# DeepakSridhar/fgdm

Hardware: AMD Instinct MI355X
Metric: 512x512 images/sec @ 50 DDIM steps, seg-ControlNet+CFG (higher is better)
Workload: dtype f16

## Files before the change

### fgdm_amd/_lib.py

```python
import ctypes as C
import os

HERE = os.path.dirname(os.path.abspath(__file__))
LIB_PATH = os.path.join(HERE, 'libfgdm_hip.so')

MAX_LEVELS = 8
MAX_CONTROLNETS = 4

FLAG_USE_ORIGINAL = 1
FLAG_ONLY_MID_CONTROL = 2
FLAG_NO_CONTROL = 4
FLAG_CFG_PAIRS = 8

ACT_NONE, ACT_SILU, ACT_RELU, ACT_GEGLU, ACT_QGELU = 0, 1, 2, 3, 4
OUT_F16, OUT_F32, OUT_F32_NCHW, OUT_F16_T = 0, 1, 2, 3
STRIDE2_PAD_BR = -2


class FgdmConfig(C.Structure):
    _fields_ = [
        ('in_channels', C.c_int32), ('out_channels', C.c_int32), ('model_channels', C.c_int32),
        ('num_res_blocks', C.c_int32), ('n_levels', C.c_int32), ('channel_mult', C.c_int32 * MAX_LEVELS),
        ('n_attention_resolutions', C.c_int32), ('attention_resolutions', C.c_int32 * MAX_LEVELS),
        ('num_heads', C.c_int32), ('context_dim', C.c_int32), ('use_adapter', C.c_int32),
# ... 38 lines not shown

_p = C.c_void_p
_f = C.c_float
_i = C.c_int
_i64 = C.c_int64

SIGNATURES = {
    'fgdm_create': (_i, [C.POINTER(FgdmConfig), _i, C.POINTER(_p)]),
    'fgdm_destroy': (None, [_p]),
    'fgdm_last_error': (C.c_char_p, [_p]),
    'fgdm_param_count': (_i, [C.POINTER(FgdmConfig)]),
    'fgdm_param_info': (_i, [C.POINTER(FgdmConfig), _i, C.c_char_p, _i, C.POINTER(_i64), C.POINTER(_i)]),
    'fgdm_load_tensor': (_i, [_p, C.c_char_p, _p, _i, C.POINTER(_i64), _i]),
    'fgdm_finalize_weights': (_i, [_p]),
    'fgdm_set_hint': (_i, [_p, _i, _p, _i, _i, _i, _p]),
    'fgdm_set_concat': (_i, [_p, _p, _i, _i, _i, _i, _p]),
    'fgdm_set_adapter_conds': (_i, [_p, _p, _i, _i, _i, _i, _p]),
    'fgdm_set_context': (_i, [_p, _p, _i, _p]),
    'fgdm_apply_model': (_i, [_p, _p, _p, _p, _p, _p, _p, _i, _i, _i, _i, _p, _p]),
    'fgdm_clip_encode': (_i, [_p, _p, _i, _i, _p, _p]),
    'fgdm_clip_encode_skip': (_i, [_p, _p, _i, _i, _i, _p, _p]),
    'fgdm_set_context_tokens': (_i, [_p, _i]),
    'fgdm_get_context_tokens': (_i, [_p]),
    'fgdm_run_block': (_i, [_p, C.c_char_p, _p, _i, _p, _i, _p, _p, _i, _i, _i, _p, _i64, C.POINTER(_i64), _p]),
    'fgdm_vae_decode': (_i, [_p, _p, _i, _i, _i, _f, _p, _p]),
    'fgdm_vae_encode': (_i, [_p, _p, _i, _i, _i, _p, _p]),
    'fgdm_unfold': (_i, [_p] + [_i] * 10 + [_p, _p]),
    'fgdm_fold_weighted': (_i, [_p, _p, _p] + [_i] * 9 + [_p, _p]),
    'fgdm_vae_decode_patches': (_i, [_p, _p, _i, _i, _i, _f] + [_i] * 5 + [_p, _p, _i, _p, _p]),
    'fgdm_apply_model_patches': (_i, [_p, _p, _p, _p, _p] + [_i] * 7 + [_p, _p, _i, _i, _p, _p]),
    'fgdm_posterior_sample': (_i, [_p, _p, _f, _p, _i, _i, _i, _p]),
    'fgdm_image_to_uint8': (_i, [_p, _i, _i, _i, _i, _i, _p, _p]),
    'fgdm_resize_linear_uint8': (_i, [_p, _i, _i, _i, _i, _i, _i, _p, _p]),
    'fgdm_uint8_to_hint': (_i, [_p, _i, _i, _i, _i, _p, _p]),
    'fgdm_controlnet': (_i, [_p, _i, _p, _p, _p, _i, _i, _i, _p, _i64, _p]),
    'fgdm_ddim_step': (_i, [_p, _p, _p, _f, _f, _f, _f, _f, _p, _p, _p, _p, _i64, _p]),
    'fgdm_plms_combine': (_i, [_p, _p, _p, _p, _i, _p, _i64, _p]),
    'fgdm_axpby': (_i, [_p, _f, _p, _f, _p, _i64, _p]),
    'fgdm_mask_blend': (_i, [_p, _p, _p, _p, _i64, _p]),
    'fgdm_ancestral_step': (_i, [_p, _p, _f, _f, _f, _f, _f, _p, _p, _i64, _p]),
    'fgdm_sample_ddim': (_i, [_p, _p, _p, _p, _f, _i, C.POINTER(_i64), C.POINTER(_f), C.POINTER(_f), C.POINTER(_f),
                              _p, _i, _i, _i, _i, _p]),
    'fgdm_sample_ddim_ex': (_i, [_p, C.POINTER(FgdmDdimParams), _p]),
    'fgdm_op_ddim_loop_step': (_i, [_p, _p, _p, _f, _f, _f, _f, _f, _p, _p, _p, _p, _f, _f, _p, _p, _p, _p, _p, _i64, _p]),
    'fgdm_sample_plms': (_i, [_p, C.POINTER(FgdmPlmsParams), _p]),
    'fgdm_sample_dpmpp': (_i, [_p, C.POINTER(FgdmDpmppParams), _p]),
    'fgdm_op_plms_loop_step': (_i, [_p, _p, _p, _f, _i, _i, _p, _p, _p, _p, _f, _f, _f, _p, _p, _p, _f, _f, _p, _p, _p, _p, _p,
                                    _i64, _p]),
    'fgdm_op_dpmpp_loop_step': (_i, [_p, _p, _p, _f, _f, _f, _p, _i, _f, _f, _f, _p, _p, _p, _p, _i64, _p]),
    'fgdm_profile_begin': (_i, [_p, _i]),
    'fgdm_profile_end': (_i, [_p, C.POINTER(C.c_double)]),
    'fgdm_workspace_stats': (_i, [_p, C.POINTER(_i64), C.POINTER(_i64)]),
    'fgdm_launch_stats': (_i, [_p, C.POINTER(_i64), C.POINTER(_i64), C.POINTER(_i64)]),
    'fgdm_replay_plan': (_i, [_i, _p, _p, _p, _p, _i, _i, _p, _i, _p]),
    'fgdm_op_conv2d': (_i, [_p, _i, _p, _i, _p, _p, _p, _p, _i, _i, _i, _i, _i, _i, _i, _i, _f, _p, _p]),
    'fgdm_op_linear': (_i, [_p, _p, _p, _p, _i, _i, _i, _i, _i, _i, _i, _p, _p]),
    'fgdm_debug_force_igemm_cfg': (_i, [_i]),
    'fgdm_bench_igemm': (_i, [_i] * 13 + [C.POINTER(_f)]),
    'fgdm_op_linear_ln_linear': (_i, [_p] * 8 + [_i] * 5 + [_p, _p, C.POINTER(_i), _p]),
    'fgdm_bench_norm': (_i, [_i] * 7 + [C.POINTER(_f)]),
    'fgdm_bench_attention': (_i, [_i] * 6 + [C.POINTER(_f)]),
    'fgdm_bench_ff': (_i, [_i] * 4 + [C.POINTER(_f)]),
    'fgdm_op_groupnorm': (_i, [_p, _i, _p, _i, _i, _i, _p, _p, _f, _i, _p, _p]),
    'fgdm_op_layernorm': (_i, [_p, _i, _i, _p, _p, _f, _p, _p]),
    'fgdm_op_attention': (_i, [_p, _i, _p, _i, _p, _i, _p, _i, _i, _i, _i, _i, _i, _p]),
    'fgdm_op_attention_ex': (_i, [_p, _i, _p, _i, _p, _i, _p, _i, _i, _i, _i, _i, _i, _i, _p]),
    'fgdm_debug_last_attention_kernel': (_i, []),
    'fgdm_op_small_attention': (_i, [_p, _i, _i, _i, _p, _i, _i, _i, _i, _i, _i, _p]),
    'fgdm_op_vae_attention': (_i, [_p, _p, _p, _p, _i, _i, _i, _p]),
    'fgdm_op_softmax_rows': (_i, [_p, _p, _i, _i, _p]),
    'fgdm_op_nchw_to_nhwc': (_i, [_p, _p, _i, _i, _i, _i, _p]),
    'fgdm_op_nhwc_to_nchw': (_i, [_p, _p, _i, _i, _i, _p]),
    'fgdm_op_pack_xcat': (_i, [_p, _p, _i, _i, _i, _i, _i, _i, _p, _p]),
    'fgdm_op_avgpool2': (_i, [_p, _p, _i, _i, _i, _i, _p]),
    'fgdm_op_transpose_pad': (_i, [_p, _p, _i, _i, _i, _i, _p]),
    'fgdm_op_timestep_embed': (_i, [_p, _p, _p, _i, _i, _i, _p]),
    'fgdm_op_add_f16': (_i, [_p, _p, _p, _i64, _p]),
    'fgdm_op_ln_qkv': (_i, [_p] * 6 + [_i] * 5 + [_p, _p, _p]),
}

_lib = None


def load():
    global _lib
    if _lib is not None:
        return _lib
    try:
        import torch
    except ImportError:
        pass
    path = os.environ.get('FGDM_LIB') or LIB_PATH
    if not os.path.exists(path):
        raise RuntimeError(f'{path} not found: build it with `python -m fgdm_amd.build` '
                           '(the HIP engine is mandatory, there is no CPU fallback)')
    lib = C.CDLL(os.path.abspath(path))
    for name, (res, args) in SIGNATURES.items():
        fn = getattr(lib, name)
        fn.restype = res
        fn.argtypes = args
    _lib = lib
    return lib
```

### fgdm_amd/csrc/common.h

```cpp
#pragma once
#include <hip/hip_runtime.h>
#include <stdint.h>

typedef _Float16 half_t;
typedef _Float16 h8 __attribute__((ext_vector_type(8)));
typedef _Float16 h4 __attribute__((ext_vector_type(4)));
typedef _Float16 h2 __attribute__((ext_vector_type(2)));
typedef float f32x16 __attribute__((ext_vector_type(16)));
typedef float f32x4 __attribute__((ext_vector_type(4)));

__device__ __forceinline__ float gelu_f(float x) {
    const float z = fminf(fabsf(x), 6.0f);
    float p = -4.7132482596e-04f;
    p = __builtin_fmaf(p, z, 7.0652551839e-03f);
    p = __builtin_fmaf(p, z, -5.1762067461e-02f);
    p = __builtin_fmaf(p, z, -4.6008771426e-01f);
    p = __builtin_fmaf(p, z, -1.1507295505e+00f);
    p = __builtin_fmaf(p, z, -4.8959157159e-05f - 1.0f);
    const float t = __builtin_amdgcn_exp2f(p);
    return __builtin_fmaf(fabsf(x), 0.5f - t, 0.5f * x);
}

typedef float f32x2 __attribute__((ext_vector_type(2)));
__device__ __forceinline__ f32x2 gelu2_f(f32x2 x) {
    const f32x2 ax = {fabsf(x[0]), fabsf(x[1])};
    const f32x2 z = {fminf(ax[0], 6.0f), fminf(ax[1], 6.0f)};
    auto c = [](float k) { return f32x2{k, k}; };
    f32x2 p = c(-4.7132482596e-04f);
    p = __builtin_elementwise_fma(p, z, c(7.0652551839e-03f));
    p = __builtin_elementwise_fma(p, z, c(-5.1762067461e-02f));
    p = __builtin_elementwise_fma(p, z, c(-4.6008771426e-01f));
    p = __builtin_elementwise_fma(p, z, c(-1.1507295505e+00f));
    p = __builtin_elementwise_fma(p, z, c(-4.8959157159e-05f - 1.0f));
    const f32x2 t = {__builtin_amdgcn_exp2f(p[0]), __builtin_amdgcn_exp2f(p[1])};
    return __builtin_elementwise_fma(ax, c(0.5f) - t, c(0.5f) * x);
}

__device__ __forceinline__ float silu_f(float x, float k = 1.0f) {
    return x * __builtin_amdgcn_rcpf(1.0f + __builtin_amdgcn_exp2f(-1.4426950408889634f * k * x));
}

__device__ __forceinline__ float ln_scale(float acc, float mean, float rstd, float u) {
    float t, w;
    asm("v_fma_f32 %0, %1, %2, %3" : "=v"(t) : "v"(-mean), "v"(u), "v"(acc));
    asm("v_mul_f32 %0, %1, %2" : "=v"(w) : "v"(rstd), "v"(t));
    return w;
}

#define FGDM_OK 0
#define FGDM_ERR_ARG -1
#define FGDM_ERR_HIP -2
#define FGDM_ERR_STATE -3
#define FGDM_ERR_NOMEM -4

enum IgemmMode { IG_LINEAR = 0, IG_CONV3 = 1, IG_CONV3_S2 = 2, IG_CONV3_UP2 = 3, IG_CONV3_S2_BR = 4, IG_CONV2_PHASE = 5 };
enum IgemmAct { ACT_NONE = 0, ACT_SILU = 1, ACT_RELU = 2, ACT_GEGLU = 3, ACT_QGELU = 4  };
enum IgemmOut { OUT_F16 = 0, OUT_F32 = 1, OUT_F32_NCHW = 2, OUT_F16_T = 3 };

struct IgemmArgs {
    const half_t* A0;
    const half_t* A1;
    const half_t* Wt;
    const float* bias;
    const float* rowvec;
    const half_t* resid;
    void* out;
    const half_t* zero;
    int C0, C1;
    int B, H, W;
    int Ho, Wo;
    int M, N;
    int K;
    int mode, act, out_kind;
    int ld_out, ld_res;
    int rv_stride;
    int rows_per_sample;
    float scale;
    int force_cfg;
    int splitk;
    float* ws;
    int debug;
    const float* ln_stats;
    const float* ln_u;
    int ln_slots;
    float ln_eps;
    float* stats_out;
    void* out2;
    int split_n, out_kind2, ld_out2;
};

int igemm_launch(const IgemmArgs& a, hipStream_t s);
bool igemm_up_phase(const IgemmArgs& a);
IgemmArgs igemm_phase_args(const IgemmArgs& a, const half_t* wt_phase);
void igemm_set_force_cfg(int cfg);
void igemm_set_twin_layers(bool on);
void igemm_set_pair_hint(int mult);
int igemm2_launch(const IgemmArgs& a, int cfg, hipStream_t s);
int igemm_stats_slots(const IgemmArgs& a);
int row_stats_slots(int C);
int row_stats_launch(const half_t* x, int rows, int C, float* stats , hipStream_t s);
int igemm_splitk_factor(const IgemmArgs& a);
int igemm_splitk_reduce(const IgemmArgs& a, hipStream_t s);
size_t igemm_npad(int n);

#define GN_PIX_PER_CHUNK 256
void groupnorm_set_group(bool on);
int groupnorm_launch(const half_t* x0, int C0, const half_t* x1, int C1, int B, int HW,
                     const float* gamma, const float* beta, float eps, int silu,
                     half_t* out, float* ws , hipStream_t s);
size_t groupnorm_ws_floats(int B, int HW);
int layernorm_launch(const half_t* x, int rows, int C, const float* gamma, const float* beta, float eps,
                     half_t* out, hipStream_t s);

int attention_launch(const half_t* Q, int ldq, const half_t* K, int ldk, const half_t* Vt, int ldvt,
                     half_t* O, int ldo, int B, int H, int T, int Tk, int d, int q_prescaled, hipStream_t s);
int attention_last_kernel();

int nchw_f32_to_nhwc_f16(const float* x, half_t* y, int B, int C, int HW, int Cpad, hipStream_t s);
int pack_xcat(const float* x, const half_t* cc, half_t* y, int B, int Bc, int Cc, int HW, int Cpad, hipStream_t s);
int f32_to_f16(const float* x, half_t* y, size_t n, hipStream_t s);
int silu_f32_to_f16(const float* x, half_t* y, size_t n, hipStream_t s);
int nhwc_f16_to_nchw_f32(const half_t* x, float* y, int B, int C, int HW, hipStream_t s);
int im2col3x3(const half_t* x, half_t* A, int B, int H, int W, int C, int stride, int Kpad, hipStream_t s);
int avgpool2(const half_t* x, half_t* y, int B, int H, int W, int C, hipStream_t s);
int add_f16(const half_t* a, const half_t* b, half_t* y, size_t n, hipStream_t s);
int add_f16_to_f32(const float* a, const half_t* b, float* y, size_t n, hipStream_t s);
int timestep_embed(const int64_t* t, const float* t_float, half_t* y, int B, int dim, int rows_pad, hipStream_t s);
int vae_prequant(const float* z, const float* wb, float scale, half_t* y, int B, int HW, hipStream_t s);
int vae_moments(const float* h, const float* wb, float* moments, int B, int HW, hipStream_t s);
int posterior_sample(const float* moments, const float* noise, float scale, float* z, int B, int zc, int HW, hipStream_t s);
int softmax_rows(const float* S, half_t* P, int rows, int cols, hipStream_t s);
int image_to_u8(const float* x, uint8_t* y, int B, int C, int HW, int mode, hipStream_t s);
int resize_linear_u8(const uint8_t* src, uint8_t* dst, int B, int H, int W, int C, int Ho, int Wo, hipStream_t s);
int u8_to_hint(const uint8_t* src, float* dst, int B, int HW, int C, hipStream_t s);
int embed_tokens(const int64_t* ids, const float* tok, const float* pos, float* out, int rows, int T, int W, int vocab,
                 hipStream_t s);
int layernorm32_launch(const float* x, int rows, int C, const float* gamma, const float* beta, float eps, half_t* out16,
                       float* out32, hipStream_t s);
int f16_to_f32(const half_t* x, float* y, size_t n, hipStream_t s);
int small_attention_launch(const half_t* qkv, int ld, int koff, int voff, half_t* out, int ldo, int B, int heads, int T,
                           int d, int causal, hipStream_t s);
int transpose_pad_keys(const half_t* v, half_t* vt, int B, int Tk, int C, int Tkpad, hipStream_t s);
int ddim_step(const float* x, const float* e_cond, const float* e_uncond, float cfg_scale,
              float a_t, float a_prev, float sigma_t, float sqrt_one_minus_at, const float* noise,
              float* x_prev, float* pred_x0, float* e_out, size_t n, hipStream_t s);
struct DdimLoopStep {
    const float *x, *ec, *eu, *noise, *mask, *x0, *qnoise;
    float *x_out, *xin_a, *xin_b, *log_x, *log_p0;
    float cfg, a_t, a_prev, sigma, s1m, sa_next, s1m_next;
    size_t n;
};
int ddim_loop_step(const DdimLoopStep& a, hipStream_t s);
enum { PLMS_PROBE = 0, PLMS_FINISH_FIRST = 1, PLMS_MULTISTEP = 2 };
struct PlmsLoopStep {
    const float *x, *ec, *eu, *e1, *e2, *e3, *mask, *x0, *qnoise;
    float *e_out, *x_out, *xin_a, *xin_b, *log_x, *log_p0;
    float cfg, a_t, a_prev, s1m, sa_next, s1m_next;
    int mode, order;
    size_t n;
};
int plms_loop_step(const PlmsLoopStep& a, hipStream_t s);
enum { DPMPP_FIRST = 1, DPMPP_SECOND = 2 };
// ... 58 lines not shown
```

### fgdm_amd/csrc/engine.hip

```cpp
#include "model.h"
#include "knobs.h"
#include "replay.h"

#include <algorithm>
#include <array>
#include <cmath>
#include <cstdlib>
#include <cstdio>
#include <cstring>
#include <map>
#include <memory>
#include <string>
#include <unordered_map>
#include <vector>

namespace {

struct Arena {
    struct Blk { char* p; size_t sz; bool free; };
    std::vector<std::vector<Blk>> slabs;
    std::vector<char*> bases;
    size_t slab_bytes = (size_t)4 << 30;
    size_t in_use = 0, peak = 0;
    bool scoped = false;
// ... 66 lines not shown
            if (on) fgdm_record_bracket_begin(cls, w, nbytes, tag);
            return;
        }
        armed = false;
        if (!on || (counter++ % stride) != 0) return;
        armed = true;
        hipEvent_t e = get();
        if (!e) return;
        (void)hipEventRecord(e, s);
        Rec r{cls, used - 1, 0, w, {0}};
        snprintf(r.tag, sizeof(r.tag), "%s", tag);
        recs.push_back(r);
        work[cls] += w;
        bytes[cls] += nbytes;
    }
    void end(hipStream_t s) override {
        if (fgdm_recording()) {
            if (on) fgdm_record_bracket_end();
            return;
        }
        if (!on || !armed || recs.empty()) return;
        armed = false;
        hipEvent_t e = get();
        if (!e) return;
        (void)hipEventRecord(e, s);
        recs.back().e1 = used - 1;
    }
};

}

struct fgdm_engine : Model {
    int device = -1;
    bool device_ready = false, finalized = false;
    struct CtxKV { Tensor k, vt; };
    std::unordered_map<const Layer*, CtxKV> ctx_cache;
    int ctx_B = 0, ctx_T = 0;
    int ctx_tokens = 77;
    Tensor ccat;
    Arena arena;
    half_t* zero = nullptr;
    int cur_comp = -1;
    bool ln_fold = true;
    hipStream_t s = nullptr;
    std::vector<std::unique_ptr<Arena>> cn_arena;
    Arena* ar = &arena;
    hipStream_t s2 = nullptr;
    hipEvent_t ev_fork = nullptr, ev_join = nullptr;
    bool twin_streams = false;
    bool pair_launch = true;
    int group_max = FGDM_MAX_GROUP;
    bool gn_group = true;
    ReplayStats replay_stats;
    struct Deferred { const GemmW* w; Tensor src; int idx; float scale; Arena* owner; };
    Prof prof;

    const ParamSlot* slot(const std::string& name) {
        auto it = params.find(name);
        if (it == params.end() || !it->second.loaded) { err = "parameter not loaded: " + name; return nullptr; }
        return &it->second;
    }
    template <typename T> T* upload(const std::vector<T>& h) {
        T* d = nullptr;
        if (hipMalloc(&d, std::max<size_t>(h.size() * sizeof(T), 256)) != hipSuccess) return nullptr;
        if (hipMemcpy(d, h.data(), h.size() * sizeof(T), hipMemcpyHostToDevice) != hipSuccess) return nullptr;
        comps[cur_comp].allocs.push_back(d);
        return d;
    }
    int pack_rows(GemmW& g, const std::vector<std::pair<const float*, int>>& srcs, int K_src, int K,
                  const std::vector<int>& kmap, const std::vector<const float*>& biases, bool geglu,
                  const std::vector<float>& src_scale = {}, const float* ln_gamma = nullptr, const float* ln_beta = nullptr) {
        int N = 0;
        for (auto& s : srcs) N += s.second;
        const size_t npad = igemm_npad(N);
        std::vector<half_t> w(npad * (size_t)K, (half_t)0);
        std::vector<float> bias(npad, 0.f), lnu(ln_gamma ? npad : 0, 0.f);
        std::vector<const float*> rowp(N);
        std::vector<float> bflat(N, 0.f), rscale(N, 1.f);
        int r = 0;
        for (size_t si = 0; si < srcs.size(); ++si)
            for (int i = 0; i < srcs[si].second; ++i, ++r) {
                rowp[r] = srcs[si].first + (size_t)i * K_src;
                if (si < biases.size() && biases[si]) bflat[r] = biases[si][i];
                if (si < src_scale.size()) rscale[r] = src_scale[si];
            }
        for (int pr = 0; pr < N; ++pr) {
            int sr = pr;
            if (geglu) {
                const int grp = pr >> 6, within = pr & 63;
                sr = within < 32 ? grp * 32 + within : N / 2 + grp * 32 + (within - 32);
            }
            const float* src = rowp[sr];
            const float rs = rscale[sr];
            half_t* dst = w.data() + (size_t)pr * K;
            if (ln_gamma) {
                double us = 0.0, cs = 0.0;
                for (int k = 0; k < K; ++k) {
                    dst[k] = (half_t)(src[k] * rs * ln_gamma[k]);
                    us += (double)(float)dst[k];
                    cs += (double)ln_beta[k] * (double)(src[k] * rs);
                }
                lnu[pr] = (float)us;
                bias[pr] = (float)((double)(bflat[sr] * rs) + cs);
                continue;
            }
            if (kmap.empty()) for (int k = 0; k < K; ++k) dst[k] = (half_t)(src[k] * rs);
// ... 102 lines not shown
        if (comp.packed && !comp.dirty) return FGDM_OK;
        for (auto& name : order) {
            const ParamSlot& ps = params[name];
            if (ps.comp == c && ps.loaded && ps.host.empty())
                return fail(FGDM_ERR_STATE, "tensor " + name + " was released after packing: reload every tensor of " + comp.prefix +
                                            " before finalizing again");
        }
        for (void* p : comp.allocs) (void)hipFree(p);
        comp.allocs.clear();
        cur_comp = c;
        Packer pk{*this};
        visit_component(c, pk);
        cur_comp = -1;
        if (pk.rc != FGDM_OK) return pk.rc;
        for (auto& name : order) { ParamSlot& ps = params[name]; if (ps.comp == c) std::vector<float>().swap(ps.host); }
        comp.packed = true;
        comp.dirty = false;
        return FGDM_OK;
    }

#define CHK(x) do { int _rc = (x); if (_rc != FGDM_OK) return _rc; } while (0)
    int dcopy(void* dst, const void* src, size_t bytes) {
        auto run = [=](hipStream_t rs) -> int { return hipMemcpyAsync(dst, src, bytes, hipMemcpyDeviceToDevice, rs) == hipSuccess ? FGDM_OK : FGDM_ERR_HIP; };
        if (!fgdm_recording()) return run(s);
        fgdm_record(run);
        return FGDM_OK;
    }
    int dzero(void* dst, size_t bytes) {
        auto run = [=](hipStream_t rs) -> int { return hipMemsetAsync(dst, 0, bytes, rs) == hipSuccess ? FGDM_OK : FGDM_ERR_HIP; };
        if (!fgdm_recording()) return run(s);
        fgdm_record(run);
        return FGDM_OK;
    }
    Tensor talloc(int B, int H, int W, int C) {
        Tensor t; t.B = B; t.H = H; t.W = W; t.C = C;
        t.p = (half_t*)ar->alloc(t.numel() * sizeof(half_t));
        return t;
    }
    void tfree(Tensor& t) { ar->release(t.p); t.p = nullptr; }

    struct LnStats { float* p = nullptr; int slots = 0; };
    struct Epi {
        const LnStats* ln = nullptr;
        LnStats* stats = nullptr;
        int act = ACT_NONE;
        const float* rowvec = nullptr; int rv_stride = 0;
        const half_t* resid = nullptr; int ld_res = 0;
        float scale = 1.f;
        int out_kind = OUT_F16;
        void* out = nullptr;
        int ld_out = 0;
        void* out2 = nullptr; int out_kind2 = OUT_F16, ld_out2 = 0, split_n = 0;
        int rps = 0;
    };
    int gemm(const GemmW& w, int mode, const Tensor& x0, const Tensor* x1, int Ho, int Wo, const Epi& e, Tensor* out) {
        IgemmArgs a{};
        a.A0 = x0.p; a.C0 = x0.C;
        a.A1 = x1 ? x1->p : nullptr; a.C1 = x1 ? x1->C : 0;
        a.Wt = w.w; a.bias = w.bias;
        a.rowvec = e.rowvec; a.rv_stride = e.rv_stride;
        a.resid = e.resid; a.ld_res = e.ld_res;
        a.zero = zero;
        a.B = x0.B; a.H = x0.H; a.W = x0.W; a.Ho = Ho; a.Wo = Wo;
        a.M = x0.B * Ho * Wo;
        a.N = w.N;
        a.K = w.K;
        a.mode = mode; a.act = e.act; a.out_kind = e.out_kind;
        const int nout = e.act == ACT_GEGLU ? w.N / 2 : w.N;
        a.out = e.out ? e.out : (void*)out->p;
        a.ld_out = e.ld_out ? e.ld_out : nout;
        a.rows_per_sample = e.rps ? e.rps : Ho * Wo;
        a.scale = e.scale;
        a.out2 = e.out2; a.out_kind2 = e.out_kind2; a.ld_out2 = e.ld_out2; a.split_n = e.split_n;
        const int taps = mode == IG_LINEAR ? 1 : 9;
        if (taps * (a.C0 + a.C1) != a.K) return fail(FGDM_ERR_ARG, "gemm: K mismatch");
        if (!a.out) return fail(FGDM_ERR_NOMEM, "gemm: null output (workspace exhausted?)");
        if (w.wph && !e.stats && !e.ln && igemm_up_phase(a)) a = igemm_phase_args(a, w.wph);
        char tag[56] = "";
        if (prof.on) snprintf(tag, sizeof(tag), "igemm M%d N%d K%d mode%d act%d out%d l%ds%dr%dv%d", a.M, a.N, a.K, a.mode, a.act, a.out_kind,
                              e.ln ? 1 : 0, e.stats ? 1 : 0, e.resid ? 1 : 0, e.rowvec ? 1 : 0);
        a.splitk = igemm_splitk_factor(a);
        if (a.splitk > 1) {
            a.ws = (float*)ar->alloc((size_t)a.splitk * a.M * a.N * sizeof(float));
            if (!a.ws) return fail(FGDM_ERR_NOMEM, "workspace (split-K partials)");
        }
        if (e.ln) {
            if (!w.ln_u || !e.ln->p || a.splitk > 1) return fail(FGDM_ERR_STATE, "gemm: LayerNorm fold without folded weights / statistics");
            a.ln_stats = e.ln->p; a.ln_slots = e.ln->slots; a.ln_u = w.ln_u; a.ln_eps = w.ln_eps;
        } else if (w.ln_u) {
            return fail(FGDM_ERR_STATE, "gemm: these weights have a LayerNorm folded in; statistics are required");
        }
        if (e.stats) {
            e.stats->slots = igemm_stats_slots(a);
            e.stats->p = (float*)ar->alloc((size_t)a.M * std::max(e.stats->slots, row_stats_slots(nout)) * 2 * sizeof(float));
            if (!e.stats->p) return fail(FGDM_ERR_NOMEM, "workspace (LayerNorm statistics)");
            if (e.stats->slots) a.stats_out = e.stats->p;
        }
        double nbytes = 0.0;
        if (prof.on) {
            const double in_b = 2.0 * ((double)x0.numel() + (x1 ? (double)x1->numel() : 0.0));
            const double out_b = (double)a.M * nout * (e.out_kind == OUT_F16 || e.out_kind == OUT_F16_T ? 2.0 : 4.0);
            nbytes = in_b + 2.0 * (double)w.N * w.K + out_b + (e.resid ? 2.0 * (double)a.M * nout : 0.0);
        }
        prof.begin(PC_IGEMM, s, 2.0 * (double)x0.B * Ho * Wo * (double)w.N * (double)w.k_real, tag, nbytes);
        int rc = igemm_launch(a, s);
        prof.end(s);
        if (a.ws) ar->release(a.ws);
        if (rc == FGDM_OK && e.stats && e.stats->slots == 0) {
            if (a.out_kind != OUT_F16 || a.ld_out != nout) return fail(FGDM_ERR_ARG, "gemm: row statistics need a dense fp16 output");
            e.stats->slots = row_stats_slots(nout);
            prof.begin(PC_NORM, s, 2.0 * (double)a.M * nout, "row_stats");
            rc = row_stats_launch((const half_t*)a.out, a.M, nout, e.stats->p, s);
            prof.end(s);
        }
        return rc == FGDM_OK ? rc : fail(rc, "igemm launch failed");
    }
    int conv3(const GemmW& w, const Tensor& x, const Tensor* x1, int stride, bool up, Epi e, Tensor* out) {
        int Ho = x.H, Wo = x.W, mode = IG_CONV3;
        if (up) { Ho *= 2; Wo *= 2; mode = IG_CONV3_UP2; }
        else if (stride == 2) { Ho = (x.H - 1) / 2 + 1; Wo = (x.W - 1) / 2 + 1; mode = IG_CONV3_S2; }
        else if (stride == FGDM_STRIDE2_PAD_BR) { Ho = (x.H - 2) / 2 + 1; Wo = (x.W - 2) / 2 + 1; mode = IG_CONV3_S2_BR; }
        const bool own_out = (e.out == nullptr);
        if (own_out) { *out = talloc(x.B, Ho, Wo, w.N); if (!out->p) return fail(FGDM_ERR_NOMEM, "workspace"); }
        if (!w.im2col) return gemm(w, mode, x, x1, Ho, Wo, e, out);
        if (up || x1 || x.C != w.cin_pad || stride == FGDM_STRIDE2_PAD_BR) return fail(FGDM_ERR_ARG, "im2col conv path: unsupported combination");
        Tensor A = talloc(1, 1, x.B * Ho * Wo, w.K);
        if (!A.p) return fail(FGDM_ERR_NOMEM, "workspace (im2col)");
        prof.begin(PC_ELEM, s, 2.0 * (double)A.numel() + 2.0 * (double)x.numel());
        bool in_gemm = false;
        const int rc = im2col_conv(x.p, A.p, x.B, x.H, x.W, x.C, stride, w.K, s, [&]() { prof.end(s); },
            [&](half_t* Ap, int Bv, int Hv, int Wv, int Kv, int rps) {
                in_gemm = true;
                Tensor Av; Av.p = Ap; Av.B = Bv; Av.H = Hv; Av.W = Wv; Av.C = Kv;
                if (!e.rps) e.rps = rps;
                return gemm(w, IG_LINEAR, Av, nullptr, Hv, Wv, e, out);
            });
        if (rc != FGDM_OK && !in_gemm) return fail(rc, "im2col failed");
        tfree(A);
        return rc;
    }
    int linear(const GemmW& w, const Tensor& x, Epi e, Tensor* out, const Tensor* x1 = nullptr) {
        if (!e.out) { *out = talloc(x.B, x.H, x.W, e.act == ACT_GEGLU ? w.N / 2 : w.N); if (!out->p) return fail(FGDM_ERR_NOMEM, "workspace"); }
        return gemm(w, IG_LINEAR, x, x1, x.H, x.W, e, out);
    }
    int gnorm(const NormW& n, const Tensor& x, const Tensor* x1, float eps, bool silu, Tensor* out) {
        const int C = x.C + (x1 ? x1->C : 0);
        *out = talloc(x.B, x.H, x.W, C);
        float* ws = (float*)ar->alloc(groupnorm_ws_floats(x.B, x.H * x.W) * sizeof(float));
        if (!out->p || !ws) return fail(FGDM_ERR_NOMEM, "workspace");
        char tag[56] = "";
        if (prof.on) snprintf(tag, sizeof(tag), "groupnorm B%d HW%d C%d", x.B, x.H * x.W, C);
        prof.begin(PC_NORM, s, 4.0 * (double)out->numel(), tag);
        const int rc = groupnorm_launch(x.p, x.C, x1 ? x1->p : nullptr, x1 ? x1->C : 0, x.B, x.H * x.W, n.g, n.b, eps,
                                        silu ? 1 : 0, out->p, ws, s);
        prof.end(s);
        ar->release(ws);
        return rc == FGDM_OK ? rc : fail(rc, "groupnorm launch failed");
    }
    int lnorm(const NormW& n, const Tensor& x, Tensor* out) {
        *out = talloc(x.B, x.H, x.W, x.C);
        if (!out->p) return fail(FGDM_ERR_NOMEM, "workspace");
        char tag[56] = "";
        if (prof.on) snprintf(tag, sizeof(tag), "layernorm rows%d C%d", x.rows(), x.C);
        prof.begin(PC_NORM, s, 4.0 * (double)out->numel(), tag);
        const int rc = layernorm_launch(x.p, x.rows(), x.C, n.g, n.b, 1e-5f, out->p, s);
        prof.end(s);
        return rc == FGDM_OK ? rc : fail(rc, "layernorm launch failed");
    }

    struct EmbCtx { const float* emb_all; int stride; };

    int res_fwd(const Layer& l, const Tensor& x, const Tensor* x1, const EmbCtx& ec, Tensor* out) {
        Tensor g1, h, g2, sk, xp;
        CHK(gnorm(l.gn1, x, x1, l.eps, true, &g1));
        const Tensor* xs = &x;
        if (l.down) {
            if (x1) return fail(FGDM_ERR_ARG, "down ResBlock with a concatenated input");
            Tensor gp = talloc(x.B, x.H / 2, x.W / 2, x.C);
            xp = talloc(x.B, x.H / 2, x.W / 2, x.C);
            if (!gp.p || !xp.p) return fail(FGDM_ERR_NOMEM, "workspace");
            if (avgpool2(g1.p, gp.p, x.B, x.H, x.W, x.C, s) != FGDM_OK || avgpool2(x.p, xp.p, x.B, x.H, x.W, x.C, s) != FGDM_OK)
                return fail(FGDM_ERR_ARG, "avgpool2: latent size must be divisible by 8 for the adapter");
            tfree(g1);
            g1 = gp;
            xs = &xp;
        }
        Epi e1;
        if (l.emb_off >= 0) { e1.rowvec = ec.emb_all + l.emb_off; e1.rv_stride = ec.stride; }
        CHK(conv3(l.c1, g1, nullptr, 1, false, e1, &h));
        tfree(g1);
        CHK(gnorm(l.gn2, h, nullptr, l.eps, true, &g2));
        tfree(h);
        Epi e2;
        if (l.cin != l.cout) {
            CHK(linear(l.skip, *xs, Epi{}, &sk, x1));
            e2.resid = sk.p; e2.ld_res = sk.C;
        } else {
            e2.resid = xs->p; e2.ld_res = xs->C;
        }
        CHK(conv3(l.c2, g2, nullptr, 1, false, e2, out));
        tfree(g2);
        if (sk.p) tfree(sk);
        if (xp.p) tfree(xp);
        return FGDM_OK;
    }

    int cross_kv(const Layer& l, const Tensor& ctx16, bool persistent, Tensor* k2, Tensor* v2t) {
        const int B = ctx16.B, C = l.cin, Tk = ctx16.H * ctx16.W, Tkp = roundup(Tk, 64);
        if (persistent) {
            k2->B = B; k2->H = ctx16.H; k2->W = ctx16.W; k2->C = C;
            v2t->B = B; v2t->H = 1; v2t->W = C; v2t->C = Tkp;
            if (hipMalloc(&k2->p, k2->numel() * sizeof(half_t)) != hipSuccess ||
                hipMalloc(&v2t->p, v2t->numel() * sizeof(half_t)) != hipSuccess) return fail(FGDM_ERR_NOMEM, "hipMalloc (context cache)");
            { Epi e; e.out = k2->p; e.ld_out = C; CHK(linear(l.k2, ctx16, e, nullptr)); }
        } else {
            CHK(linear(l.k2, ctx16, Epi{}, k2));
            *v2t = talloc(B, 1, C, Tkp);
            if (!v2t->p) return fail(FGDM_ERR_NOMEM, "workspace");
        }
        if (Tkp != Tk) CHK(dzero(v2t->p, v2t->numel() * sizeof(half_t)));
        { Epi e; e.out_kind = OUT_F16_T; e.out = v2t->p; e.ld_out = Tkp; e.rps = Tk; CHK(linear(l.v2, ctx16, e, nullptr)); }
        return FGDM_OK;
    }
    void drop_context() {
        for (auto& kv : ctx_cache) { (void)hipFree(kv.second.k.p); (void)hipFree(kv.second.vt.p); }
        ctx_cache.clear();
        ctx_B = 0;
    }
    int set_context(const float* ctx, int B) {
        if (!finalized) return fail(FGDM_ERR_STATE, "weights not finalized");
        if (B <= 0) return fail(FGDM_ERR_ARG, "bad shape");
        drop_context();
        Tensor ctx16 = talloc(B, 1, ctx_tokens, cfg.context_dim);
        if (!ctx16.p) return fail(FGDM_ERR_NOMEM, "workspace");
        if (f32_to_f16(ctx, ctx16.p, ctx16.numel(), s) != FGDM_OK) return fail(FGDM_ERR_HIP, "convert kernel");
        auto walk = [&](const Block& blk) -> int {
            for (const Layer& l : blk)
                if (l.type == L_ATTN) { CtxKV kv; CHK(cross_kv(l, ctx16, true, &kv.k, &kv.vt)); ctx_cache[&l] = kv; }
            return FGDM_OK;
        };
        CHK(for_each_block(unet, false, walk));
        for (auto& n : cns) CHK(for_each_block(n, false, walk));
        tfree(ctx16);
        ctx_B = B; ctx_T = ctx_tokens;
        return FGDM_OK;
    }

    int attn_fwd(const Layer& l, const Tensor& x_in, const Tensor& ctx16, Tensor* out, bool dup = false) {
        Tensor x = x_in, x_full;
        int B = x.B;
        const int T = x.H * x.W, C = x.C, d = C / l.heads;
        Tensor g, h, qk, vt, a, h2, q2, k2, v2t, f;
        LnStats s1, s2, s3;
        CHK(gnorm(l.gn, x, nullptr, 1e-6f, false, &g));
        Tensor nrm;
        { Epi e; if (ln_fold) e.stats = &s1; CHK(linear(l.pin, g, e, &h)); }
        tfree(g);
        if (!ln_fold) CHK(lnorm(l.ln1, h, &nrm));
        const Tensor& a1 = ln_fold ? h : nrm;
        const int Tp = roundup(T, 64);
        qk = talloc(B, x.H, x.W, 2 * C);
        vt = talloc(B, 1, C, Tp);
        if (!qk.p || !vt.p) return fail(FGDM_ERR_NOMEM, "workspace");
        if (Tp != T) CHK(dzero(vt.p, vt.numel() * sizeof(half_t)));
        { Epi e; if (ln_fold) e.ln = &s1; e.out = qk.p; e.ld_out = 2 * C; e.rps = T;
          e.out2 = vt.p; e.out_kind2 = OUT_F16_T; e.ld_out2 = Tp; e.split_n = 2 * C;
          CHK(linear(l.qkv1, a1, e, nullptr)); }
        if (s1.p) ar->release(s1.p);
        if (nrm.p) tfree(nrm);
        a = talloc(B, x.H, x.W, C);
        if (!a.p) return fail(FGDM_ERR_NOMEM, "workspace");
        { char tag[56]; snprintf(tag, sizeof(tag), "attn B%d T%d Tk%d d%d", B, T, T, d);
          prof.begin(PC_ATTN, s, 4.0 * (double)B * T * (double)T * C, tag);
          int rc = attention_launch(qk.p, 2 * C, qk.p + C, 2 * C, vt.p, Tp, a.p, C, B, l.heads, T, T, d, 1, s);
          prof.end(s);
          if (rc != FGDM_OK) return fail(rc, "attention launch failed (unsupported head dim?)"); }
        tfree(qk); tfree(vt);
        { Epi e; e.resid = h.p; e.ld_res = C; if (ln_fold) e.stats = &s2; CHK(linear(l.o1, a, e, &h2)); }
        tfree(a); tfree(h);
        if (dup) {
            Tensor f2;
            CHK(dup_rows(h2, &f2)); tfree(h2); h2 = f2;
            CHK(dup_rows(x, &x_full)); x = x_full;
            B *= 2;
        }
        if (dup && ln_fold) {
            const size_t sb = (size_t)(B / 2) * T * s2.slots * 2 * sizeof(float);
            float* s2f = (float*)ar->alloc(2 * sb);
            if (!s2f) return fail(FGDM_ERR_NOMEM, "workspace");
            CHK(dcopy(s2f, s2.p, sb));
            CHK(dcopy((char*)s2f + sb, s2.p, sb));
            ar->release(s2.p); s2.p = s2f;
        }
        if (!ln_fold) CHK(lnorm(l.ln2, h2, &nrm));
        { Epi e; if (ln_fold) e.ln = &s2; CHK(linear(l.q2, ln_fold ? h2 : nrm, e, &q2)); }
        if (s2.p) ar->release(s2.p);
        if (nrm.p) tfree(nrm);
        int Tk, Tkp;
        const bool cached = (ctx16.p == nullptr);
        if (cached) {
            auto it = ctx_cache.find(&l);
            if (it == ctx_cache.end() || ctx_B != B) return fail(FGDM_ERR_STATE, "no cached context for this batch (fgdm_set_context)");
            k2 = it->second.k; v2t = it->second.vt;
            Tk = ctx_T; Tkp = roundup(Tk, 64);
        } else {
            Tk = ctx16.H * ctx16.W; Tkp = roundup(Tk, 64);
            CHK(cross_kv(l, ctx16, false, &k2, &v2t));
        }
        a = talloc(B, x.H, x.W, C);
        if (!a.p) return fail(FGDM_ERR_NOMEM, "workspace");
        { char tag[56]; snprintf(tag, sizeof(tag), "attn B%d T%d Tk%d d%d", B, T, Tk, d);
          prof.begin(PC_ATTN, s, 4.0 * (double)B * T * (double)Tk * C, tag);
          int rc = attention_launch(q2.p, C, k2.p, C, v2t.p, Tkp, a.p, C, B, l.heads, T, Tk, d, 1, s);
          prof.end(s);
          if (rc != FGDM_OK) return fail(rc, "attention launch failed"); }
        tfree(q2);
        if (!cached) { tfree(k2); tfree(v2t); }
        { Epi e; e.resid = h2.p; e.ld_res = C; if (ln_fold) e.stats = &s3; CHK(linear(l.o2, a, e, &h)); }
        tfree(a); tfree(h2);
        if (!ln_fold) CHK(lnorm(l.ln3, h, &nrm));
        { Epi e; if (ln_fold) e.ln = &s3; e.act = ACT_GEGLU; CHK(linear(l.ffp, ln_fold ? h : nrm, e, &f)); }
        if (s3.p) ar->release(s3.p);
        if (nrm.p) tfree(nrm);
        { Epi e; e.resid = h.p; e.ld_res = C; CHK(linear(l.ffo, f, e, &h2)); }
        tfree(f); tfree(h);
        { Epi e; e.resid = x.p; e.ld_res = C; CHK(linear(l.pout, h2, e, out)); }
        tfree(h2);
        if (x_full.p) tfree(x_full);
        return FGDM_OK;
    }

    int dup_rows(const Tensor& h, Tensor* full) {
        *full = talloc(2 * h.B, h.H, h.W, h.C);
        if (!full->p) return fail(FGDM_ERR_NOMEM, "workspace");
        const size_t bytes = h.numel() * sizeof(half_t);
        CHK(dcopy(full->p, h.p, bytes));
        CHK(dcopy((char*)full->p + bytes, h.p, bytes));
        return FGDM_OK;
    }
    int block_fwd_shared(const Block& blk, Tensor xh, bool own_x, const EmbCtx& ec, const Tensor& ctx16, Tensor* out) {
        Tensor cur = xh;
        bool own = own_x, full = false;
        for (size_t j = 0; j < blk.size(); ++j) {
            const Layer& l = blk[j];
            Tensor nxt;
            switch (l.type) {
                case L_CONV: CHK(conv3(l.conv, cur, nullptr, 1, false, Epi{}, &nxt)); break;
                case L_RES: CHK(res_fwd(l, cur, nullptr, ec, &nxt)); break;
                case L_ATTN: CHK(attn_fwd(l, cur, ctx16, &nxt, !full)); full = true; break;
                case L_DOWN: CHK(conv3(l.conv, cur, nullptr, 2, false, Epi{}, &nxt)); break;
                case L_UP: CHK(conv3(l.conv, cur, nullptr, 1, true, Epi{}, &nxt)); break;
            }
            if (own) tfree(cur);
            cur = nxt;
            own = true;
        }
        if (!full) { Tensor f; CHK(dup_rows(cur, &f)); if (own) tfree(cur); cur = f; }
        *out = cur;
        return FGDM_OK;
    }

    int block_fwd(const Block& blk, Tensor x, bool own_x, const Tensor* x1, const EmbCtx& ec, const Tensor& ctx16,
                  const half_t* conv_resid, Tensor* out) {
        Tensor cur = x;
        bool own = own_x;
        for (size_t j = 0; j < blk.size(); ++j) {
            const Layer& l = blk[j];
            Tensor nxt;
            switch (l.type) {
                case L_CONV: { Epi e; if (conv_resid) { e.resid = conv_resid; e.ld_res = l.cout; }
                               CHK(conv3(l.conv, cur, nullptr, 1, false, e, &nxt)); break; }
                case L_RES: CHK(res_fwd(l, cur, j == 0 ? x1 : nullptr, ec, &nxt)); break;
                case L_ATTN: CHK(attn_fwd(l, cur, ctx16, &nxt)); break;
                case L_DOWN: CHK(conv3(l.conv, cur, nullptr, 2, false, Epi{}, &nxt)); break;
                case L_UP: CHK(conv3(l.conv, cur, nullptr, 1, true, Epi{}, &nxt)); break;
            }
            if (own) tfree(cur);
            cur = nxt;
            own = true;
        }
        *out = cur;
        return FGDM_OK;
    }

    int embed(Net& n, const int64_t* t, const float* tf, int B, float** emb_all) {
        const int mc = cfg.model_channels;
        Tensor te = talloc(1, 1, B, mc), e1, e2;
        if (!te.p) return fail(FGDM_ERR_NOMEM, "workspace");
        if (timestep_embed(t, tf, te.p, B, mc, B, s) != FGDM_OK) return fail(FGDM_ERR_HIP, "timestep_embed");
        { Epi e; e.act = ACT_SILU; e.rps = 1; CHK(linear(n.time0, te, e, &e1)); }
        { Epi e; e.act = ACT_SILU; e.rps = 1; CHK(linear(n.time2, e1, e, &e2)); }
        *emb_all = (float*)ar->alloc((size_t)B * n.emb_total * sizeof(float));
        if (!*emb_all) return fail(FGDM_ERR_NOMEM, "workspace");
        { Epi e; e.out_kind = OUT_F32; e.out = *emb_all; e.ld_out = n.emb_total; e.rps = 1; CHK(linear(n.emb_all, e2, e, nullptr)); }
        tfree(te); tfree(e1); tfree(e2);
        return FGDM_OK;
    }

    int adapter_fwd(Net& n, const Tensor& x4, Tensor feats[4]) { return adapter_run(n.ad_conv_in, n.ad_body, x4, feats); }
    int adapter_run(const GemmW& conv_in, const std::vector<AdapterBlk>& body, const Tensor& x4, Tensor feats[4]) {
        Tensor cur;
        CHK(conv3(conv_in, x4, nullptr, 1, false, Epi{}, &cur));
        auto drop = [&](Tensor& t) {
            for (int f = 0; f < 4; ++f) if (feats[f].p == t.p) return;
            tfree(t);
        };
        for (size_t k = 0; k < body.size(); ++k) {
            const AdapterBlk& b = body[k];
            if (b.down) {
                Tensor p = talloc(cur.B, cur.H / 2, cur.W / 2, cur.C);
                if (!p.p) return fail(FGDM_ERR_NOMEM, "workspace");
                if (avgpool2(cur.p, p.p, cur.B, cur.H, cur.W, cur.C, s) != FGDM_OK)
                    return fail(FGDM_ERR_ARG, "avgpool2: latent size must be divisible by 8 for the adapter");
                drop(cur);
                cur = p;
            }
            if (b.ic != b.oc) { Tensor y; CHK(linear(b.in_conv, cur, Epi{}, &y)); drop(cur); cur = y; }
            Tensor h, y;
            { Epi e; e.act = ACT_RELU; CHK(conv3(b.b1, cur, nullptr, 1, false, e, &h)); }
            { Epi e; e.resid = cur.p; e.ld_res = cur.C; CHK(linear(b.b2, h, e, &y)); }
            tfree(h);
            drop(cur);
            cur = y;
            if (k % 2 == 1) feats[k / 2] = cur;
        }
        return FGDM_OK;
    }

    void drop_adapter_conds() {
        for (Tensor& t : unet.xad_sum) { if (t.p) (void)hipFree(t.p); t = Tensor{}; }
        unet.xad_valid = false;
    }
    int set_adapter_conds(const float* const* conds, int nc, int B, int H, int W) {
// ... 318 lines not shown
                        half_t* dst = nxt.p + (size_t)half * fa[k].numel();
                        if (n.xad_valid) {
                            if (n.xad_sum[k].numel() != nxt.numel()) return fail(FGDM_ERR_ARG, "registered adapter conds do not match this batch / latent size");
                            const half_t* xs = n.xad_sum[k].p + (size_t)half * fa[k].numel();
                            if (add_f16(dst, xs, dst, fa[k].numel(), s) != FGDM_OK) return fail(FGDM_ERR_HIP, "add kernel");
                        }
                        if (add_f16(dst, fa[k].p, dst, fa[k].numel(), s) != FGDM_OK) return fail(FGDM_ERR_HIP, "add kernel");
                    }
                    tfree(fa[k]);
                    ++k;
                }
                h = nxt;
                hs.push_back(h);
            }
            CHK(block_fwd(n.middle, h, false, nullptr, ec, ctx16, nullptr, &hm));
            return FGDM_OK;
        };
        if (paired) {
            std::vector<RecWalk> walks(1 + cns.size());
            {
                const bool fat = knob_once(KNOB_PAIR_FAT_TILES) != 0;
                LayerHints fused(*this, false, fat ? std::min<int>(group_max, 1 + (int)cns.size()) : 0);
                groupnorm_set_group(gn_group);
                CHK(controlnets_fwd(x4, t, tf, ctx16, scales, nullptr, nullptr, false, pairs, &deferred,
                                    [&](size_t c) { return RecordScope(*this, &walks[1 + c], cn_arena[c].get()); }));
                RecordScope rec(*this, &walks[0], &arena);
                CHK(encoder());
            }
            std::vector<RecWalk*> lists;
            for (RecWalk& w : walks) lists.push_back(&w);
            CHK(fgdm_replay(lists, group_max, s, prof, replay_stats));
        } else {
            if (twin) {
                if (hipEventRecord(ev_fork, s) != hipSuccess || hipStreamWaitEvent(s2, ev_fork, 0) != hipSuccess) return fail(FGDM_ERR_HIP, "stream fork");
                hipStream_t main_s = s;
                s = s2;
                const int rc = controlnets_fwd(x4, t, tf, ctx16, scales, nullptr, nullptr, false, pairs, &deferred,
                                               [&](size_t) { return RecordScope(*this, nullptr, cn_arena[0].get()); });
                s = main_s;
                if (rc != FGDM_OK) return rc;
                if (hipEventRecord(ev_join, s2) != hipSuccess) return fail(FGDM_ERR_HIP, "stream join");
            }
            CHK(encoder());
        }
        if (twin || paired) {
            if (twin && hipStreamWaitEvent(s, ev_join, 0) != hipSuccess) return fail(FGDM_ERR_HIP, "stream join");
            for (const Deferred& d : deferred) CHK(zero_conv_into(*d.w, d.src, d.idx < 0 ? hm : hs[d.idx], d.scale));
            for (Deferred& d : deferred) { d.owner->release(d.src.p); d.src.p = nullptr; }
        } else if (with_cn) {
            CHK(controlnets_fwd(x4, t, tf, ctx16, scales, &hs, &hm, (flags & FGDM_FLAG_ONLY_MID_CONTROL) != 0, pairs, nullptr,
                                [&](size_t) { return RecordScope(*this, nullptr, &arena); }));
        }
        h = hm;
        for (size_t i = 0; i < n.output.size(); ++i) {
            Tensor skip = hs.back();
            hs.pop_back();
            Tensor nxt;
            CHK(block_fwd(n.output[i], h, true, &skip, ec, ctx16, nullptr, &nxt));
            tfree(skip);
            h = nxt;
        }
        Tensor g;
        CHK(gnorm(n.out_gn, h, nullptr, 1e-5f, true, &g));
        tfree(h);
        { Epi e; e.out_kind = OUT_F32_NCHW; e.out = eps_out; e.ld_out = HW; CHK(conv3(n.out_conv, g, nullptr, 1, false, e, nullptr)); }
        tfree(g);
        tfree(x4);
        if (ctx16.p) tfree(ctx16);
        ar->release(emb);
        return FGDM_OK;
    }

    int clip_encode(const int64_t* ids, int B, int T, float* out, int clip_skip = 0) {
        if (!clip.on) return fail(FGDM_ERR_STATE, "engine was created without a text encoder (clip_layers = 0)");
        if (!comps[clip_comp].packed) return fail(FGDM_ERR_STATE, "weights not finalized");
        if (B <= 0 || T <= 0 || T > cfg.clip_max_len) return fail(FGDM_ERR_ARG, "bad shape (T must be <= clip_max_len)");
        if (clip_skip > cfg.clip_layers + 1) return fail(FGDM_ERR_ARG, "clip_skip exceeds the number of hidden states");
        const int n_run = cfg.clip_layers - (clip_skip > 1 ? clip_skip - 1 : 0);
        int li = 0;
        const int W = cfg.clip_width, rows = B * T;
        Tensor n, qkv, a, f;
        float* h = (float*)ar->alloc((size_t)rows * W * sizeof(float));
        float* h2 = (float*)ar->alloc((size_t)rows * W * sizeof(float));
        if (!h || !h2) return fail(FGDM_ERR_NOMEM, "workspace");
        if (embed_tokens(ids, clip.tok, clip.pos, h, rows, T, W, cfg.clip_vocab, s) != FGDM_OK) return fail(FGDM_ERR_HIP, "embedding kernel");
        auto ln32 = [&](const NormW& nw, const float* src, Tensor* dst) -> int {
            *dst = talloc(1, 1, rows, W);
            if (!dst->p) return fail(FGDM_ERR_NOMEM, "workspace");
            return layernorm32_launch(src, rows, W, nw.g, nw.b, 1e-5f, dst->p, nullptr, s) == FGDM_OK ? FGDM_OK : fail(FGDM_ERR_HIP, "layernorm");
        };
        for (const ClipLayer& l : clip.layers) {
            if (li++ >= n_run) break;
            CHK(ln32(l.ln1, h, &n));
            CHK(linear(l.qkv, n, Epi{}, &qkv));
            tfree(n);
            a = talloc(1, 1, rows, W);
            if (!a.p) return fail(FGDM_ERR_NOMEM, "workspace");
            if (small_attention_launch(qkv.p, 3 * W, W, 2 * W, a.p, W, B, cfg.clip_heads, T, W / cfg.clip_heads, 1, s) != FGDM_OK)
                return fail(FGDM_ERR_HIP, "text attention kernel");
            tfree(qkv);
            Tensor br;
            CHK(linear(l.o, a, Epi{}, &br));
            tfree(a);
            if (add_f16_to_f32(h, br.p, h2, br.numel(), s) != FGDM_OK) return fail(FGDM_ERR_HIP, "add kernel");
            tfree(br);
            CHK(ln32(l.ln2, h2, &n));
            { Epi e; e.act = ACT_QGELU; CHK(linear(l.fc1, n, e, &f)); }
            tfree(n);
            CHK(linear(l.fc2, f, Epi{}, &br));
            tfree(f);
            if (add_f16_to_f32(h2, br.p, h, br.numel(), s) != FGDM_OK) return fail(FGDM_ERR_HIP, "add kernel");
            tfree(br);
        }
        if (layernorm32_launch(h, rows, W, clip.final_ln.g, clip.final_ln.b, 1e-5f, nullptr, out, s) != FGDM_OK) return fail(FGDM_ERR_HIP, "layernorm");
        ar->release(h); ar->release(h2);
        return FGDM_OK;
// ... 139 lines not shown
    void drop_concat() { if (ccat.p) (void)hipFree(ccat.p); ccat = Tensor{}; }
    int set_concat(const float* cc, int B, int Cc, int H, int W) {
        if (cfg.in_channels == 4) return fail(FGDM_ERR_ARG, "fgdm_set_concat: this engine's UNet takes x alone (in_channels = 4)");
        if (!cc) { drop_concat(); return FGDM_OK; }
        if (Cc != cfg.in_channels - 4) {
            drop_concat();
            return fail(FGDM_ERR_ARG, "fgdm_set_concat: c_concat must have in_channels - 4 = " + std::to_string(cfg.in_channels - 4) + " channels");
        }
        if (B <= 0 || H <= 0 || W <= 0) { drop_concat(); return fail(FGDM_ERR_ARG, "bad shape"); }
        if (ccat.p && (ccat.B != B || ccat.H != H || ccat.W != W)) drop_concat();
        if (!ccat.p) {
            ccat.B = B; ccat.H = H; ccat.W = W; ccat.C = Cc;
            if (hipMalloc(&ccat.p, ccat.numel() * sizeof(half_t)) != hipSuccess) { ccat = Tensor{}; return fail(FGDM_ERR_NOMEM, "hipMalloc (c_concat cache)"); }
        }
        if (nchw_f32_to_nhwc_f16(cc, ccat.p, B, Cc, H * W, Cc, s) != FGDM_OK) return fail(FGDM_ERR_HIP, "layout kernel");
        return FGDM_OK;
    }
};

static std::string g_create_err;

static int make_desc(const fgdm_config* cfg, fgdm_engine** out) {
    fgdm_engine* e = new fgdm_engine();
    e->cfg = *cfg;
    const int rc = e->build();
    if (rc != FGDM_OK) { g_create_err = "unsupported configuration: " + e->err; delete e; return rc; }
    *out = e;
    return FGDM_OK;
}

template <typename F> static int scoped_call(fgdm_engine* e, void* stream, F f) {
    e->s = as_stream(stream);
    e->ar = &e->arena;
    e->arena.begin_scope();
    for (auto& a : e->cn_arena) a->begin_scope();
    const int rc = f();
    e->s = as_stream(stream);
    e->ar = &e->arena;
    if (rc != FGDM_OK && e->s2) (void)hipStreamSynchronize(e->s2);
    e->arena.end_scope(rc != FGDM_OK);
    for (auto& a : e->cn_arena) a->end_scope(rc != FGDM_OK);
    return rc;
}

extern "C" {

int fgdm_create(const fgdm_config* cfg, int device, fgdm_engine** out) {
    if (!cfg || !out) return FGDM_ERR_ARG;
    fgdm_engine* e = nullptr;
    int rc = make_desc(cfg, &e);
    if (rc != FGDM_OK) return rc;
    e->device = device;
    e->ln_fold = knob_on(KNOB_LN_FOLD);
    rc = e->ensure_device();
    if (rc != FGDM_OK) {
        g_create_err = e->err + " [" + hipGetErrorString(hipGetLastError()) + "]";
        delete e;
        return rc;
    }
    e->twin_streams = knob_on(KNOB_TWIN_STREAMS);
    e->pair_launch = knob_on(KNOB_PAIR_LAUNCH);
    e->group_max = std::max(2, std::min(FGDM_MAX_GROUP, knob_int(KNOB_GROUP_MAX)));
    e->gn_group = knob_on(KNOB_GN_GROUP);
    if (e->twin_streams && !e->cns.empty()) {
        if (hipStreamCreateWithFlags(&e->s2, hipStreamNonBlocking) != hipSuccess ||
            hipEventCreateWithFlags(&e->ev_fork, hipEventDisableTiming) != hipSuccess ||
            hipEventCreateWithFlags(&e->ev_join, hipEventDisableTiming) != hipSuccess) {
            g_create_err = "second stream could not be created";
            delete e;
            return FGDM_ERR_HIP;
        }
    }
    for (size_t c = 0; c < e->cns.size(); ++c) {
        e->cn_arena.emplace_back(new Arena());
        if (e->cfg.workspace_bytes > 0) e->cn_arena.back()->slab_bytes = (size_t)e->cfg.workspace_bytes;
    }
    *out = e;
    return FGDM_OK;
}

void fgdm_destroy(fgdm_engine* e) {
    if (!e) return;
    for (hipEvent_t ev : e->prof.pool) (void)hipEventDestroy(ev);
    for (auto& c : e->comps) for (void* p : c.allocs) (void)hipFree(p);
    if (e->zero) (void)hipFree(e->zero);
    for (auto& n : e->cns) if (n.guided.p) (void)hipFree(n.guided.p);
    e->drop_concat();
    e->drop_context();
    e->drop_adapter_conds();
    if (knob_text(KNOB_PAIR_DEBUG) && e->replay_stats.replayed)
        fprintf(stderr, "[fgdm] grouped twin launches: %ld of %ld replayed launches were fused (%ld problems)\n", e->replay_stats.fused, e->replay_stats.replayed, e->replay_stats.problems);
    if (e->s2) { (void)hipStreamSynchronize(e->s2); (void)hipStreamDestroy(e->s2); }
    if (e->ev_fork) (void)hipEventDestroy(e->ev_fork);
    if (e->ev_join) (void)hipEventDestroy(e->ev_join);
    delete e;
}

const char* fgdm_last_error(const fgdm_engine* e) { return e ? e->err.c_str() : g_create_err.c_str(); }

static fgdm_engine* g_desc = nullptr;
static fgdm_config g_desc_cfg;
static fgdm_engine* desc_for(const fgdm_config* cfg) {
    if (g_desc && memcmp(&g_desc_cfg, cfg, sizeof(*cfg)) == 0) return g_desc;
    if (g_desc) { delete g_desc; g_desc = nullptr; }
    if (make_desc(cfg, &g_desc) != FGDM_OK) return nullptr;
    g_desc_cfg = *cfg;
// ... 61 lines not shown
    e->prof.counter = 0;
    e->prof.used = 0;
    e->prof.recs.clear();
    for (int c = 0; c < PC_COUNT; ++c) { e->prof.work[c] = 0; e->prof.bytes[c] = 0; }
    return FGDM_OK;
}
int fgdm_profile_end(fgdm_engine* e, double* out) {
    if (!e || !out) return FGDM_ERR_ARG;
    e->prof.on = false;
    if (hipDeviceSynchronize() != hipSuccess) return e->fail(FGDM_ERR_HIP, "hipDeviceSynchronize failed");
    for (int c = 0; c < PC_COUNT * 4; ++c) out[c] = 0;
    for (auto& r : e->prof.recs) {
        if (!r.e1) continue;
        float ms = 0.f;
        if (hipEventElapsedTime(&ms, e->prof.pool[r.e0], e->prof.pool[r.e1]) != hipSuccess) continue;
        out[r.cls * 4 + 0] += ms;
        out[r.cls * 4 + 1] += 1;
    }
    for (int c = 0; c < PC_COUNT; ++c) { out[c * 4 + 2] = e->prof.work[c]; out[c * 4 + 3] = e->prof.bytes[c]; }
    if (const char* path = knob_text(KNOB_PROF_DUMP)) {
        std::map<std::string, std::array<double, 3>> agg;
        for (auto& r : e->prof.recs) {
            if (!r.e1) continue;
            float ms = 0.f;
            if (hipEventElapsedTime(&ms, e->prof.pool[r.e0], e->prof.pool[r.e1]) != hipSuccess) continue;
            auto& a = agg[r.tag];
            a[0] += 1; a[1] += ms; a[2] += r.w;
        }
        if (FILE* f = fopen(path, "w")) {
            for (auto& kv : agg) fprintf(f, "%s\t%.0f\t%.4f\t%.6g\n", kv.first.c_str(), kv.second[0], kv.second[1], kv.second[2]);
            fclose(f);
        }
    }
    return FGDM_OK;
}
int fgdm_workspace_stats(fgdm_engine* e, int64_t* peak_bytes, int64_t* reserved_bytes) {
    if (!e || !peak_bytes || !reserved_bytes) return FGDM_ERR_ARG;
    size_t pk = e->arena.peak, r = 0;
    for (auto& sl : e->arena.slabs) for (auto& b : sl) r += b.sz;
    for (auto& a : e->cn_arena) {
        pk += a->peak;
        for (auto& sl : a->slabs) for (auto& b : sl) r += b.sz;
    }
    *peak_bytes = (int64_t)pk;
    *reserved_bytes = (int64_t)r;
    return FGDM_OK;
}

int fgdm_launch_stats(fgdm_engine* e, int64_t* replayed_launches, int64_t* fused_launches, int64_t* fused_problems) {
    if (!e || !replayed_launches || !fused_launches || !fused_problems) return FGDM_ERR_ARG;
    *replayed_launches = (int64_t)e->replay_stats.replayed;
    *fused_launches = (int64_t)e->replay_stats.fused;
    *fused_problems = (int64_t)e->replay_stats.problems;
    return FGDM_OK;
}

int fgdm_set_hint(fgdm_engine* e, int cn, const float* hint, int B, int Hh, int Wh, void* stream) {
    if (!e || !hint) return FGDM_ERR_ARG;
    return scoped_call(e, stream, [&] { return e->set_hint(cn, hint, B, Hh, Wh); });
}

int fgdm_set_concat(fgdm_engine* e, const float* c_concat, int B, int Cc, int H, int W, void* stream) {
    if (!e) return FGDM_ERR_ARG;
    return scoped_call(e, stream, [&] { return e->set_concat(c_concat, B, Cc, H, W); });
}

int fgdm_apply_model(fgdm_engine* e, const float* x, const int64_t* t, const float* t_float, const float* ctx,
                     const float* pcond, const float* control_scales, int B, int H, int W, int flags, float* eps_out,
                     void* stream) {
    if (!e || !x || (!t && !t_float) || !eps_out) return FGDM_ERR_ARG;
    return scoped_call(e, stream, [&] { return e->apply_model(x, t, t_float, ctx, pcond, control_scales, B, H, W, flags, eps_out); });
}

int fgdm_set_adapter_conds(fgdm_engine* e, const float* const* conds, int n_conds, int B, int H, int W, void* stream) {
    if (!e) return FGDM_ERR_ARG;
    return scoped_call(e, stream, [&] { return e->set_adapter_conds(conds, n_conds, B, H, W); });
}

int fgdm_set_context(fgdm_engine* e, const float* ctx, int B, void* stream) {
    if (!e || !ctx) return FGDM_ERR_ARG;
    return scoped_call(e, stream, [&] { return e->set_context(ctx, B); });
}

int fgdm_clip_encode(fgdm_engine* e, const int64_t* ids, int B, int T, float* out, void* stream) {
    if (!e || !ids || !out) return FGDM_ERR_ARG;
    return scoped_call(e, stream, [&] { return e->clip_encode(ids, B, T, out); });
}

int fgdm_clip_encode_skip(fgdm_engine* e, const int64_t* ids, int B, int T, int clip_skip, float* out, void* stream) {
    if (!e || !ids || !out) return FGDM_ERR_ARG;
    return scoped_call(e, stream, [&] { return e->clip_encode(ids, B, T, out, clip_skip); });
}

int fgdm_set_context_tokens(fgdm_engine* e, int tokens) {
    if (!e) return FGDM_ERR_ARG;
    if (tokens < 1) return e->fail(FGDM_ERR_ARG, "context token count must be >= 1");
    if (tokens != e->ctx_tokens) { e->drop_context(); e->ctx_tokens = tokens; }
    return FGDM_OK;
}

int fgdm_get_context_tokens(const fgdm_engine* e) { return e ? e->ctx_tokens : FGDM_ERR_ARG; }

int fgdm_vae_decode(fgdm_engine* e, const float* z, int B, int H, int W, float scale, float* image, void* stream) {
    if (!e || !z || !image) return FGDM_ERR_ARG;
    return scoped_call(e, stream, [&] { return e->vae_decode(z, B, H, W, scale, image); });
}
// ... 438 lines not shown
```

### fgdm_amd/csrc/igemm.hip

```cpp
#include "common.h"
#include "knobs.h"
#include <algorithm>

#define LDS_AS __attribute__((address_space(3)))
#define GLB_AS __attribute__((address_space(1)))

__device__ __forceinline__ void glds16(const void* g, void* lds_wave_base) {
    __builtin_amdgcn_global_load_lds((const GLB_AS void*)g, (LDS_AS void*)lds_wave_base, 16, 0, 0);
}

template <int BM, int BN, int WM, int WN>
__global__ __launch_bounds__(WM * WN * 64) void igemm_kernel(const IgemmArgs a) {
    constexpr int T = WM * WN * 64;
    constexpr int TM = BM / WM, TN = BN / WN;
    constexpr int MI = TM / 32, NI = TN / 32;
    constexpr int A_IT = BM * 8 / T, B_IT = BN * 8 / T;
    constexpr int A_BYTES = BM * 128, STAGE = (BM + BN) * 128;
    static_assert(A_IT >= 1 && B_IT >= 1, "tile too small for the thread count");
    extern __shared__ __attribute__((aligned(16))) char smem[];

    const int tid = threadIdx.x, lane = tid & 63;
    const int wave = __builtin_amdgcn_readfirstlane(tid >> 6);
    const int wm = wave / WN, wn = wave % WN;

// ... 249 lines not shown
}

static int g_force_cfg = 0;
void igemm_set_force_cfg(int cfg) { g_force_cfg = cfg; }
static thread_local int g_pair_mult = 1;
void igemm_set_pair_hint(int mult) { g_pair_mult = mult > 1 ? mult : 1; }

static int pick_force(const IgemmArgs& a) {
    int force = a.force_cfg ? a.force_cfg : g_force_cfg;
    if (a.act == ACT_QGELU) {
        if (force >= 4) force = 0;
        if (force == 0) return 0;
    }
    const bool small_tiles = knob_once(KNOB_IGEMM_SMALL_TILES) != 0;
    const bool other_widths = knob_once(KNOB_IGEMM_OTHER_WIDTHS) != 0;
    if (a.mode == IG_CONV2_PHASE) {
        if (force >= 4) return force;
        return (long)((a.M + 255) / 256) * (a.N / 320) * 4 * g_pair_mult >= 192 ? 4 : 6;
    }
    if (force == 0) {
        const bool geglu = a.act == ACT_GEGLU;
        if (!geglu && a.N % 320 == 0) {
            const long b256 = (long)((a.M + 255) / 256) * (a.N / 320);
            const long b128 = (long)((a.M + 127) / 128) * (a.N / 320);
            const bool small_m = knob_once(KNOB_IGEMM_SMALL_M) != 0;
            const bool lin64 = a.mode == IG_LINEAR && !(a.K & 31) && !(a.C0 & 31) && !(a.C1 & 31) && small_tiles;
            const long b64 = (long)((a.M + 63) / 64) * (a.N / 160);
            const long b256n = (long)((a.M + 255) / 256) * (a.N / 128);
            if (b256 * g_pair_mult >= 192) force = 4;
            else if (small_m && lin64 && a.K >= 2560 && !(a.N % 128) && !a.ln_stats && !a.stats_out && !a.out2 && b128 >= 96 && b128 * g_pair_mult < 192 &&
                     b64 >= 512 && b256n >= 144 && b256n <= 256) force = 10;
            else if (b128 >= 96 && !(small_m && lin64 && b128 * g_pair_mult < 192 && b64 >= 512)) force = 6;
            else if (lin64 && b64 >= 128) force = 11;
        } else if (geglu && a.N % 256 == 0 && (long)((a.M + 255) / 256) * (a.N / 256) >= 128) {
            force = 5;
        } else if (!geglu && !a.ln_stats && !(a.K & 31) && !(a.C0 & 31) && !(a.C1 & 31) && other_widths) {
            const long rows = (a.M + 255) / 256;
            if (a.N % 256 == 0 && rows * (a.N / 256) >= 192) force = 5;
            else if (a.N == 128 && rows >= 192) force = 10;
        }
    }
    return force;
}

int igemm_stats_slots(const IgemmArgs& a) {
    if (a.out_kind != OUT_F16 || a.act == ACT_GEGLU || a.splitk > 1 || (a.N % 320) || (a.K & 31) || (a.C0 & 31) || (a.C1 & 31)) return 0;
    const int f = pick_force(a);
    if (f < 4) return 0;
    const int tile = (f - 4) & 15;
    const bool stats64 = knob_once(KNOB_IGEMM_STATS64) != 0;
    return (tile == 0 || tile == 2 || tile == 3 || tile == 5 || (tile == 7 && stats64)) ? a.N / 160 : 0;
}

bool igemm_up_phase(const IgemmArgs& a) {
    if (!knob_once(KNOB_IGEMM_UP_PHASE)) return false;
    const int force = a.force_cfg ? a.force_cfg : g_force_cfg;
    if (force >= 1 && force <= 3) return false;
    if (a.H * a.W < 64) return false;
    return a.mode == IG_CONV3_UP2 && !a.C1 && a.C0 > 0 && !(a.C0 & 63) && a.K == 9 * a.C0 && a.N % 320 == 0 && a.out_kind == OUT_F16 &&
           a.act != ACT_GEGLU && a.act != ACT_QGELU && !a.rowvec && !a.stats_out && !a.out2 && !a.ln_stats;
}
IgemmArgs igemm_phase_args(const IgemmArgs& a, const half_t* wt_phase) {
    IgemmArgs p = a;
    p.mode = IG_CONV2_PHASE;
    p.Wt = wt_phase;
    p.K = 4 * a.C0;
    p.M = a.B * a.H * a.W;
    p.rows_per_sample = a.H * a.W;
    p.splitk = 1; p.ws = nullptr;
    return p;
}

int igemm_launch(const IgemmArgs& a, hipStream_t s) {
    if (a.M <= 0 || a.N <= 0 || a.K <= 0 || (a.K & 63) || (a.C0 & 63) || (a.C1 & 63)) return FGDM_ERR_ARG;
    if (a.act == ACT_GEGLU && (a.N & 63)) return FGDM_ERR_ARG;
    if (a.ln_stats && (a.mode != IG_LINEAR || a.C1 || a.ln_slots <= 0 || !a.ln_u)) return FGDM_ERR_ARG;
    if (a.stats_out && igemm_stats_slots(a) == 0) return FGDM_ERR_ARG;
    if (a.out2 && (a.act == ACT_GEGLU || a.splitk > 1 || a.stats_out || a.split_n <= 0 || a.split_n >= a.N || (a.split_n % 640))) return FGDM_ERR_ARG;
    if (a.mode == IG_CONV2_PHASE && (a.splitk > 1 || a.N % 320)) return FGDM_ERR_ARG;
    if (a.splitk > 1) {
        if (!a.ws || a.ln_stats) return FGDM_ERR_ARG;
        const bool fat = (long)((a.M + 255) / 256) * (a.N / 320) * a.splitk >= 192 && !(a.K & 31) && !(a.C0 & 31) && !(a.C1 & 31);
        const int rc = igemm2_launch(a, fat ? 0 : 2, s);
        return rc == FGDM_OK ? igemm_splitk_reduce(a, s) : rc;
    }
    int force = pick_force(a);
    const bool mfma32 = knob_once(KNOB_IGEMM_MFMA32) != 0;
    if (mfma32 && force >= 4 && force <= 6 && !a.force_cfg && !g_force_cfg) force += 3;
    if (force >= 4) return igemm2_launch(a, force - 4, s);
    struct Cfg { int bm, bn; float eff; int per_cu; };
    static const Cfg cfgs[] = {{128, 128, 1.00f, 2}, {128, 64, 0.80f, 3}, {64, 64, 0.62f, 4}};
    int best = 0;
    float best_cost = 1e30f;
    for (int i = 0; i < 3; ++i) {
        const Cfg& c = cfgs[i];
        const long nblk = (long)((a.M + c.bm - 1) / c.bm) * ((a.N + c.bn - 1) / c.bn);
        const long slots = 256L * c.per_cu;
        const float rounds = (float)((nblk + slots - 1) / slots);
        const long conc = std::min<long>(c.per_cu, (nblk + 255) / 256);
        const float cost = rounds * (float)conc * (float)(c.bm * c.bn) / c.eff;
        if (cost < best_cost) { best_cost = cost; best = i; }
    }
    if ((long)((a.M + 127) / 128) * ((a.N + 127) / 128) < 256) best = 2;
    if (a.act == ACT_GEGLU) best = 0;
    if (force >= 1 && force <= 3) best = force - 1;
    switch (best) {
        case 0: return launch_cfg<128, 128, 2, 2>(a, s);
        case 1: return launch_cfg<128, 64, 2, 2>(a, s);
        default: return launch_cfg<64, 64, 2, 2>(a, s);
    }
}
```

### fgdm_amd/csrc/igemm2.hip

```cpp
#include "common.h"
#include "knobs.h"
#include <algorithm>
#include <type_traits>

#pragma clang diagnostic ignored "-Winline-asm"
#define LDS_AS __attribute__((address_space(3)))
#define GLB_AS __attribute__((address_space(1)))

namespace {

__device__ __forceinline__ void glds16(const void* g, unsigned lds_wave_addr) {
    unsigned keep;
    asm volatile("s_mov_b32 %0, m0\n\ts_mov_b32 m0, %2\n\ts_nop 0\n\tglobal_load_lds_dwordx4 %1, off\n\ts_mov_b32 m0, %0"
                 : "=&s"(keep)
                 : "v"(g), "s"(lds_wave_addr)
                 : "memory", "m0");
}
__device__ __forceinline__ void glds16_m0(const void* g, unsigned lds_wave_addr) {
    asm volatile("s_mov_b32 m0, %1\n\ts_nop 0\n\tglobal_load_lds_dwordx4 %0, off" ::"v"(g), "s"(lds_wave_addr) : "memory", "m0");
}
__device__ __forceinline__ void glds16_sv(unsigned voff, const void* sbase, unsigned lds_wave_addr) {
    asm volatile("s_mov_b32 m0, %2\n\ts_nop 0\n\tglobal_load_lds_dwordx4 %0, %1" ::"v"(voff), "s"(sbase), "s"(lds_wave_addr) : "memory", "m0");
}
__device__ __forceinline__ unsigned lds_addr(const void* p) { return (unsigned)(size_t)(LDS_AS const void*)p; }
template <int N> __device__ __forceinline__ void wait_vmcnt() {
    asm volatile("s_waitcnt vmcnt(%0)" ::"n"(N) : "memory");
}

constexpr int BK = 32;
constexpr int ROWB = BK * 2;

constexpr int RV_MAX = 6;

template <int BM> constexpr int halo_px() { return BM == 256 ? 400 : 272; }
template <int BM, int BN, int STAGES, int PIPE> constexpr int ring_bytes() {
    return PIPE == 2 ? 2 * halo_px<BM>() * ROWB + STAGES * BN * ROWB : STAGES * (BM + BN) * ROWB;
}

template <int BM, int BN, int WM, int WN, int STAGES, int CONV, bool GEGLU, bool SPLIT, int MS, bool LN, int PATH, int PIPE, bool ABL>
__device__ __forceinline__ void igemm2_body(const IgemmArgs& a, const int yb) {
    constexpr int NW = WM * WN, T = NW * 64;
    constexpr int TM = BM / WM, TN = BN / WN;
    constexpr int MI = TM / MS, NI = TN / MS;
    constexpr int KS = MS == 32 ? 2 : 1;
    constexpr int AR = MS == 32 ? 16 : 4;
    typedef float acc_t __attribute__((ext_vector_type(AR)));
    auto swz_of = [](int r) { return MS == 32 ? ((r >> 2) & 3) : (((r >> 3) & 1) << 1); };
    constexpr int A_INSTR = BM * 4 / 64, B_INSTR = BN * 4 / 64;
    static_assert(A_INSTR % NW == 0, "A tile must split evenly over the waves");
    constexpr int LA = A_INSTR / NW, LB = (B_INSTR + NW - 1) / NW;
    constexpr int LPS = LA + LB;
    constexpr int STAGE_BYTES = (BM + BN) * ROWB;
    constexpr int A_BYTES = BM * ROWB;
    constexpr int RING_BYTES = ring_bytes<BM, BN, STAGES, PIPE>();
    static_assert(TM % 32 == 0 && TN % MS == 0, "wave tile: 32-pixel epilogue passes, MFMA-sized channel tiles");
    static_assert(!GEGLU || TN % 64 == 0, "GEGLU: whole 64-row [32 value | 32 gate] groups per wave");
    extern __shared__ __attribute__((aligned(16))) char smem[];

    const int tid = threadIdx.x, lane = tid & 63;
    const int wave = __builtin_amdgcn_readfirstlane(tid >> 6);
    const int wm = wave / WN, wn = wave % WN;

    const int ntn = (a.N + BN - 1) / BN;
    const int nb = gridDim.x;
    int logical;
    {
        const int bid = blockIdx.x, xcd = bid & 7, q = nb >> 3, r = nb & 7;
        logical = (xcd < r ? xcd * (q + 1) : r * (q + 1) + (xcd - r) * q) + (bid >> 3);
    }
    const int nsplit = SPLIT ? a.splitk : 1;
    int split = 0, m0, n0;
    if (SPLIT) {
        const int ntm = (a.M + BM - 1) / BM;
        const int row = logical % ntm, pair = logical / ntm;
        split = pair % nsplit; n0 = (pair / nsplit) * BN; m0 = row * BM;
    } else {
        m0 = (logical / ntn) * BM; n0 = (logical % ntn) * BN;
    }

    const int nk_all = a.K >> 5;
    const int per = (nk_all + nsplit - 1) / nsplit;
    const int k_begin = split * per;
    const int nk = max(0, min(per, nk_all - k_begin));

    int a_pix[LA], a_yx[LA], a_off[LA];
    int b_off[LB], b_lds[LB];
    const int br = (CONV && a.mode == IG_CONV3_S2_BR) ? 1 : 0;
    const int sy = (CONV && (a.mode == IG_CONV3_S2 || a.mode == IG_CONV3_S2_BR)) ? 2 : 1;
    const int up = (CONV && a.mode == IG_CONV3_UP2) ? 1 : 0;
    constexpr bool ph = CONV == 2;
    const int pa = ph ? (yb >> 1) : 0, pb = ph ? (yb & 1) : 0;
    const int NT = ph ? 4 : 9;
    const int Wq = ph ? a.W : a.Wo, hwq = ph ? a.H * a.W : a.Ho * a.Wo;
// ... 430 lines not shown
                    const int col = n0 + wn * TN + j * MS + (MS == 32 ? 8 * g : 0) + lq;
                    f32x4 pk = {acc[j][i][g * 4], acc[j][i][g * 4 + 1], acc[j][i][g * 4 + 2], acc[j][i][g * 4 + 3]};
                    *(f32x4*)(wsp + (size_t)row * a.N + col) = pk;
                }
        }
        return;
    } else {
    if (ABL && (a.debug & 4)) {
        float sink = 0.f;
#pragma unroll
        for (int j = 0; j < NI; ++j)
#pragma unroll
            for (int i = 0; i < MI; ++i) sink += acc[j][i][0] + acc[j][i][AR - 1];
        if (sink == 12345.678f) ((float*)a.out)[0] = sink;
        return;
    }
    asm volatile("s_waitcnt lgkmcnt(0)" ::: "memory");
    __builtin_amdgcn_s_barrier();
    if constexpr (LN) {
        const float* uw = u_l + wn * TN;
#pragma unroll
        for (int j = 0; j < NI; ++j)
#pragma unroll
            for (int g = 0; g < AR / 4; ++g) {
                const f32x4 uq = *(const f32x4*)(uw + j * MS + (MS == 32 ? 8 * g : 0) + lq);
#pragma unroll
                for (int i = 0; i < MI; ++i) {
                    const int trow = wm * TM + i * MS + lrow;
                    const float mean = mr_l[2 * trow], rstd = mr_l[2 * trow + 1];
#pragma unroll
                    for (int e = 0; e < 4; ++e) acc[j][i][g * 4 + e] = ln_scale(acc[j][i][g * 4 + e], mean, rstd, uq[e]);
                }
            }
    }
    constexpr int OUT_TN = GEGLU ? TN / 2 : TN;
    constexpr int PITCH = OUT_TN * 2 + 8;
    constexpr int CPR = OUT_TN / 8;
    constexpr int WB_IT = (32 * CPR + 63) / 64;
    static_assert(!GEGLU || NI % 2 == 0, "GEGLU needs value/gate tile pairs");
    constexpr bool TR = PATH == 1 && LN && !GEGLU;
    constexpr int TPITCH = 32 * 2 + 16;
    constexpr int CST_BYTES = TR && OUT_TN * TPITCH > 32 * PITCH ? OUT_TN * TPITCH : 32 * PITCH;
    static_assert(NW * CST_BYTES <= RING_BYTES, "epilogue staging must fit in the ring");
    char* cst = smem + wave * CST_BYTES;
    const bool second = a.out2 && n0 >= a.split_n;
    void* const outp = second ? a.out2 : a.out;
    const int okind = second ? a.out_kind2 : a.out_kind, ldo = second ? a.ld_out2 : a.ld_out;
    const int ncol0 = second ? a.split_n : 0, nend = a.out2 ? (second ? a.N : a.split_n) : a.N;
    const bool tr = TR && okind == OUT_F16_T;
    const int ocol0 = GEGLU ? ((n0 + wn * TN) >> 1) : (n0 + wn * TN - ncol0);
    const int nvalid = GEGLU ? a.N / 2 : nend - ncol0;
    const float* bw = bias_l + wn * TN;

    constexpr int PT = 32 / MS;
    constexpr int NG = AR / 4;
#pragma unroll
    for (int ip = 0; ip < TM / 32; ++ip) {
#pragma unroll
      for (int hf = 0; hf < PT; ++hf) {
        const int i = ip * PT + hf;
        const int prow = hf * MS + lrow;
        const int row = m0 + wm * TM + ip * 32 + prow;
        const int bsmp = (a.rowvec && row < a.M) ? row / rps : smp0;
        const float* rw = rv_l + (bsmp - smp0) * BN + wn * TN;
#pragma unroll
        for (int j = 0; j < NI; ++j) {
            if (GEGLU && (MS == 32 ? (j & 1) : (j & 2))) continue;
#pragma unroll
            for (int g = 0; g < NG; ++g) {
                const int wc = j * MS + (MS == 32 ? 8 * g : 0) + lq;
                const f32x4 bq = *(const f32x4*)(bw + wc);
                float v[4];
#pragma unroll
                for (int e = 0; e < 4; ++e) v[e] = acc[j][i][g * 4 + e] + bq[e];
                if (PATH == 2 || (PATH == 0 && a.rowvec)) {
                    if (PATH == 2 || rv_in_lds) {
                        const f32x4 rq = *(const f32x4*)(rw + wc);
#pragma unroll
                        for (int e = 0; e < 4; ++e) v[e] += rq[e];
                    } else if (row < a.M) {
#pragma unroll
                        for (int e = 0; e < 4; ++e) v[e] += a.rowvec[(size_t)bsmp * a.rv_stride + n0 + wn * TN + wc + e];
                    }
                }
                if (PATH == 0 && a.act == ACT_SILU) {
#pragma unroll
                    for (int e = 0; e < 4; ++e) v[e] = silu_f(v[e]);
                } else if (PATH == 0 && a.act == ACT_RELU) {
#pragma unroll
                    for (int e = 0; e < 4; ++e) v[e] = fmaxf(v[e], 0.f);
                }
                if constexpr (GEGLU) {
                    constexpr int GJ = MS == 32 ? 1 : 2;
                    const f32x4 gq = *(const f32x4*)(bw + wc + 32);
                    const f32x2 g01 = gelu2_f(f32x2{acc[j + GJ][i][g * 4] + gq[0], acc[j + GJ][i][g * 4 + 1] + gq[1]});
                    const f32x2 g23 = gelu2_f(f32x2{acc[j + GJ][i][g * 4 + 2] + gq[2], acc[j + GJ][i][g * 4 + 3] + gq[3]});
                    v[0] *= g01[0]; v[1] *= g01[1]; v[2] *= g23[0]; v[3] *= g23[1];
                }
#pragma unroll
                for (int e = 0; e < 4; ++e) v[e] *= a.scale;
                const int oc = !GEGLU ? wc : (MS == 32 ? (j >> 1) * 32 + 8 * g + lq : (j >> 2) * 32 + (j & 1) * 16 + lq);
                if (TR && tr) {
#pragma unroll
                    for (int e = 0; e < 4; ++e) *(half_t*)(cst + (oc + e) * TPITCH + prow * 2) = (half_t)v[e];
                } else if (PATH != 0 || okind == OUT_F16) {
                    h4 pk = {(half_t)v[0], (half_t)v[1], (half_t)v[2], (half_t)v[3]};
// ... 17 lines not shown
        }
      }
        if (TR && tr) {
            asm volatile("s_waitcnt lgkmcnt(0)" ::: "memory");
            const int row0 = m0 + wm * TM + ip * 32;
            const int b = row0 / rps, t0 = row0 - b * rps;
            constexpr int TT = OUT_TN * 4;
            if (row0 < a.M) {
#pragma unroll
                for (int it = 0; it < (TT + 63) / 64; ++it) {
                    const int task = lane + it * 64, c = task >> 2, q = task & 3;
                    if (task < TT && ocol0 + c < nvalid) {
                        const h8 val = *(const h8*)(cst + c * TPITCH + q * 16);
                        *(h8*)((half_t*)outp + ((size_t)b * nvalid + ocol0 + c) * ldo + t0 + q * 8) = val;
                    }
                }
            }
            asm volatile("s_waitcnt lgkmcnt(0)" ::: "memory");
        } else if (PATH != 0 || okind == OUT_F16) {
            asm volatile("s_waitcnt lgkmcnt(0)" ::: "memory");
            h8 v[WB_IT], rr[WB_IT];
            size_t goff[WB_IT];
            bool ok[WB_IT];
#pragma unroll
            for (int it = 0; it < WB_IT; ++it) {
                const int c = lane + it * 64;
                const int pr = c / CPR, ck = c - pr * CPR;
                const int grow = m0 + wm * TM + ip * 32 + pr;
                const int gcol = ocol0 + ck * 8;
                ok[it] = c < 32 * CPR && grow < a.M && gcol < nvalid;
                size_t orow = (size_t)grow;
                if (ph) {
                    const int img = grow / hwq, rem = grow - img * hwq, si = rem / a.W, sj = rem - si * a.W;
                    orow = ((size_t)img * a.Ho + (size_t)(2 * si + pa)) * a.Wo + (size_t)(2 * sj + pb);
                }
                goff[it] = orow * ldo + gcol;
                if (ok[it]) {
                    const char* sp = cst + pr * PITCH + ck * 16;
                    const h4 lo = *(const h4*)sp, hi = *(const h4*)(sp + 8);
                    v[it] = h8{lo[0], lo[1], lo[2], lo[3], hi[0], hi[1], hi[2], hi[3]};
                    if (a.resid) rr[it] = *(const h8*)(a.resid + orow * a.ld_res + gcol);
                }
            }
            bool want_stats = false;
            constexpr bool HALF = OUT_TN == 80 && WN == 2 && TM == 32 && !GEGLU;
            if constexpr (OUT_TN == 160 || HALF) want_stats = a.stats_out != nullptr;
            float* tab = (float*)cst;
            if (want_stats) asm volatile("s_waitcnt lgkmcnt(0)" ::: "memory");
#pragma unroll
            for (int it = 0; it < WB_IT; ++it) {
                if (ok[it]) {
                    if (a.resid) v[it] = v[it] + rr[it];
                    *(h8*)((half_t*)outp + goff[it]) = v[it];
                }
                if (want_stats) {
                    const int c = lane + it * 64;
                    if (c < 32 * CPR) {
                        float sm = 0.f, sq = 0.f;
                        if (ok[it]) {
#pragma unroll
                            for (int e = 0; e < 8; ++e) { const float f = (float)v[it][e]; sm += f; sq += f * f; }
                        }
                        tab[2 * c] = sm; tab[2 * c + 1] = sq;
                    }
                }
            }
            asm volatile("s_waitcnt lgkmcnt(0)" ::: "memory");
            if constexpr (HALF) {
                if (want_stats) {
                    __builtin_amdgcn_s_barrier();
                    if (wn == 0 && lane < 32) {
                        const float* tab1 = (const float*)(smem + (wave + 1) * CST_BYTES);
                        const int grow = m0 + wm * TM + ip * 32 + lane;
                        float sm = 0.f, sq = 0.f;
#pragma unroll
                        for (int k = 0; k < CPR; ++k) { sm += tab[2 * (lane * CPR + k)]; sq += tab[2 * (lane * CPR + k) + 1]; }
#pragma unroll
                        for (int k = 0; k < CPR; ++k) { sm += tab1[2 * (lane * CPR + k)]; sq += tab1[2 * (lane * CPR + k) + 1]; }
                        if (grow < a.M) {
                            float* dst = a.stats_out + ((size_t)grow * (a.N / 160) + n0 / 160) * 2;
                            dst[0] = sm; dst[1] = sq;
                        }
                    }
                    asm volatile("s_waitcnt lgkmcnt(0)" ::: "memory");
                }
            } else
            if (want_stats) {
                if (lane < 32) {
                    const int grow = m0 + wm * TM + ip * 32 + lane;
                    float sm = 0.f, sq = 0.f;
#pragma unroll
                    for (int k = 0; k < CPR; ++k) { sm += tab[2 * (lane * CPR + k)]; sq += tab[2 * (lane * CPR + k) + 1]; }
                    if (grow < a.M) {
                        float* dst = a.stats_out + ((size_t)grow * (a.N / 160) + (n0 + wn * TN) / 160) * 2;
                        dst[0] = sm; dst[1] = sq;
                    }
                }
                asm volatile("s_waitcnt lgkmcnt(0)" ::: "memory");
            }
        }
    }
    }
}

template <int BM, int BN, int WM, int WN, int STAGES, int CONV, bool GEGLU, bool SPLIT, int MS, bool LN, int PATH, int PIPE, bool ABL>
__global__ __launch_bounds__(WM * WN * 64) void igemm2_kernel(const IgemmArgs a) {
    igemm2_body<BM, BN, WM, WN, STAGES, CONV, GEGLU, SPLIT, MS, LN, PATH, PIPE, ABL>(a, (int)blockIdx.y);
}
struct IgemmArgsG { IgemmArgs g[FGDM_MAX_GROUP]; };
template <int BM, int BN, int WM, int WN, int STAGES, int CONV, bool GEGLU, bool SPLIT, int MS, bool LN, int PATH, int PIPE, bool ABL>
__global__ __launch_bounds__(WM * WN * 64) void igemm2_pair_kernel(const IgemmArgsG p) {
    igemm2_body<BM, BN, WM, WN, STAGES, CONV, GEGLU, SPLIT, MS, LN, PATH, PIPE, ABL>(p.g[blockIdx.y], 0);
}

template <bool LN>
__global__ __launch_bounds__(512) void igemm2_geglu_persist_kernel(const IgemmArgs a, int ntiles, int contiguous) {
    constexpr int BM = 256, BN = 256, WM = 4, WN = 2, NW = 8, T = 512, STAGES = 4, MS = 16;
    constexpr int TM = BM / WM, TN = BN / WN, MI = TM / MS, NI = TN / MS, AR = 4;
    typedef float acc_t __attribute__((ext_vector_type(AR)));
    constexpr int LA = BM * 4 / 64 / NW, LB = BN * 4 / 64 / NW, LPS = LA + LB;
    constexpr int STAGE_BYTES = (BM + BN) * ROWB, A_BYTES = BM * ROWB, RING_BYTES = STAGES * STAGE_BYTES;
    constexpr int OPS_FLOATS = BN + 2 * BM + BN;
    extern __shared__ __attribute__((aligned(16))) char smem[];
    auto swz_of = [](int r) { return ((r >> 3) & 1) << 1; };

    const int tid = threadIdx.x, lane = tid & 63;
    const int wave = __builtin_amdgcn_readfirstlane(tid >> 6);
    const int wm = wave / WN, wn = wave % WN;
    const int ntn = a.N / BN;
    const int nk = a.K >> 5;
    const int xcd = blockIdx.x & 7, G8 = gridDim.x >> 3, tq = ntiles >> 3, tr = ntiles & 7;
    const int x_first = xcd < tr ? xcd * (tq + 1) : tr * (tq + 1) + (xcd - tr) * tq, x_count = tq + (xcd < tr ? 1 : 0);
    const int per = (x_count + G8 - 1) / G8, jw = blockIdx.x >> 3;
    const int t_first = contiguous ? x_first + jw * per : x_first + jw;
    const int t_count = contiguous ? min(per, x_count - jw * per) : (x_count - jw + G8 - 1) / G8;
    const int t_step = contiguous ? 1 : G8;
    int local = 0;
    if (t_count <= 0) return;

    const int lrow = lane & (MS - 1), lh = lane / MS, lq = 4 * lh;
    const int koff = lrow * ROWB + ((lh ^ swz_of(lrow)) << 4);
    unsigned a_b0[LA], a_ok[LA], b_b[LB];
    int b_lds[LB];
    auto setup = [&](int m0x, int n0x) {
#pragma unroll
        for (int i = 0; i < LA; ++i) {
            const int q = (wave + i * NW) * 64 + lane, r = q >> 2, sp = q & 3, m = m0x + r;
            a_ok[i] = m < a.M ? 1u : 0u;
            a_b0[i] = a_ok[i] ? ((unsigned)m * (unsigned)a.C0 + (unsigned)((sp ^ swz_of(r)) << 3)) * 2u : 0u;
        }
#pragma unroll
// ... 221 lines not shown
    if (fgdm_dyn_lds<k>(smem) != FGDM_OK) return FGDM_ERR_HIP;
    const int ntm = (a.M + BM - 1) / BM, ntn = (a.N + BN - 1) / BN;
    const unsigned gx = (unsigned)(ntm * ntn * (SPLIT ? a.splitk : 1));
    constexpr bool phases = CONV == 2;
    const unsigned gy = phases ? 4u : 1u;
    if (fgdm_recording()) {
        auto single = [=](hipStream_t rs) -> int {
            hipLaunchKernelGGL(k, dim3(gx, gy), dim3(WM * WN * 64), smem, rs, a);
            return hipGetLastError() == hipSuccess ? FGDM_OK : FGDM_ERR_HIP;
        };
        if (phases) { fgdm_record(single); return FGDM_OK; }
        if constexpr (PIPE != 0 && PATH != 0 && !SPLIT && !ABL && MS == 16) {
            constexpr auto kp = igemm2_pair_kernel<BM, BN, WM, WN, STAGES, CONV, GEGLU, SPLIT, MS, LN, PATH, PIPE, ABL>;
            if (fgdm_dyn_lds<kp>(smem) != FGDM_OK) return FGDM_ERR_HIP;
            static_assert(sizeof(IgemmArgs) <= FGDM_GROUP_BLOB, "the recorded blob holds an IgemmArgs");
            FgdmGroupFn pf = [](const void* const* av, int n, unsigned grid_x, hipStream_t rs) -> int {
                if (n < 2 || n > FGDM_MAX_GROUP) return FGDM_ERR_ARG;
                IgemmArgsG pg;
                for (int i = 0; i < FGDM_MAX_GROUP; ++i) pg.g[i] = *(const IgemmArgs*)av[i < n ? i : 0];
                hipLaunchKernelGGL((igemm2_pair_kernel<BM, BN, WM, WN, STAGES, CONV, GEGLU, SPLIT, MS, LN, PATH, PIPE, ABL>), dim3(grid_x, n),
                                   dim3(WM * WN * 64), smem, rs, pg);
                return hipGetLastError() == hipSuccess ? FGDM_OK : FGDM_ERR_HIP;
            };
            fgdm_record(single, (const void*)kp, pf, &a, sizeof(a), gx, 0);
        } else {
            fgdm_record(single);
        }
        return FGDM_OK;
    }
    hipLaunchKernelGGL(k, dim3(gx, gy), dim3(WM * WN * 64), smem, s, a);
    return hipGetLastError() == hipSuccess ? FGDM_OK : FGDM_ERR_HIP;
}
template <int BM, bool GEGLU, bool LN>
int epilogue_path(const IgemmArgs& a) {
    if (a.out_kind != OUT_F16 || !(a.act == ACT_NONE || GEGLU)) return 0;
    if (a.out2 && a.out_kind2 != OUT_F16) {
        const bool staged = LN && a.out_kind2 == OUT_F16_T && a.rows_per_sample % 32 == 0 && a.M % 32 == 0 && a.ld_out2 % 8 == 0 &&
                            ((size_t)a.out2 & 15) == 0;
        if (!staged || a.rowvec) return 0;
    }
    if (!a.rowvec) return 1;
    return (BM - 1) / a.rows_per_sample + 2 <= RV_MAX ? 2 : 0;
}
template <int BM, int BN, int WM, int WN, int STAGES, int CONV, bool GEGLU, bool SPLIT, int MS, bool LN, bool FAST, int PIPE>
int launch2(const IgemmArgs& a, hipStream_t s) {
    const bool fast_on = knob_once(KNOB_IGEMM_EPI_PATHS) != 0;
    if constexpr (FAST && !SPLIT && !LN) {
        if (a.debug)
            return epilogue_path<BM, GEGLU, LN>(a) == 1 ? launch2p<BM, BN, WM, WN, STAGES, CONV, GEGLU, SPLIT, MS, LN, 1, (PIPE == 2 ? 1 : PIPE), true>(a, s)
                                                        : FGDM_ERR_ARG;
    }
    if (a.debug) return FGDM_ERR_ARG;
    if constexpr (SPLIT) return launch2p<BM, BN, WM, WN, STAGES, CONV, GEGLU, SPLIT, MS, LN, 0, PIPE, false>(a, s);
    if constexpr (FAST && !SPLIT) {
        switch (fast_on ? epilogue_path<BM, GEGLU, LN>(a) : 0) {
            case 1: return launch2p<BM, BN, WM, WN, STAGES, CONV, GEGLU, SPLIT, MS, LN, 1, PIPE, false>(a, s);
            case 2: if constexpr (!GEGLU && !LN && CONV != 2) return launch2p<BM, BN, WM, WN, STAGES, CONV, GEGLU, SPLIT, MS, LN, 2, PIPE, false>(a, s);
            default: break;
        }
    }
    if constexpr (CONV == 2 && BM == 256 && BN == 320 && MS == 16) return launch2p<128, BN, WM, WN, STAGES, CONV, GEGLU, SPLIT, MS, LN, 0, 0, false>(a, s);
    else return launch2p<BM, BN, WM, WN, STAGES, CONV, GEGLU, SPLIT, MS, LN, 0, 0, false>(a, s);
}
template <int BM, int BN, bool GEGLU, int MS, int PIPE, int WM, int WN>
int launch2m(const IgemmArgs& a, hipStream_t s) {
    constexpr int PL = PIPE == 2 ? 1 : PIPE;
    if (a.mode == IG_CONV2_PHASE) {
        if constexpr (!GEGLU) return launch2<BM, BN, WM, WN, 4, 2, false, false, MS, false, MS == 16, PL>(a, s);
        else return FGDM_ERR_ARG;
    }
    return a.mode == IG_LINEAR ? launch2<BM, BN, WM, WN, 4, 0, GEGLU, false, MS, false, MS == 16, PL>(a, s)
                               : launch2<BM, BN, WM, WN, 4, 1, GEGLU, false, MS, false, MS == 16, (GEGLU ? PL : PIPE)>(a, s);
}
template <int BM, int BN, bool GEGLU, int MS, int PIPE, int WM, int WN>
int launch2ln(const IgemmArgs& a, hipStream_t s) {
    return launch2<BM, BN, WM, WN, 4, false, GEGLU, false, MS, true, MS == 16, (PIPE == 2 ? 1 : PIPE)>(a, s);
}
template <int BM, int BN, int MS, int PIPE, int WM = 4, int WN = 2>
int launch_tile(const IgemmArgs& a, hipStream_t s) {
    const bool g = a.act == ACT_GEGLU;
    if (a.ln_stats) {
        if constexpr (BN == 256) { if (g) return launch2ln<BM, BN, true, MS, PIPE, WM, WN>(a, s); }
        if constexpr (BN == 128) return FGDM_ERR_ARG;
        else return launch2ln<BM, BN, false, MS, PIPE, WM, WN>(a, s);
    }
    if constexpr (BN == 256) { if (g) return launch2m<BM, BN, true, MS, PIPE, WM, WN>(a, s); }
    return launch2m<BM, BN, false, MS, PIPE, WM, WN>(a, s);
}

__global__ __launch_bounds__(256) void splitk_reduce_kernel(const IgemmArgs a) {
    const size_t total4 = (size_t)a.M * a.N / 4, plane = (size_t)a.M * a.N;
    for (size_t i = (size_t)blockIdx.x * 256 + threadIdx.x; i < total4; i += (size_t)gridDim.x * 256) {
        const size_t e0 = i * 4;
        const int row = (int)(e0 / a.N), col = (int)(e0 - (size_t)row * a.N);
        f32x4 v = *(const f32x4*)(a.ws + e0);
        for (int s = 1; s < a.splitk; ++s) {
            const f32x4 u = *(const f32x4*)(a.ws + (size_t)s * plane + e0);
            v[0] += u[0]; v[1] += u[1]; v[2] += u[2]; v[3] += u[3];
        }
        h4 r = {(half_t)0, (half_t)0, (half_t)0, (half_t)0};
        if (a.resid) r = *(const h4*)(a.resid + (size_t)row * a.ld_res + col);
        h4 o;
#pragma unroll
        for (int e = 0; e < 4; ++e) {
            float x = v[e] + (a.bias ? a.bias[col + e] : 0.f);
            if (a.rowvec) x += a.rowvec[(size_t)(row / a.rows_per_sample) * a.rv_stride + col + e];
            if (a.act == ACT_SILU) x = silu_f(x);
            else if (a.act == ACT_RELU) x = fmaxf(x, 0.f);
            else if (a.act == ACT_QGELU) x = silu_f(x, 1.702f);
            const half_t y = (half_t)(x * a.scale);
            o[e] = a.resid ? (half_t)((float)y + (float)r[e]) : y;
        }
        *(h4*)((half_t*)a.out + (size_t)row * a.ld_out + col) = o;
    }
}

}

static thread_local bool g_twin_layers = false;
void igemm_set_twin_layers(bool on) { g_twin_layers = on; }

int igemm_splitk_factor(const IgemmArgs& a) {
    if (a.force_cfg || a.act == ACT_GEGLU || a.out_kind != OUT_F16 || a.N % 320 || (a.K & 31)) return 1;
    if (a.mode == IG_CONV2_PHASE) return 1;
    const int nk = a.K >> 5;
    const bool fat = knob_once(KNOB_SPLITK_FAT) != 0;
    if (fat && a.rows_per_sample > 64 && a.rows_per_sample <= 256 && (nk >= 540 || (nk >= 360 && !g_twin_layers))) return 2;
    if (a.rows_per_sample > 64 || nk < 96) return 1;
    return (fat && nk >= 360) ? 8 : 4;
}
int igemm_splitk_reduce(const IgemmArgs& a, hipStream_t s) {
    const size_t total4 = (size_t)a.M * a.N / 4;
    const int grid = (int)std::min<size_t>(2048, (total4 + 255) / 256);
    FGDM_LAUNCH(splitk_reduce_kernel, dim3(grid), dim3(256), 0, s, a);
    return hipGetLastError() == hipSuccess ? FGDM_OK : FGDM_ERR_HIP;
}

static bool halo_geometry(const IgemmArgs& a) {
    if (a.mode != IG_CONV3 || a.Ho != a.H || a.Wo != a.W || (a.C0 & 63) || (a.C1 & 63) || (a.K % 288) || a.debug) return false;
    if ((a.W == 16 || a.W == 32 || a.W == 64) && (a.H * a.W) % 256 == 0) return true;
    return a.W == 8 && a.H == 8;
}

int igemm2_launch(const IgemmArgs& a, int cfg, hipStream_t s) {
    if ((a.K & 31) || (a.C0 & 31) || (a.C1 & 31)) return FGDM_ERR_ARG;
    const int pipe_default = knob_once(KNOB_IGEMM_PIPE);
    const int tile = cfg & 15, psel = cfg >> 4;
    const size_t px = a.mode == IG_LINEAR ? (size_t)a.M : (size_t)a.B * a.H * a.W;
    const bool small = px * (size_t)std::max(a.C0, a.C1) * 2 < (1ull << 32) && (size_t)(a.N + 320) * a.K * 2 < (1ull << 32);
    const bool pipe = (psel == 0 ? pipe_default != 0 : psel == 2) && small;
    if (a.mode == IG_CONV2_PHASE && (a.splitk > 1 || a.C1 || a.out_kind != OUT_F16 || a.stats_out || a.out2 || a.ln_stats || a.act == ACT_GEGLU ||
                                     a.Ho != 2 * a.H || a.Wo != 2 * a.W || a.K != 4 * a.C0 || a.M != a.B * a.H * a.W || !small))
        return FGDM_ERR_ARG;
    const bool halo = knob_once(KNOB_IGEMM_HALO) != 0 && pipe && halo_geometry(a);
    const int bn = (tile == 1 || tile == 4) ? 256 : tile == 6 ? 128 : tile == 7 ? 160 : 320;
    if (a.N % bn) return FGDM_ERR_ARG;
    if (a.act == ACT_GEGLU && bn != 256) return FGDM_ERR_ARG;
    if (a.splitk > 1) {
        if ((tile != 2 && tile != 0) || a.ln_stats) return FGDM_ERR_ARG;
        const int nk_all = a.K >> 5;
        if (halo && nk_all % a.splitk == 0 && (nk_all / a.splitk) % 9 == 0)
            return tile == 0 ? launch2<256, 320, 4, 2, 4, true, false, true, 16, false, false, 2>(a, s)
                             : launch2<128, 320, 4, 2, 4, true, false, true, 16, false, false, 2>(a, s);
        if (tile == 0 && pipe)
            return a.mode == IG_LINEAR ? launch2<256, 320, 4, 2, 4, false, false, true, 16, false, false, 1>(a, s)
                                       : launch2<256, 320, 4, 2, 4, true, false, true, 16, false, false, 1>(a, s);
        if (pipe)
            return a.mode == IG_LINEAR ? launch2<128, 320, 4, 2, 4, false, false, true, 16, false, false, 1>(a, s)
                                       : launch2<128, 320, 4, 2, 4, true, false, true, 16, false, false, 1>(a, s);
        return a.mode == IG_LINEAR ? launch2<128, 320, 4, 2, 4, false, false, true, 16, false, false, 0>(a, s)
                                   : launch2<128, 320, 4, 2, 4, true, false, true, 16, false, false, 0>(a, s);
    }
    if (a.ln_stats && a.mode != IG_LINEAR) return FGDM_ERR_ARG;
    const int persist_mode = knob_once(KNOB_IGEMM_PERSIST);
    const bool persist_on = persist_mode != 0;
    if (persist_on && tile == 1 && pipe && a.act == ACT_GEGLU && a.mode == IG_LINEAR && !a.C1 && a.out_kind == OUT_F16 && !a.rowvec &&
        !a.resid && !a.out2 && !a.stats_out && !a.debug && a.N % 256 == 0) {
        const int ntiles = ((a.M + 255) / 256) * (a.N / 256);
        if (ntiles > 256) return a.ln_stats ? launch_geglu_persist<true>(a, ntiles, persist_mode == 2, s) : launch_geglu_persist<false>(a, ntiles, persist_mode == 2, s);
    }
    switch (tile) {
        case 0: return halo ? launch_tile<256, 320, 16, 2>(a, s) : pipe ? launch_tile<256, 320, 16, 1>(a, s) : launch_tile<256, 320, 16, 0>(a, s);
        case 1: return pipe ? launch_tile<256, 256, 16, 1>(a, s) : launch_tile<256, 256, 16, 0>(a, s);
        case 2: return halo ? launch_tile<128, 320, 16, 2>(a, s) : pipe ? launch_tile<128, 320, 16, 1>(a, s) : launch_tile<128, 320, 16, 0>(a, s);
        case 3: return launch_tile<256, 320, 32, 0>(a, s);
        case 4: return launch_tile<256, 256, 32, 0>(a, s);
        case 5: return launch_tile<128, 320, 32, 0>(a, s);
        case 6: return pipe ? launch_tile<256, 128, 16, 1>(a, s) : launch_tile<256, 128, 16, 0>(a, s);
        case 7: return a.mode != IG_LINEAR ? FGDM_ERR_ARG : pipe ? launch_tile<64, 160, 16, 1, 2, 2>(a, s) : launch_tile<64, 160, 16, 0, 2, 2>(a, s);
        default: return FGDM_ERR_ARG;
    }
}
```

### fgdm_amd/csrc/knobs.h

```cpp
#pragma once
#include "common.h"
#include <array>
#include <cstdlib>

#define FGDM_STR_(x) #x
#define FGDM_STR(x) FGDM_STR_(x)

#define FGDM_KNOBS(X)                                                                                                          \
    X(ATTN_PP, "FGDM_ATTN_PP", "1", "0: the four-wave attention kernel where the eight-wave ping-pong one would run")           \
    X(ATTN_DQ, "FGDM_ATTN_DQ", "3", "long self-attention, d = 40: 3 = two-strand kernel, 32-wide V^T P^T; 1 = 16-wide; 0 = off") \
    X(ATTN_DQ80, "FGDM_ATTN_DQ80", "1", "0: the ping-pong kernel instead of the two-strand one at d = 64 / 80")                 \
    X(ATTN_ABL, "FGDM_ATTN_ABL", "0", "ablation instantiations of the two-strand kernel (tools/bench_attention.py only)")       \
    X(ATTN_CROSS, "FGDM_ATTN_CROSS", "4", "query chunks per wave of the text-token kernel (65 - 96 keys); 0 = off")             \
    X(ATTN_CROSS_LONG, "FGDM_ATTN_CROSS_LONG", "8", "query chunks per wave of the key-resident kernel (97 - 256 keys); 0 = off") \
    X(IGEMM_EPI_PATHS, "FGDM_IGEMM_EPI_PATHS", "1", "0: the general GEMM epilogue instead of the host-selected straight-line paths") \
    X(IGEMM_HALO, "FGDM_IGEMM_HALO", "1", "0: per-tap K loop instead of the halo-tile loop (stride-1 3x3 convolutions, split K too)") \
    X(IGEMM_MFMA32, "FGDM_IGEMM_MFMA32", "0", "1: automatic tile choices take the 32x32x16 MFMA instantiations")                \
    X(IGEMM_OTHER_WIDTHS, "FGDM_IGEMM_OTHER_WIDTHS", "1", "0: widths 128 / 256 / 512 back on the 2-stage kernel")               \
    X(IGEMM_PERSIST, "FGDM_IGEMM_PERSIST", "1", "GEGLU projections: 1 = persistent, tiles round-robin; 2 = contiguous runs; 0 = off") \
    X(IGEMM_PIPE, "FGDM_IGEMM_PIPE", "1", "0: the phase-locked K loop instead of the software-pipelined one")                   \
    X(IGEMM_UP_PHASE, "FGDM_IGEMM_UP_PHASE", "1", "0: Upsample convs as the 3x3 walk over the virtual upsampled image, not four 2x2 phase GEMMs") \
    X(IGEMM_SMALL_M, "FGDM_IGEMM_SMALL_M", "1", "0: linears with a thin 128-row grid stay on 128 x 320 tiles")                  \
    X(IGEMM_SMALL_TILES, "FGDM_IGEMM_SMALL_TILES", "1", "0: the 8x8 level's linears back on the 2-stage kernel")                \
    X(IGEMM_STATS64, "FGDM_IGEMM_STATS64", "1", "0: the 64 x 160 tile leaves the LayerNorm partial sums to the row-statistics pass") \
    X(SPLITK_FAT, "FGDM_SPLITK_FAT", "1", "0: split K four ways on 128 x 320 tiles at the 8x8 level only")                      \
    X(PAIR_FAT_TILES, "FGDM_PAIR_FAT_TILES", "1", "0: grouped launches keep the tile a single problem would take")              \
    X(GN_REG, "FGDM_GN_REG", "1024", "largest pixel count per sample of the register-resident GroupNorm; 0 = off")              \
    X(GN_REG_NG, "FGDM_GN_REG_NG", "4", "widest slice of the register-resident GroupNorm, in groups")                           \
    X(GN_FUSED_MAXKB, "FGDM_GN_FUSED_MAXKB", "64", "largest LDS slice (KB) of the single-kernel GroupNorm; 0 = always two kernels") \
    X(GN_CHUNK, "FGDM_GN_CHUNK", FGDM_STR(GN_PIX_PER_CHUNK), "pixels per partial-sum chunk of the two-kernel GroupNorm (multiples of 64)") \
    X(LN_FOLD, "FGDM_LN_FOLD", "1", "fgdm_create; 0: the transformer blocks' LayerNorms as kernels of their own")               \
    X(TWIN_STREAMS, "FGDM_TWIN_STREAMS", "0", "fgdm_create; 1: the ControlNets on a second stream next to the UNet encoder")    \
    X(PAIR_LAUNCH, "FGDM_PAIR_LAUNCH", "1", "fgdm_create; 0: no grouped launches of twin layers")                               \
    X(GROUP_MAX, "FGDM_GROUP_MAX", FGDM_STR(FGDM_MAX_GROUP), "fgdm_create; problems per grouped launch, clamped to [2, FGDM_MAX_GROUP]") \
    X(GN_GROUP, "FGDM_GN_GROUP", "1", "fgdm_create; 0: single-pass GroupNorm launches stay out of the grouped launches")        \
    X(PAIR_DEBUG, "FGDM_PAIR_DEBUG", nullptr, "set (to anything): fgdm_destroy prints how many replayed launches were fused")   \
    X(PROF_DUMP, "FGDM_PROF_DUMP", nullptr, "path: fgdm_profile_end writes the per-shape time table there")                     \
    X(BENCH_DATA_SCALE, "FGDM_BENCH_DATA_SCALE", "1", "atof; scale of the random operands of fgdm_bench_igemm / _attention")

enum Knob {
#define X(id, name, dflt, meaning) KNOB_##id,
    FGDM_KNOBS(X)
#undef X
    KNOB_COUNT
};
struct KnobDef { const char* name; const char* dflt; const char* meaning; };
inline constexpr KnobDef KNOB_TABLE[KNOB_COUNT] = {
#define X(id, name, dflt, meaning) {name, dflt, meaning},
    FGDM_KNOBS(X)
#undef X
};

inline const char* knob_text(Knob k) {
    const char* v = getenv(KNOB_TABLE[k].name);
    return v ? v : KNOB_TABLE[k].dflt;
}
inline int knob_int(Knob k) { return atoi(knob_text(k)); }
inline bool knob_on(Knob k) { return knob_int(k) != 0; }
inline int knob_once(Knob k) {
    static const std::array<int, KNOB_COUNT> v = [] {
        std::array<int, KNOB_COUNT> a{};
        for (int i = 0; i < KNOB_COUNT; ++i)
            if (KNOB_TABLE[i].dflt) a[i] = knob_int((Knob)i);
        return a;
    }();
    return v[k];
}
```

### fgdm_amd/csrc/norm.hip

```cpp
#include "common.h"
#include "knobs.h"
#include <algorithm>
#include <cstring>

__device__ __forceinline__ const half_t* src_octet(const half_t* x0, int C0, const half_t* x1, int C1,
                                                   size_t pix, int o) {
    const int c = o << 3;
    return c < C0 ? x0 + pix * C0 + c : x1 + pix * C1 + (c - C0);
}

__global__ __launch_bounds__(256) void gn_stats_kernel(const half_t* __restrict__ x0, int C0,
                                                        const half_t* __restrict__ x1, int C1, int HW,
                                                        float* __restrict__ partial, int pix_per_chunk) {
    extern __shared__ float red[];
    const int C = C0 + C1, P = C >> 3, cpg = C >> 5;
    const int b = blockIdx.y, chunk = blockIdx.x, nchunk = gridDim.x;
    const int tid = threadIdx.x;
    const int p_begin = chunk * pix_per_chunk;
    const int p_end = min(HW, p_begin + pix_per_chunk);
    const int PI = P <= 256 ? 256 / P : 1;
    const int nslot = P <= 256 ? 1 : 2;
    for (int slot = 0; slot < nslot; ++slot) {
        int o, pi;
        bool active;
        if (P <= 256) { o = tid % P; pi = tid / P; active = pi < PI; }
        else { o = tid + slot * 256; pi = 0; active = o < P; }
        if (active) {
            float s[8], q[8];
#pragma unroll
            for (int e = 0; e < 8; ++e) { s[e] = 0.f; q[e] = 0.f; }
            int p = p_begin + pi;
            for (; p + 3 * PI < p_end; p += 4 * PI) {
                h8 v[4];
#pragma unroll
                for (int u = 0; u < 4; ++u) v[u] = *(const h8*)src_octet(x0, C0, x1, C1, (size_t)b * HW + p + u * PI, o);
#pragma unroll
                for (int u = 0; u < 4; ++u)
#pragma unroll
                    for (int e = 0; e < 8; ++e) { const float f = (float)v[u][e]; s[e] += f; q[e] += f * f; }
            }
            for (; p < p_end; p += PI) {
                const h8 v = *(const h8*)src_octet(x0, C0, x1, C1, (size_t)b * HW + p, o);
#pragma unroll
                for (int e = 0; e < 8; ++e) { const float f = (float)v[e]; s[e] += f; q[e] += f * f; }
            }
#pragma unroll
            for (int e = 0; e < 8; ++e) {
                red[((size_t)pi * C + (o << 3) + e) * 2] = s[e];
                red[((size_t)pi * C + (o << 3) + e) * 2 + 1] = q[e];
            }
        }
    }
    __syncthreads();
    if (tid < 64) {
        const int g = tid >> 1, which = tid & 1;
        float acc = 0.f;
        for (int pi = 0; pi < PI; ++pi)
            for (int c = g * cpg; c < (g + 1) * cpg; ++c) acc += red[((size_t)pi * C + c) * 2 + which];
        partial[((size_t)b * nchunk + chunk) * 64 + tid] = acc;
    }
}

__global__ __launch_bounds__(256) void gn_apply_kernel(const half_t* __restrict__ x0, int C0,
                                                        const half_t* __restrict__ x1, int C1, int HW,
                                                        const float* __restrict__ partial, int nchunk,
                                                        float inv_count, float eps,
                                                        const float* __restrict__ gamma,
                                                        const float* __restrict__ beta, int silu,
                                                        half_t* __restrict__ out) {
    extern __shared__ __attribute__((aligned(16))) float sc[];
    const int C = C0 + C1, P = C >> 3, cpg = C >> 5;
    const int b = blockIdx.y;
    float* scale = sc;
    float* shift = sc + C;
    float* stats = sc + 2 * C;
    {
        const int g = threadIdx.x >> 3, part = threadIdx.x & 7;
        double s = 0.0, q = 0.0;
        for (int c = part; c < nchunk; c += 8) {
            s += (double)partial[((size_t)b * nchunk + c) * 64 + g * 2];
            q += (double)partial[((size_t)b * nchunk + c) * 64 + g * 2 + 1];
        }
#pragma unroll
        for (int off = 4; off > 0; off >>= 1) { s += __shfl_xor(s, off); q += __shfl_xor(q, off); }
        if (part == 0) {
            const double mean = s * inv_count;
            double var = q * inv_count - mean * mean;
            if (var < 0.0) var = 0.0;
            stats[g * 2] = (float)mean;
            stats[g * 2 + 1] = (float)(1.0 / sqrt(var + (double)eps));
        }
    }
    __syncthreads();
    for (int c = threadIdx.x; c < C; c += 256) {
        const int g = c / cpg;
        const float mean = stats[g * 2], rstd = stats[g * 2 + 1];
        const float w = gamma[c] * rstd;
        scale[c] = w;
        shift[c] = beta[c] - mean * w;
    }
    __syncthreads();
    const unsigned total = (unsigned)HW * (unsigned)P;
    for (unsigned i0 = blockIdx.x * 1024u + threadIdx.x; i0 < total; i0 += gridDim.x * 1024u) {
        h8 v[4];
        unsigned pix[4];
        int oct[4];
#pragma unroll
        for (int u = 0; u < 4; ++u) {
            const unsigned i = i0 + (unsigned)u * 256u;
            pix[u] = i / (unsigned)P;
            oct[u] = (int)(i - pix[u] * (unsigned)P);
            if (i < total) v[u] = *(const h8*)src_octet(x0, C0, x1, C1, (size_t)b * HW + pix[u], oct[u]);
        }
// ... 243 lines not shown
    bool same = n <= FGDM_MAX_GROUP;
    for (int k = 1; k < n && same; ++k) same = gn_same_shape(r0, *(const GnRec*)args[k]);
    if (!same) {
        for (int k = 0; k < n; ++k) { const int rc = single(*(const GnRec*)args[k], grid_x, s); if (rc != FGDM_OK) return rc; }
        return FGDM_OK;
    }
    GnArgsG g{};
    for (int k = 0; k < n; ++k) g.p[k] = ((const GnRec*)args[k])->p;
    g.C0 = r0.C0; g.C1 = r0.C1; g.B = r0.B; g.HW = r0.HW; g.NG = r0.NG; g.silu = r0.silu; g.eps = r0.eps;
    return group(g, r0, grid_x, (unsigned)n, s);
}
#define GN_SINGLE(KERNEL) [](const GnRec& r, unsigned gx, hipStream_t st) -> int {                                                       \
        hipLaunchKernelGGL(KERNEL, dim3(gx), dim3(GN_BLOCK), r.smem, st, r.p.x0, r.C0, r.p.x1, r.C1, r.B, r.HW, r.NG, r.eps, r.p.gamma,   \
                           r.p.beta, r.silu, r.p.out);                                                                                 \
        return hipGetLastError() == hipSuccess ? FGDM_OK : FGDM_ERR_HIP; }
#define GN_GROUP(KERNEL) [](const GnArgsG& g, const GnRec& r, unsigned gx, unsigned n, hipStream_t st) -> int {                            \
        hipLaunchKernelGGL(KERNEL, dim3(gx, n), dim3(GN_BLOCK), r.smem, st, g);                                                       \
        return hipGetLastError() == hipSuccess ? FGDM_OK : FGDM_ERR_HIP; }
static int gn_group_fn(const void* const* args, int n, unsigned grid_x, hipStream_t s) {
    const int sel = ((const GnRec*)args[0])->np_sel;
    switch (sel) {
#define GN_BLOCK 1024
        case 6: return gn_group_dispatch(args, n, grid_x, s, 1024, GN_SINGLE(gn_reg_kernel<6>), GN_GROUP(gn_reg_group_kernel<6>));
        case 11: return gn_group_dispatch(args, n, grid_x, s, 1024, GN_SINGLE(gn_reg_kernel<11>), GN_GROUP(gn_reg_group_kernel<11>));
        case 16: return gn_group_dispatch(args, n, grid_x, s, 1024, GN_SINGLE(gn_reg_kernel<16>), GN_GROUP(gn_reg_group_kernel<16>));
        case 21: return gn_group_dispatch(args, n, grid_x, s, 1024, GN_SINGLE(gn_reg_kernel<21>), GN_GROUP(gn_reg_group_kernel<21>));
#undef GN_BLOCK
#define GN_BLOCK 256
        case 256: return gn_group_dispatch(args, n, grid_x, s, 256, GN_SINGLE(gn_fused_kernel<256>), GN_GROUP(gn_fused_group_kernel<256>));
#undef GN_BLOCK
#define GN_BLOCK 512
        case 512: return gn_group_dispatch(args, n, grid_x, s, 512, GN_SINGLE(gn_fused_kernel<512>), GN_GROUP(gn_fused_group_kernel<512>));
#undef GN_BLOCK
        default: return FGDM_ERR_ARG;
    }
}
static thread_local bool g_gn_group = true;
void groupnorm_set_group(bool on) { g_gn_group = on; }
static int gn_single_pass_launch(const GnRec& r, unsigned grid_x, hipStream_t s) {
    const void* args[1] = {&r};
    if (!fgdm_recording()) return gn_group_fn(args, 1, grid_x, s);
    const GnRec rc = r;
    static_assert(sizeof(GnRec) <= FGDM_GROUP_BLOB, "the recorded blob holds a GnRec");
    fgdm_record([rc, grid_x](hipStream_t rs) -> int { const void* a1[1] = {&rc}; return gn_group_fn(a1, 1, grid_x, rs); },
                (const void*)&gn_group_fn, g_gn_group ? gn_group_fn : nullptr, &r, sizeof(r), grid_x, gn_shape_hash(r, r.np_sel));
    return FGDM_OK;
}

size_t groupnorm_ws_floats(int B, int HW) {
    const int nchunk = (HW + 63) / 64;
    return (size_t)B * nchunk * 64 + (size_t)B * 64;
}

int groupnorm_launch(const half_t* x0, int C0, const half_t* x1, int C1, int B, int HW, const float* gamma,
                     const float* beta, float eps, int silu, half_t* out, float* ws, hipStream_t s) {
    const int C = C0 + C1;
    if ((C & 31) || (C0 & 7) || (C1 & 7) || C > 4096 || B <= 0 || HW <= 0 || (size_t)HW * (C >> 3) >= (1u << 31)) return FGDM_ERR_ARG;
    auto try_reg = [&]() -> int {
        const int reg_hw = knob_once(KNOB_GN_REG);
        const bool reg_on = HW <= reg_hw;
        const int cpg = C >> 5;
        const int ng_max = knob_once(KNOB_GN_REG_NG);
        for (int NG = ng_max; reg_on && NG >= 1; NG >>= 1) {
            const int CW = NG * cpg;
            if (CW & 7) continue;
            const int OW = CW >> 3;
            if (OW < 5 || OW > 64) continue;
            const int PI = 1024 / OW, np = (HW + PI - 1) / PI;
            if (np > 21) continue;
            const size_t smem = ((size_t)PI * CW * 2 + 8 + 2 * (size_t)CW + 2 * (size_t)CW) * sizeof(float);
            if (smem > 150 * 1024) continue;
            constexpr int lds = 150 * 1024;
            if (fgdm_dyn_lds<gn_reg_kernel<6>>(lds) || fgdm_dyn_lds<gn_reg_kernel<11>>(lds) || fgdm_dyn_lds<gn_reg_kernel<16>>(lds) ||
                fgdm_dyn_lds<gn_reg_kernel<21>>(lds) || fgdm_dyn_lds<gn_reg_group_kernel<6>>(lds) || fgdm_dyn_lds<gn_reg_group_kernel<11>>(lds) ||
                fgdm_dyn_lds<gn_reg_group_kernel<16>>(lds) || fgdm_dyn_lds<gn_reg_group_kernel<21>>(lds))
                return FGDM_ERR_HIP;
            GnRec r{{x0, x1, gamma, beta, out}, C0, C1, B, HW, NG, silu, eps, np <= 6 ? 6 : np <= 11 ? 11 : np <= 16 ? 16 : 21, (unsigned)smem};
            return gn_single_pass_launch(r, (unsigned)((32 / NG) * 8 * ((B + 7) / 8)), s);
        }
        return 1;
    };
    if ((size_t)HW * C >= 64 * 2560) { const int rc = try_reg(); if (rc != 1) return rc; }
    {
        const int cpg = C >> 5;
        const int max_kb = knob_once(KNOB_GN_FUSED_MAXKB);
        for (int pass = 0; pass < 2; ++pass)
        for (int NG = 4; NG >= 1; NG >>= 1) {
            const int CW = NG * cpg;
            const size_t slice = (size_t)HW * CW * 2;
            if ((CW & 7) || CW > 320 || slice > (size_t)std::min(pass == 0 ? 40 : 64, max_kb) * 1024) continue;
            const int NT = slice > 40 * 1024 ? 512 : 256;
            const int OW = CW >> 3, PI = NT / OW;
            const size_t smem = slice + ((size_t)PI * CW * 2 + 8 + 2 * (size_t)CW) * sizeof(float);
            if (smem > 150 * 1024) continue;
            constexpr int lds = 150 * 1024;
            if (fgdm_dyn_lds<gn_fused_kernel<256>>(lds) || fgdm_dyn_lds<gn_fused_kernel<512>>(lds) ||
                fgdm_dyn_lds<gn_fused_group_kernel<256>>(lds) || fgdm_dyn_lds<gn_fused_group_kernel<512>>(lds))
                return FGDM_ERR_HIP;
            GnRec r{{x0, x1, gamma, beta, out}, C0, C1, B, HW, NG, silu, eps, NT, (unsigned)smem};
            return gn_single_pass_launch(r, (unsigned)((32 / NG) * 8 * ((B + 7) / 8)), s);
        }
    }
    { const int rc = try_reg(); if (rc != 1) return rc; }
    const int ppc_env = knob_once(KNOB_GN_CHUNK);
    const int ppc = (ppc_env >= 64 && ppc_env % 64 == 0) ? ppc_env : GN_PIX_PER_CHUNK;
    const int nchunk = (HW + ppc - 1) / ppc;
    float* partial = ws;
    const int P = C >> 3, PI = P <= 256 ? 256 / P : 1;
    FGDM_LAUNCH(gn_stats_kernel, dim3(nchunk, B), dim3(256), (size_t)PI * C * 2 * sizeof(float), s, x0, C0, x1,
                       C1, HW, partial, ppc);
    const float inv_count = 1.0f / ((float)HW * (float)(C / 32));
    const size_t total = (size_t)HW * (C >> 3);
    int gx = (int)((total + 1023) / 1024);
    const int cap = 256 / (B < 8 ? B : 8);
    if (gx > cap) gx = cap;
    if (gx < 1) gx = 1;
    FGDM_LAUNCH(gn_apply_kernel, dim3(gx, B), dim3(256), (2 * C + 64) * sizeof(float), s, x0, C0, x1, C1, HW,
                       partial, nchunk, inv_count, eps, gamma, beta, silu, out);
    return hipGetLastError() == hipSuccess ? FGDM_OK : FGDM_ERR_HIP;
}

template <int NO>
__global__ __launch_bounds__(256) void ln_kernel(const half_t* __restrict__ x, int rows, int C,
                                                 const float* __restrict__ gamma, const float* __restrict__ beta,
                                                 float eps, half_t* __restrict__ out) {
    const int lane = threadIdx.x & 63;
    const int row = blockIdx.x * 4 + (threadIdx.x >> 6);
    if (row >= rows) return;
    const int P = C >> 3;
    h8 v[NO];
    float sum = 0.f;
#pragma unroll
    for (int k = 0; k < NO; ++k) {
        const int o = lane + k * 64;
        if (o < P) {
            v[k] = *(const h8*)(x + (size_t)row * C + (o << 3));
#pragma unroll
            for (int e = 0; e < 8; ++e) sum += (float)v[k][e];
        }
    }
#pragma unroll
    for (int off = 32; off > 0; off >>= 1) sum += __shfl_xor(sum, off);
    const float mean = sum / (float)C;
    float sq = 0.f;
#pragma unroll
    for (int k = 0; k < NO; ++k) {
        const int o = lane + k * 64;
        if (o < P) {
#pragma unroll
            for (int e = 0; e < 8; ++e) { const float d = (float)v[k][e] - mean; sq += d * d; }
        }
    }
#pragma unroll
    for (int off = 32; off > 0; off >>= 1) sq += __shfl_xor(sq, off);
    const float rstd = rsqrtf(sq / (float)C + eps);
#pragma unroll
    for (int k = 0; k < NO; ++k) {
        const int o = lane + k * 64;
        if (o < P) {
            h8 r;
#pragma unroll
            for (int e = 0; e < 8; ++e) {
                const int c = (o << 3) + e;
// ... 79 lines not shown
```

### fgdm_amd/csrc/ops_abi.hip

```cpp
#include "engine_shared.h"
#include "replay_plan.h"

static int op_pack(IgemmArgs& a, TmpDev& tmp, const float* w, const float* bias, int N, int K, int Ks, bool geglu,
                   const int* kmap = nullptr, const float* gamma = nullptr, const float* beta = nullptr) {
    auto host = [](const float* d, size_t n, std::vector<float>& v) { v.resize(n); return hipMemcpy(v.data(), d, n * sizeof(float), hipMemcpyDefault) == hipSuccess; };
    std::vector<float> wh, bh(N, 0.f), g, bt;
    if (!host(w, (size_t)N * Ks, wh) || (bias && !host(bias, N, bh))) return FGDM_ERR_HIP;
    if (gamma && (!host(gamma, K, g) || !host(beta, K, bt))) return FGDM_ERR_HIP;
    const size_t npad = igemm_npad(N);
    std::vector<half_t> pk(npad * (size_t)K, (half_t)0);
    std::vector<float> bp(npad, 0.f), u(gamma ? npad : 0, 0.f);
    for (int pr = 0; pr < N; ++pr) {
        int sr = pr;
        if (geglu) { const int grp = pr >> 6, within = pr & 63; sr = within < 32 ? grp * 32 + within : N / 2 + grp * 32 + (within - 32); }
        const float* row = &wh[(size_t)sr * Ks];
        double us = 0.0, cs = 0.0;
        for (int k = 0; k < K; ++k) {
            const int ks = kmap ? kmap[k] : k;
            if (ks < 0) continue;
            const half_t wq = (half_t)(gamma ? row[ks] * g[k] : row[ks]);
            pk[(size_t)pr * K + k] = wq;
            if (gamma) { us += (double)(float)wq; cs += (double)bt[k] * (double)row[ks]; }
        }
        bp[pr] = gamma ? (float)((double)bh[sr] + cs) : bh[sr];
        if (gamma) u[pr] = (float)us;
    }
    a.Wt = tmp.up(pk); a.bias = tmp.up(bp);
    if (gamma) a.ln_u = tmp.up(u);
    return a.Wt && a.bias && (!gamma || a.ln_u) ? FGDM_OK : FGDM_ERR_NOMEM;
}

static int op_gemm_rows(IgemmArgs& a, const half_t* A, int B, int Ho, int Wo, int K, int rps, TmpDev& tmp, hipStream_t s) {
    a.A0 = A; a.C0 = K; a.A1 = nullptr; a.C1 = 0;
    a.zero = g_zero_page();
    if (!a.zero) return FGDM_ERR_NOMEM;
    a.B = B; a.H = Ho; a.W = Wo; a.Ho = Ho; a.Wo = Wo;
    a.M = B * Ho * Wo; a.K = K; a.mode = IG_LINEAR; a.rows_per_sample = rps;
    if (plan_splitk(a, tmp) != FGDM_OK) return FGDM_ERR_NOMEM;
    return igemm_launch(a, s);
}

static int op_conv3_im2col(const half_t* x, int Cin, const float* w, const float* bias, const float* rowvec, const half_t* resid,
                           int B, int H, int W, int Cout, int stride, int act, float scale, void* out, hipStream_t s) {
    int cp = 0;
    const std::vector<int> kmap = conv3_kmap(Cin, &cp);
    const int K = (int)kmap.size(), Ho = (H - 1) / stride + 1, Wo = (W - 1) / stride + 1;
    TmpDev tmp;
    IgemmArgs a{};
    const int prc = op_pack(a, tmp, w, bias, Cout, K, Cin * 9, false, kmap.data());
    if (prc != FGDM_OK) return prc;
    half_t* A = tmp.alloc<half_t>((size_t)B * Ho * Wo * K);
    if (!A) return FGDM_ERR_NOMEM;
    a.rowvec = rowvec; a.rv_stride = Cout;
    a.resid = resid; a.ld_res = Cout;
// ... 97 lines not shown
    int slots = igemm_stats_slots(a);
    float* stats = tmp.alloc<float>((size_t)M * std::max(slots, row_stats_slots(C)) * 2);
    if (!stats) return FGDM_ERR_NOMEM;
    if (slots) a.stats_out = stats;
    rc = igemm_launch(a, s);
    if (rc == FGDM_OK && !slots) { slots = row_stats_slots(C); rc = row_stats_launch((const half_t*)h_out, M, C, stats, s); }
    if (slots_used) *slots_used = a.stats_out ? slots : -slots;
    if (rc != FGDM_OK) { (void)hipStreamSynchronize(s); return rc; }
    b.A0 = (const half_t*)h_out; b.C0 = C; b.zero = a.zero;
    b.ln_stats = stats; b.ln_slots = slots; b.ln_eps = 1e-5f;
    const int nout = act2 == ACT_GEGLU ? N2 / 2 : N2;
    b.B = 1; b.H = 1; b.W = M; b.Ho = 1; b.Wo = M; b.M = M; b.N = N2; b.K = C; b.mode = IG_LINEAR; b.act = act2;
    b.out_kind = OUT_F16; b.out = y_out; b.ld_out = nout; b.rows_per_sample = M; b.scale = 1.f;
    rc = igemm_launch(b, s);
    (void)hipStreamSynchronize(s);
    return rc;
}

int fgdm_op_ln_qkv(const void* h, const float* gamma, const float* beta, const float* wq, const float* wk, const float* wv,
                   int B, int T, int C, int Tp, int fold, void* qk, void* vt, void* stream) {
    if (!h || !wq || !wk || !wv || !qk || !vt) return FGDM_ERR_ARG;
    if (B <= 0 || T <= 0 || C <= 0 || (C % 320) || Tp < T || (Tp & 7)) return FGDM_ERR_ARG;
    if (fold ? (!gamma || !beta) : (gamma || beta)) return FGDM_ERR_ARG;
    if ((long long)B * T > 0x7fffffffLL / (3 * C)) return FGDM_ERR_ARG;
    hipStream_t s = as_stream(stream);
    const int M = B * T, N = 3 * C;
    const size_t cc = (size_t)C * C;
    std::vector<float> w(3 * cc);
    const float* src[3] = {wq, wk, wv};
    for (int i = 0; i < 3; ++i)
        if (hipMemcpy(&w[i * cc], src[i], cc * sizeof(float), hipMemcpyDefault) != hipSuccess) return FGDM_ERR_HIP;
    TmpDev tmp;
    IgemmArgs a{};
    int rc = op_pack(a, tmp, w.data(), nullptr, N, C, C, false, nullptr, fold ? gamma : nullptr, fold ? beta : nullptr);
    if (rc != FGDM_OK) return rc;
    a.A0 = (const half_t*)h; a.C0 = C; a.zero = g_zero_page();
    if (!a.zero) return FGDM_ERR_NOMEM;
    a.B = B; a.H = 1; a.W = T; a.Ho = 1; a.Wo = T; a.M = M; a.N = N; a.K = C; a.mode = IG_LINEAR; a.act = ACT_NONE;
    a.out_kind = OUT_F16; a.out = qk; a.ld_out = 2 * C; a.rows_per_sample = T; a.scale = 1.f;
    a.out2 = vt; a.out_kind2 = OUT_F16_T; a.ld_out2 = Tp; a.split_n = 2 * C;
    if (fold) {
        const int slots = row_stats_slots(C);
        float* stats = tmp.alloc<float>((size_t)M * slots * 2);
        if (!stats) return FGDM_ERR_NOMEM;
        rc = row_stats_launch((const half_t*)h, M, C, stats, s);
        if (rc != FGDM_OK) { (void)hipStreamSynchronize(s); return rc; }
        a.ln_stats = stats; a.ln_slots = slots; a.ln_eps = 1e-5f;
    }
    rc = igemm_launch(a, s);
    (void)hipStreamSynchronize(s);
    return rc;
}

int fgdm_debug_force_igemm_cfg(int cfg) { igemm_set_force_cfg(cfg); return FGDM_OK; }

int fgdm_op_groupnorm(const void* x0, int C0, const void* x1, int C1, int B, int HW, const float* gamma, const float* beta,
                      float eps, int silu, void* out, void* stream) {
    if (!x0 || !gamma || !beta || !out) return FGDM_ERR_ARG;
    hipStream_t s = as_stream(stream);
    float* ws = nullptr;
    if (hipMalloc(&ws, groupnorm_ws_floats(B, HW) * sizeof(float)) != hipSuccess) return FGDM_ERR_NOMEM;
    const int rc = groupnorm_launch((const half_t*)x0, C0, (const half_t*)x1, C1, B, HW, gamma, beta, eps, silu, (half_t*)out, ws, s);
    (void)hipStreamSynchronize(s);
    (void)hipFree(ws);
    return rc;
}
int fgdm_op_layernorm(const void* x, int rows, int C, const float* gamma, const float* beta, float eps, void* out, void* stream) {
    if (!x || !gamma || !beta || !out) return FGDM_ERR_ARG;
    return layernorm_launch((const half_t*)x, rows, C, gamma, beta, eps, (half_t*)out, as_stream(stream));
}
int fgdm_op_attention(const void* q, int ldq, const void* k, int ldk, const void* vt, int ldvt, void* o, int ldo, int B,
                      int heads, int T, int Tk, int d, void* stream) {
    if (!q || !k || !vt || !o) return FGDM_ERR_ARG;
    return attention_launch((const half_t*)q, ldq, (const half_t*)k, ldk, (const half_t*)vt, ldvt, (half_t*)o, ldo, B, heads, T, Tk, d, 0, as_stream(stream));
}
int fgdm_op_attention_ex(const void* q, int ldq, const void* k, int ldk, const void* vt, int ldvt, void* o, int ldo, int B,
                         int heads, int T, int Tk, int d, int q_prescaled, void* stream) {
    if (!q || !k || !vt || !o) return FGDM_ERR_ARG;
    return attention_launch((const half_t*)q, ldq, (const half_t*)k, ldk, (const half_t*)vt, ldvt, (half_t*)o, ldo, B, heads, T, Tk, d,
                            q_prescaled ? 1 : 0, as_stream(stream));
}
int fgdm_debug_last_attention_kernel(void) { return attention_last_kernel(); }
int fgdm_op_small_attention(const void* qkv, int ld, int koff, int voff, void* out, int ldo, int B, int heads, int T, int d,
                            int causal, void* stream) {
    if (!qkv || !out) return FGDM_ERR_ARG;
    return small_attention_launch((const half_t*)qkv, ld, koff, voff, (half_t*)out, ldo, B, heads, T, d, causal, as_stream(stream));
}

int fgdm_op_vae_attention(const void* q, const void* k, const void* vt, void* out, int B, int T, int C, void* stream) {
    if (!q || !k || !vt || !out || B <= 0 || T <= 0 || C <= 0 || (T & 63) || (C & 63)) return FGDM_ERR_ARG;
    hipStream_t s = as_stream(stream);
    TmpDev tmp;
    float* S = tmp.alloc<float>((size_t)T * T);
    half_t* P = tmp.alloc<half_t>((size_t)T * T);
    if (!S || !P) return FGDM_ERR_NOMEM;
    bool softmax_failed = false;
    const int rc = vattn_core((const half_t*)q, (const half_t*)k, (const half_t*)vt, (half_t*)out, S, P, B, T, C, s, &softmax_failed,
        [&](const half_t* Wt, int N, int K, const half_t* A, int M, int out_kind, void* o, int ld_out, float scale) {
            IgemmArgs a{};
            a.Wt = Wt; a.N = N; a.act = ACT_NONE; a.out_kind = out_kind; a.out = o; a.ld_out = ld_out; a.scale = scale;
            return op_gemm_rows(a, A, 1, 1, M, K, M, tmp, s);
        });
    (void)hipStreamSynchronize(s);
    return rc;
}
int fgdm_op_softmax_rows(const float* S, void* P, int rows, int cols, void* stream) {
// ... 88 lines not shown
```

### fgdm_amd/engine.py

```python
import ctypes as C
import os
from collections import OrderedDict

import numpy as np
import torch

from . import _lib

SD_V1 = dict(in_channels=4, out_channels=4, model_channels=320, attention_resolutions=(4, 2, 1),
             num_res_blocks=2, channel_mult=(1, 2, 4, 4), num_heads=8, context_dim=768)


SD_VAE = dict(ch=128, out_ch=3, ch_mult=(1, 2, 4, 4), num_res_blocks=2, attn_resolutions=(), z_channels=4)


SD_CLIP = dict(vocab_size=49408, hidden_size=768, intermediate_size=3072, num_hidden_layers=12,
               num_attention_heads=12, max_position_embeddings=77)


def make_config(cfg=None, use_adapter=False, n_controlnets=0, hint_channels=3, workspace_bytes=0, vae=None, clip=None,
                num_prompts=1, vae_encoder=False):
    if vae_encoder and not vae:
        raise ValueError('vae_encoder needs the first-stage config: pass vae=True or a ddconfig dict')
    if cfg is not None and ('target' in cfg or any(k not in SD_V1 for k in cfg)):
# ... 341 lines not shown
    def run_block(self, prefix, x, emb=None, ctx=None, x_skip=None):
        f32 = lambda v: None if v is None else v.to(self.device, torch.float32).contiguous()
        x, emb, ctx, x_skip = f32(x), f32(emb), f32(ctx), f32(x_skip)
        if ctx is not None:
            self.set_context_tokens(ctx.shape[1])
        B, Cc, H, W = x.shape
        cap = 4 * B * 1280 * 4 * H * W
        out = torch.empty(cap, device=self.device, dtype=torch.float32)
        n = C.c_int64(0)
        rc = self.lib.fgdm_run_block(self.h, prefix.encode(), _ptr(x), Cc, _ptr(x_skip), 0 if x_skip is None else x_skip.shape[1],
                                     _ptr(emb), _ptr(ctx), B, H, W, _ptr(out), cap, C.byref(n), _stream())
        self._check(rc, f'fgdm_run_block({prefix})')
        return out[:n.value]

    def controlnet(self, cn, x, t, ctx):
        x = x.to(self.device, torch.float32).contiguous()
        t = t.to(self.device, torch.int64).contiguous()
        ctx = ctx.to(self.device, torch.float32).contiguous()
        self.set_context_tokens(ctx.shape[1])
        B, _, H, W = x.shape
        shapes = self.control_shapes(B, H, W)
        total = sum(int(np.prod(s)) for s in shapes)
        buf = torch.empty(total, device=self.device, dtype=torch.float32)
        rc = self.lib.fgdm_controlnet(self.h, cn, _ptr(x), _ptr(t), _ptr(ctx), B, H, W, _ptr(buf), total, _stream())
        self._check(rc, 'fgdm_controlnet')
        outs, off = [], 0
        for s in shapes:
            n = int(np.prod(s))
            outs.append(buf[off:off + n].view(*s))
            off += n
        return outs

    PROFILE_CLASSES = ('igemm', 'attention', 'norm', 'im2col')

    def profile_begin(self, stride=1):
        self._check(self.lib.fgdm_profile_begin(self.h, int(stride)), 'fgdm_profile_begin')

    def profile_end(self):
        buf = (C.c_double * 16)()
        self._check(self.lib.fgdm_profile_end(self.h, buf), 'fgdm_profile_end')
        return {n: dict(ms=buf[4 * i], launches=int(buf[4 * i + 1]), work=buf[4 * i + 2], bytes=buf[4 * i + 3])
                for i, n in enumerate(self.PROFILE_CLASSES)}

    def workspace_stats(self):
        a, b = C.c_int64(), C.c_int64()
        self._check(self.lib.fgdm_workspace_stats(self.h, C.byref(a), C.byref(b)), 'fgdm_workspace_stats')
        return dict(peak_bytes=a.value, reserved_bytes=b.value)

    def launch_stats(self):
        a, b, c = C.c_int64(), C.c_int64(), C.c_int64()
        self._check(self.lib.fgdm_launch_stats(self.h, C.byref(a), C.byref(b), C.byref(c)), 'fgdm_launch_stats')
        return dict(replayed_launches=a.value, fused_launches=b.value, fused_problems=c.value)

    def control_shapes(self, B, H, W):
        c = self.config
        mc = c.model_channels
        shapes = [(B, mc, H, W)]
        ch, h, w = mc, H, W
        for level in range(c.n_levels):
            for _ in range(c.num_res_blocks):
                ch = mc * c.channel_mult[level]
                shapes.append((B, ch, h, w))
            if level != c.n_levels - 1:
                h, w = (h - 1) // 2 + 1, (w - 1) // 2 + 1
                shapes.append((B, ch, h, w))
        shapes.append((B, ch, h, w))
        return shapes

    def sample_ddim(self, x_T, cond, uncond, cfg_scale, timesteps, alphas, alphas_prev, sqrt_one_minus_alphas,
                    control_scales=None, flags=0):
        x = x_T.to(self.device, torch.float32).clone().contiguous()
        cond = cond.to(self.device, torch.float32).contiguous()
        if uncond is not None:
            uncond = uncond.to(self.device, torch.float32).contiguous()
            if tuple(uncond.shape) != tuple(cond.shape):
                raise ValueError(f'sample_ddim: cond {tuple(cond.shape)} and uncond {tuple(uncond.shape)} must agree')
        self.set_context_tokens(cond.shape[1])
        B, _, H, W = x.shape
        S = len(timesteps)
        ts = (C.c_int64 * S)(*[int(v) for v in timesteps])
        fa = lambda a: (C.c_float * S)(*[float(v) for v in a])
        if control_scales is not None:
            sc_host = np.asarray(control_scales, dtype=np.float32).ravel().copy()
            sc_ptr = sc_host.ctypes.data_as(C.c_void_p)
        else:
            sc_ptr = C.c_void_p(0)
        rc = self.lib.fgdm_sample_ddim(self.h, _ptr(x), _ptr(cond), _ptr(uncond), float(cfg_scale), S, ts, fa(alphas),
                                       fa(alphas_prev), fa(sqrt_one_minus_alphas), sc_ptr, B, H, W, flags, _stream())
        self._ctx_policy = ContextCachePolicy()
        self._check(rc, 'fgdm_sample_ddim')
        return x

    def sample_ddim_ex(self, x_T, cond, uncond, cfg_scale, timesteps, alphas, alphas_prev, sqrt_one_minus_alphas, sigmas=None,
                       cfg_scales=None, step_noise=None, mask=None, x0=None, q_noise=None, sqrt_alphas_cumprod_t=None,
                       sqrt_one_minus_alphas_cumprod_t=None, log_steps=(), control_scales=None, flags=0, out=None,
                       x_inter_out=None, pred_x0_out=None):
        dev = lambda v: None if v is None else v.to(self.device, torch.float32).contiguous()
        x = x_T.to(self.device, torch.float32).clone().contiguous() if out is None else out.copy_(x_T)
        cond, uncond = dev(cond), dev(uncond)
        if uncond is not None and tuple(uncond.shape) != tuple(cond.shape):
            raise ValueError(f'sample_ddim_ex: cond {tuple(cond.shape)} and uncond {tuple(uncond.shape)} must agree')
        self.set_context_tokens(cond.shape[1])
        B, _, H, W = x.shape
        S, n_log = len(timesteps), len(log_steps)
        step_noise, q_noise, mask, x0 = dev(step_noise), dev(q_noise), dev(mask), dev(x0)
        for name, v, shape in (('step_noise', step_noise, (S, *x.shape)), ('q_noise', q_noise, (S, *x.shape)),
# ... 237 lines not shown
```

### include/fgdm.h

```cpp
#ifndef FGDM_H
#define FGDM_H
#include <stdint.h>
#ifdef __cplusplus
extern "C" {
#endif

#define FGDM_MAX_LEVELS 8
#define FGDM_MAX_CONTROLNETS 4

typedef struct fgdm_engine fgdm_engine;

typedef struct fgdm_config {
    int32_t in_channels, out_channels, model_channels, num_res_blocks;
    int32_t n_levels;
    int32_t channel_mult[FGDM_MAX_LEVELS];
    int32_t n_attention_resolutions;
    int32_t attention_resolutions[FGDM_MAX_LEVELS];
    int32_t num_heads, context_dim;
    int32_t use_adapter;
    int32_t n_controlnets;
    int32_t hint_channels;
    int64_t workspace_bytes;
    int32_t vae_ch, vae_n_levels;
    int32_t vae_ch_mult[FGDM_MAX_LEVELS];
// ... 124 lines not shown
    const float* alphas_prev;
    const float* sqrt_one_minus_alphas;
    const float* control_scales;
    const float* mask;
    const float* x0;
    const float* q_noise;
    const float* sqrt_alphas_cumprod_t;
    const float* sqrt_one_minus_alphas_cumprod_t;
    const int32_t* log_steps;
    float* x_inter_out;
    float* pred_x0_out;
    float cfg_scale;
    int32_t S;
    int32_t B;
    int32_t H;
    int32_t W;
    int32_t flags;
    int32_t n_log;
    int32_t reserved0;
} fgdm_plms_params;
int fgdm_sample_plms(fgdm_engine* e, const fgdm_plms_params* p, void* stream);

#define FGDM_DPMPP_FIRST 1
#define FGDM_DPMPP_SECOND 2
#define FGDM_DPMPP_PARAMS_SIZE_V1 128
typedef struct fgdm_dpmpp_params {
    int64_t struct_size;
    float* x;
    const float* cond;
    const float* uncond;
    const float* control_scales;
    const float* t_float;
    const float* inv_alpha;
    const float* neg_sigma_over_alpha;
    const int32_t* update_kind;
    const float* c1;
    const float* cm0;
    const float* cm1;
    float cfg_scale;
    int32_t n_eval;
    int32_t B;
    int32_t H;
    int32_t W;
    int32_t flags;
    int32_t reserved0;
    int32_t reserved1;
} fgdm_dpmpp_params;
int fgdm_sample_dpmpp(fgdm_engine* e, const fgdm_dpmpp_params* p, void* stream);

int fgdm_profile_begin(fgdm_engine* e, int stride );
int fgdm_profile_end(fgdm_engine* e, double* out);
int fgdm_workspace_stats(fgdm_engine* e, int64_t* peak_bytes, int64_t* reserved_bytes);
int fgdm_launch_stats(fgdm_engine* e, int64_t* replayed_launches, int64_t* fused_launches, int64_t* fused_problems);
int fgdm_replay_plan(int n_walks, const int32_t* lens, const uint64_t* key, const uint32_t* grid_x, const uint64_t* shape,
                     int group_max, int chunk, int32_t* out, int out_cap, int* limits);

#define FGDM_STRIDE2_PAD_BR (-2)
int fgdm_op_conv2d(const void* x0, int C0, const void* x1, int C1, const float* w, const float* bias,
                   const float* rowvec, const void* resid, int B, int H, int W, int Cout, int ksize, int stride,
                   int upsample, int act, float scale, void* out, void* stream);
int fgdm_op_linear(const void* x, const float* w, const float* bias, const void* resid, int M, int K, int N,
                   int act, int out_kind, int rows_per_sample, int ld_out, void* out, void* stream);
int fgdm_op_linear_ln_linear(const void* x, const float* w1, const float* b1, const void* resid, const float* gamma,
                             const float* beta, const float* w2, const float* b2, int M, int K1, int C, int N2, int act2,
                             void* h_out, void* y_out, int* slots_used, void* stream);
int fgdm_debug_force_igemm_cfg(int cfg);
int fgdm_bench_igemm(int B, int H, int W, int C0, int C1, int Cout, int ksize, int stride, int upsample, int act,
                     int use_resid, int cfg, int iters, float* avg_ms);
int fgdm_bench_ff(int M, int C, int chunk_rows, int iters, float* avg_ms);
int fgdm_bench_attention(int B, int heads, int T, int Tk, int d, int iters, float* avg_ms);
int fgdm_bench_norm(int kind, int B, int HW, int C0, int C1, int silu, int iters, float* avg_ms);
int fgdm_op_groupnorm(const void* x0, int C0, const void* x1, int C1, int B, int HW, const float* gamma,
                      const float* beta, float eps, int silu, void* out, void* stream);
int fgdm_op_layernorm(const void* x, int rows, int C, const float* gamma, const float* beta, float eps,
                      void* out, void* stream);
int fgdm_op_attention(const void* q, int ldq, const void* k, int ldk, const void* vt, int ldvt, void* o, int ldo,
                      int B, int heads, int T, int Tk, int d, void* stream);
int fgdm_op_attention_ex(const void* q, int ldq, const void* k, int ldk, const void* vt, int ldvt, void* o, int ldo,
                         int B, int heads, int T, int Tk, int d, int q_prescaled, void* stream);
int fgdm_debug_last_attention_kernel(void);
int fgdm_op_small_attention(const void* qkv, int ld, int koff, int voff, void* out, int ldo, int B, int heads, int T, int d,
                            int causal, void* stream);

int fgdm_op_vae_attention(const void* q, const void* k, const void* vt, void* out, int B, int T, int C, void* stream);
int fgdm_op_softmax_rows(const float* S, void* P, int rows, int cols, void* stream);
int fgdm_op_nchw_to_nhwc(const float* x, void* y, int B, int C, int HW, int Cpad, void* stream);
int fgdm_op_nhwc_to_nchw(const void* x, float* y, int B, int C, int HW, void* stream);
int fgdm_op_pack_xcat(const float* x, const void* cc16, int B, int Bc, int Cc, int H, int W, int cin_pad, void* out, void* stream);
int fgdm_op_avgpool2(const void* x, void* y, int B, int H, int W, int C, void* stream);
int fgdm_op_transpose_pad(const void* v, void* vt, int B, int Tk, int C, int Tkpad, void* stream);
int fgdm_op_timestep_embed(const int64_t* t, const float* t_float, void* y, int B, int dim, int rows_pad, void* stream);
int fgdm_op_add_f16(const void* a, const void* b, void* y, int64_t n, void* stream);

int fgdm_op_ddim_loop_step(const float* x, const float* e_cond, const float* e_uncond, float cfg_scale, float a_t, float a_prev,
                           float sigma_t, float sqrt_one_minus_at, const float* noise, const float* mask, const float* x0,
                           const float* q_noise, float sqrt_ac_next, float sqrt_one_minus_ac_next, float* x_out, float* xin_a,
                           float* xin_b, float* log_x, float* log_pred_x0, int64_t n, void* stream);

int fgdm_op_plms_loop_step(const float* x, const float* e_cond, const float* e_uncond, float cfg_scale, int mode, int order,
                           const float* e1, const float* e2, const float* e3, float* e_out, float a_t, float a_prev,
                           float sqrt_one_minus_at, const float* mask, const float* x0, const float* q_noise, float sqrt_ac_next,
                           float sqrt_one_minus_ac_next, float* x_out, float* xin_a, float* xin_b, float* log_x, float* log_pred_x0,
                           int64_t n, void* stream);
int fgdm_op_dpmpp_loop_step(const float* x, const float* e_cond, const float* e_uncond, float cfg_scale, float inv_alpha,
                            float neg_sigma_over_alpha, const float* m1, int update_kind, float c1, float cm0, float cm1,
                            float* m0_out, float* x_out, float* xin_a, float* xin_b, int64_t n, void* stream);
// ... 9 lines not shown
```

Measured before the change: 8.219.

## Emit GroupNorm partial sums from producing GEMM epilogue to skip stats pass

The implicit-GEMM epilogue for the 256x320 tile now accumulates per-group sum and sum-of-squares of its output and writes per-block partials. The engine threads these partials through res, attention and block forward passes so the following GroupNorm can skip its separate statistics kernel. This saves one full read of the activation per GroupNorm, at the cost of extra LDS work, a barrier in the GEMM epilogue, and more template instantiations. A test entry point and a counter are added to check the producer partials against the standalone stats.

```diff
diff --git a/fgdm_amd/_lib.py b/fgdm_amd/_lib.py
--- a/fgdm_amd/_lib.py
+++ b/fgdm_amd/_lib.py
@@ -114,6 +114,8 @@
     'fgdm_profile_end': (_i, [_p, C.POINTER(C.c_double)]),
     'fgdm_workspace_stats': (_i, [_p, C.POINTER(_i64), C.POINTER(_i64)]),
     'fgdm_launch_stats': (_i, [_p, C.POINTER(_i64), C.POINTER(_i64), C.POINTER(_i64)]),
+    'fgdm_gn_producer_stats': (_i, [_p, C.POINTER(_i64)]),
+    'fgdm_op_conv_gn_partials': (_i, [_p, _p, _i, _p, _p, _p, _p, _i, _i, _i, _i, _i, _p, _p, _p, _p, _p, _p, C.POINTER(_i), _p]),
     'fgdm_replay_plan': (_i, [_i, _p, _p, _p, _p, _i, _i, _p, _i, _p]),
     'fgdm_op_conv2d': (_i, [_p, _i, _p, _i, _p, _p, _p, _p, _i, _i, _i, _i, _i, _i, _i, _i, _f, _p, _p]),
     'fgdm_op_linear': (_i, [_p, _p, _p, _p, _i, _i, _i, _i, _i, _i, _i, _p, _p]),
diff --git a/fgdm_amd/csrc/common.h b/fgdm_amd/csrc/common.h
--- a/fgdm_amd/csrc/common.h
+++ b/fgdm_amd/csrc/common.h
@@ -45,6 +45,16 @@
     asm("v_fma_f32 %0, %1, %2, %3" : "=v"(t) : "v"(-mean), "v"(u), "v"(acc));
     asm("v_mul_f32 %0, %1, %2" : "=v"(w) : "v"(rstd), "v"(t));
     return w;
+}
+
+#define GN_BLOCK_PIX 32
+__device__ __forceinline__ void gn_acc(float& s, float& q, float f) {
+    s += f;
+    q = __builtin_fmaf(f, f, q);
+}
+__device__ __forceinline__ void gn_acc2(float& s, float& q, h2 x) {
+    s = __builtin_amdgcn_fdot2(x, h2{(half_t)1, (half_t)1}, s, false);
+    q = __builtin_amdgcn_fdot2(x, x, q, false);
 }
 
 #define FGDM_OK 0
@@ -87,6 +97,7 @@
     float* stats_out;
     void* out2;
     int split_n, out_kind2, ld_out2;
+    float* gn_partial_out;
 };
 
 int igemm_launch(const IgemmArgs& a, hipStream_t s);
@@ -96,6 +107,8 @@
 void igemm_set_twin_layers(bool on);
 void igemm_set_pair_hint(int mult);
 int igemm2_launch(const IgemmArgs& a, int cfg, hipStream_t s);
+bool igemm_gn_partials(const IgemmArgs& a);
+bool igemm2_gn_capable(const IgemmArgs& a, int cfg);
 int igemm_stats_slots(const IgemmArgs& a);
 int row_stats_slots(int C);
 int row_stats_launch(const half_t* x, int rows, int C, float* stats , hipStream_t s);
@@ -107,7 +120,10 @@
 void groupnorm_set_group(bool on);
 int groupnorm_launch(const half_t* x0, int C0, const half_t* x1, int C1, int B, int HW,
                      const float* gamma, const float* beta, float eps, int silu,
-                     half_t* out, float* ws , hipStream_t s);
+                     half_t* out, float* ws , hipStream_t s,
+                     const float* partial_in = nullptr );
+int groupnorm_stats_launch(const half_t* x0, int C0, const half_t* x1, int C1, int B, int HW, float* partial, hipStream_t s);
+bool groupnorm_takes_partials(int C, int HW);
 size_t groupnorm_ws_floats(int B, int HW);
 int layernorm_launch(const half_t* x, int rows, int C, const float* gamma, const float* beta, float eps,
                      half_t* out, hipStream_t s);
diff --git a/fgdm_amd/csrc/engine.hip b/fgdm_amd/csrc/engine.hip
--- a/fgdm_amd/csrc/engine.hip
+++ b/fgdm_amd/csrc/engine.hip
@@ -142,6 +142,8 @@
     int group_max = FGDM_MAX_GROUP;
     bool gn_group = true;
     ReplayStats replay_stats;
+    bool gn_producer_stats = true;
+    int64_t gn_stats_skipped = 0;
     struct Deferred { const GemmW* w; Tensor src; int idx; float scale; Arena* owner; };
     Prof prof;
 
@@ -350,6 +352,7 @@
         int ld_out = 0;
         void* out2 = nullptr; int out_kind2 = OUT_F16, ld_out2 = 0, split_n = 0;
         int rps = 0;
+        float** gn_part = nullptr;
     };
     int gemm(const GemmW& w, int mode, const Tensor& x0, const Tensor* x1, int Ho, int Wo, const Epi& e, Tensor* out) {
         IgemmArgs a{};
@@ -394,6 +397,14 @@
             if (!e.stats->p) return fail(FGDM_ERR_NOMEM, "workspace (LayerNorm statistics)");
             if (e.stats->slots) a.stats_out = e.stats->p;
         }
+        if (e.gn_part) {
+            *e.gn_part = nullptr;
+            if (gn_producer_stats && !e.out && groupnorm_takes_partials(nout, a.rows_per_sample) && igemm_gn_partials(a)) {
+                a.gn_partial_out = (float*)ar->alloc((size_t)(a.M / 256) * 64 * sizeof(float));
+                if (!a.gn_partial_out) return fail(FGDM_ERR_NOMEM, "workspace (GroupNorm statistics)");
+                *e.gn_part = a.gn_partial_out;
+            }
+        }
         double nbytes = 0.0;
         if (prof.on) {
             const double in_b = 2.0 * ((double)x0.numel() + (x1 ? (double)x1->numel() : 0.0));
@@ -441,7 +452,7 @@
         if (!e.out) { *out = talloc(x.B, x.H, x.W, e.act == ACT_GEGLU ? w.N / 2 : w.N); if (!out->p) return fail(FGDM_ERR_NOMEM, "workspace"); }
         return gemm(w, IG_LINEAR, x, x1, x.H, x.W, e, out);
     }
-    int gnorm(const NormW& n, const Tensor& x, const Tensor* x1, float eps, bool silu, Tensor* out) {
+    int gnorm(const NormW& n, const Tensor& x, const Tensor* x1, float eps, bool silu, Tensor* out, const float* part = nullptr) {
         const int C = x.C + (x1 ? x1->C : 0);
         *out = talloc(x.B, x.H, x.W, C);
         float* ws = (float*)ar->alloc(groupnorm_ws_floats(x.B, x.H * x.W) * sizeof(float));
@@ -450,9 +461,10 @@
         if (prof.on) snprintf(tag, sizeof(tag), "groupnorm B%d HW%d C%d", x.B, x.H * x.W, C);
         prof.begin(PC_NORM, s, 4.0 * (double)out->numel(), tag);
         const int rc = groupnorm_launch(x.p, x.C, x1 ? x1->p : nullptr, x1 ? x1->C : 0, x.B, x.H * x.W, n.g, n.b, eps,
-                                        silu ? 1 : 0, out->p, ws, s);
+                                        silu ? 1 : 0, out->p, ws, s, part);
         prof.end(s);
         ar->release(ws);
+        if (part && rc == FGDM_OK) ++gn_stats_skipped;
         return rc == FGDM_OK ? rc : fail(rc, "groupnorm launch failed");
     }
     int lnorm(const NormW& n, const Tensor& x, Tensor* out) {
@@ -468,9 +480,11 @@
 
     struct EmbCtx { const float* emb_all; int stride; };
 
-    int res_fwd(const Layer& l, const Tensor& x, const Tensor* x1, const EmbCtx& ec, Tensor* out) {
+    int res_fwd(const Layer& l, const Tensor& x, const Tensor* x1, const EmbCtx& ec, Tensor* out, const float* x_part = nullptr,
+                float** out_part = nullptr) {
         Tensor g1, h, g2, sk, xp;
-        CHK(gnorm(l.gn1, x, x1, l.eps, true, &g1));
+        float* h_part = nullptr;
+        CHK(gnorm(l.gn1, x, x1, l.eps, true, &g1, x1 ? nullptr : x_part));
         const Tensor* xs = &x;
         if (l.down) {
             if (x1) return fail(FGDM_ERR_ARG, "down ResBlock with a concatenated input");
@@ -485,11 +499,14 @@
         }
         Epi e1;
         if (l.emb_off >= 0) { e1.rowvec = ec.emb_all + l.emb_off; e1.rv_stride = ec.stride; }
+        e1.gn_part = &h_part;
         CHK(conv3(l.c1, g1, nullptr, 1, false, e1, &h));
         tfree(g1);
-        CHK(gnorm(l.gn2, h, nullptr, l.eps, true, &g2));
+        CHK(gnorm(l.gn2, h, nullptr, l.eps, true, &g2, h_part));
+        if (h_part) ar->release(h_part);
         tfree(h);
         Epi e2;
+        e2.gn_part = out_part;
         if (l.cin != l.cout) {
             CHK(linear(l.skip, *xs, Epi{}, &sk, x1));
             e2.resid = sk.p; e2.ld_res = sk.C;
@@ -544,13 +561,14 @@
         return FGDM_OK;
     }
 
-    int attn_fwd(const Layer& l, const Tensor& x_in, const Tensor& ctx16, Tensor* out, bool dup = false) {
+    int attn_fwd(const Layer& l, const Tensor& x_in, const Tensor& ctx16, Tensor* out, bool dup = false, const float* x_part = nullptr,
+                 float** out_part = nullptr) {
         Tensor x = x_in, x_full;
         int B = x.B;
         const int T = x.H * x.W, C = x.C, d = C / l.heads;
         Tensor g, h, qk, vt, a, h2, q2, k2, v2t, f;
         LnStats s1, s2, s3;
-        CHK(gnorm(l.gn, x, nullptr, 1e-6f, false, &g));
+        CHK(gnorm(l.gn, x, nullptr, 1e-6f, false, &g, x_part));
         Tensor nrm;
         { Epi e; if (ln_fold) e.stats = &s1; CHK(linear(l.pin, g, e, &h)); }
         tfree(g);
@@ -622,7 +640,7 @@
         if (nrm.p) tfree(nrm);
         { Epi e; e.resid = h.p; e.ld_res = C; CHK(linear(l.ffo, f, e, &h2)); }
         tfree(f); tfree(h);
-        { Epi e; e.resid = x.p; e.ld_res = C; CHK(linear(l.pout, h2, e, out)); }
+        { Epi e; e.resid = x.p; e.ld_res = C; e.gn_part = out_part; CHK(linear(l.pout, h2, e, out)); }
         tfree(h2);
         if (x_full.p) tfree(x_full);
         return FGDM_OK;
@@ -659,24 +677,35 @@
     }
 
     int block_fwd(const Block& blk, Tensor x, bool own_x, const Tensor* x1, const EmbCtx& ec, const Tensor& ctx16,
-                  const half_t* conv_resid, Tensor* out) {
+                  const half_t* conv_resid, Tensor* out, const float* x_part = nullptr, float** out_part = nullptr) {
         Tensor cur = x;
         bool own = own_x;
+        float* part = nullptr;
+        if (out_part) *out_part = nullptr;
         for (size_t j = 0; j < blk.size(); ++j) {
             const Layer& l = blk[j];
             Tensor nxt;
+            float* nxt_part = nullptr;
+            const bool last = j + 1 == blk.size();
+            const bool gn_next = last ? out_part != nullptr : (blk[j + 1].type == L_RES || blk[j + 1].type == L_ATTN);
+            float** np = gn_next ? &nxt_part : nullptr;
+            const float* cp = j == 0 ? x_part : part;
             switch (l.type) {
                 case L_CONV: { Epi e; if (conv_resid) { e.resid = conv_resid; e.ld_res = l.cout; }
+                               e.gn_part = np;
                                CHK(conv3(l.conv, cur, nullptr, 1, false, e, &nxt)); break; }
-                case L_RES: CHK(res_fwd(l, cur, j == 0 ? x1 : nullptr, ec, &nxt)); break;
-                case L_ATTN: CHK(attn_fwd(l, cur, ctx16, &nxt)); break;
+                case L_RES: CHK(res_fwd(l, cur, j == 0 ? x1 : nullptr, ec, &nxt, cp, np)); break;
+                case L_ATTN: CHK(attn_fwd(l, cur, ctx16, &nxt, false, cp, np)); break;
                 case L_DOWN: CHK(conv3(l.conv, cur, nullptr, 2, false, Epi{}, &nxt)); break;
                 case L_UP: CHK(conv3(l.conv, cur, nullptr, 1, true, Epi{}, &nxt)); break;
             }
+            if (part) ar->release(part);
+            part = nxt_part;
             if (own) tfree(cur);
             cur = nxt;
             own = true;
         }
+        if (out_part) *out_part = part;
         *out = cur;
         return FGDM_OK;
     }
@@ -1101,16 +1130,19 @@
                                 [&](size_t) { return RecordScope(*this, nullptr, &arena); }));
         }
         h = hm;
+        float* out_part = nullptr;
         for (size_t i = 0; i < n.output.size(); ++i) {
             Tensor skip = hs.back();
             hs.pop_back();
             Tensor nxt;
-            CHK(block_fwd(n.output[i], h, true, &skip, ec, ctx16, nullptr, &nxt));
+            const bool last = i + 1 == n.output.size();
+            CHK(block_fwd(n.output[i], h, true, &skip, ec, ctx16, nullptr, &nxt, nullptr, last ? &out_part : nullptr));
             tfree(skip);
             h = nxt;
         }
         Tensor g;
-        CHK(gnorm(n.out_gn, h, nullptr, 1e-5f, true, &g));
+        CHK(gnorm(n.out_gn, h, nullptr, 1e-5f, true, &g, out_part));
+        if (out_part) ar->release(out_part);
         tfree(h);
         { Epi e; e.out_kind = OUT_F32_NCHW; e.out = eps_out; e.ld_out = HW; CHK(conv3(n.out_conv, g, nullptr, 1, false, e, nullptr)); }
         tfree(g);
@@ -1356,6 +1388,7 @@
     if (rc != FGDM_OK) return rc;
     e->device = device;
     e->ln_fold = knob_on(KNOB_LN_FOLD);
+    e->gn_producer_stats = knob_on(KNOB_GN_PRODUCER_STATS);
     rc = e->ensure_device();
     if (rc != FGDM_OK) {
         g_create_err = e->err + " [" + hipGetErrorString(hipGetLastError()) + "]";
@@ -1523,6 +1556,12 @@
     *replayed_launches = (int64_t)e->replay_stats.replayed;
     *fused_launches = (int64_t)e->replay_stats.fused;
     *fused_problems = (int64_t)e->replay_stats.problems;
+    return FGDM_OK;
+}
+
+int fgdm_gn_producer_stats(fgdm_engine* e, int64_t* skipped_stats_launches) {
+    if (!e || !skipped_stats_launches) return FGDM_ERR_ARG;
+    *skipped_stats_launches = e->gn_stats_skipped;
     return FGDM_OK;
 }
 
diff --git a/fgdm_amd/csrc/igemm.hip b/fgdm_amd/csrc/igemm.hip
--- a/fgdm_amd/csrc/igemm.hip
+++ b/fgdm_amd/csrc/igemm.hip
@@ -325,6 +325,13 @@
     return (tile == 0 || tile == 2 || tile == 3 || tile == 5 || (tile == 7 && stats64)) ? a.N / 160 : 0;
 }
 
+bool igemm_gn_partials(const IgemmArgs& a) {
+    if (a.splitk > 1 || a.mode == IG_CONV2_PHASE || (a.K & 63) || (a.C0 & 63) || (a.C1 & 63)) return false;
+    if (knob_once(KNOB_IGEMM_MFMA32) != 0) return false;
+    const int f = pick_force(a);
+    return f >= 4 && igemm2_gn_capable(a, f - 4);
+}
+
 bool igemm_up_phase(const IgemmArgs& a) {
     if (!knob_once(KNOB_IGEMM_UP_PHASE)) return false;
     const int force = a.force_cfg ? a.force_cfg : g_force_cfg;
@@ -349,6 +356,7 @@
     if (a.act == ACT_GEGLU && (a.N & 63)) return FGDM_ERR_ARG;
     if (a.ln_stats && (a.mode != IG_LINEAR || a.C1 || a.ln_slots <= 0 || !a.ln_u)) return FGDM_ERR_ARG;
     if (a.stats_out && igemm_stats_slots(a) == 0) return FGDM_ERR_ARG;
+    if (a.gn_partial_out && !igemm_gn_partials(a)) return FGDM_ERR_ARG;
     if (a.out2 && (a.act == ACT_GEGLU || a.splitk > 1 || a.stats_out || a.split_n <= 0 || a.split_n >= a.N || (a.split_n % 640))) return FGDM_ERR_ARG;
     if (a.mode == IG_CONV2_PHASE && (a.splitk > 1 || a.N % 320)) return FGDM_ERR_ARG;
     if (a.splitk > 1) {
diff --git a/fgdm_amd/csrc/igemm2.hip b/fgdm_amd/csrc/igemm2.hip
--- a/fgdm_amd/csrc/igemm2.hip
+++ b/fgdm_amd/csrc/igemm2.hip
@@ -37,8 +37,9 @@
     return PIPE == 2 ? 2 * halo_px<BM>() * ROWB + STAGES * BN * ROWB : STAGES * (BM + BN) * ROWB;
 }
 
-template <int BM, int BN, int WM, int WN, int STAGES, int CONV, bool GEGLU, bool SPLIT, int MS, bool LN, int PATH, int PIPE, bool ABL>
+template <int BM, int BN, int WM, int WN, int STAGES, int CONV, bool GEGLU, bool SPLIT, int MS, bool LN, int PATHX, int PIPE, bool ABL>
 __device__ __forceinline__ void igemm2_body(const IgemmArgs& a, const int yb) {
+    constexpr int PATH = PATHX > 2 ? PATHX - 2 : PATHX;
     constexpr int NW = WM * WN, T = NW * 64;
     constexpr int TM = BM / WM, TN = BN / WN;
     constexpr int MI = TM / MS, NI = TN / MS;
@@ -575,6 +576,12 @@
     const int nvalid = GEGLU ? a.N / 2 : nend - ncol0;
     const float* bw = bias_l + wn * TN;
 
+    constexpr bool GNP = PATHX > 2;
+    static_assert(!GNP || (BM == 256 && BN == 320 && MS == 16 && !LN && !GEGLU && !SPLIT && !ABL && CONV != 2), "the tile that emits GroupNorm partial sums");
+    static_assert(!GNP || NW * CST_BYTES + (BM / 32) * (BN / 2) * 2 * 4 <= RING_BYTES, "the block sums sit in the ring behind the staging tiles");
+    float* const gn_tab = (float*)(smem + NW * CST_BYTES);
+    constexpr bool gn_on = GNP;
+
     constexpr int PT = 32 / MS;
     constexpr int NG = AR / 4;
 #pragma unroll
@@ -698,6 +705,14 @@
                 if (ok[it]) {
                     if (a.resid) v[it] = v[it] + rr[it];
                     *(h8*)((half_t*)outp + goff[it]) = v[it];
+                    if constexpr (GNP) {
+                        if (gn_on && a.resid) {
+                            const int c = lane + it * 64, pr = c / CPR, ck = c - pr * CPR;
+                            char* sp = cst + pr * PITCH + ck * 16;
+                            *(h4*)sp = h4{v[it][0], v[it][1], v[it][2], v[it][3]};
+                            *(h4*)(sp + 8) = h4{v[it][4], v[it][5], v[it][6], v[it][7]};
+                        }
+                    }
                 }
                 if (want_stats) {
                     const int c = lane + it * 64;
@@ -743,6 +758,41 @@
                     }
                 }
                 asm volatile("s_waitcnt lgkmcnt(0)" ::: "memory");
+            }
+            if constexpr (GNP) {
+                if (gn_on) {
+                    if (lane < OUT_TN / 4) {
+                        float sm[2] = {0.f, 0.f}, sq[2] = {0.f, 0.f};
+                        const char* col = cst + lane * 8;
+#pragma unroll
+                        for (int p0 = 0; p0 < GN_BLOCK_PIX; p0 += 8) {
+                            h4 x[8];
+#pragma unroll
+                            for (int u = 0; u < 8; ++u) x[u] = *(const h4*)(col + (p0 + u) * PITCH);
+#pragma unroll
+                            for (int u = 0; u < 8; ++u) {
+                                gn_acc2(sm[0], sq[0], h2{x[u][0], x[u][1]});
+                                gn_acc2(sm[1], sq[1], h2{x[u][2], x[u][3]});
+                            }
+                        }
+                        float* t = gn_tab + ((size_t)((wm * (TM / 32) + ip) * (BN / 2) + (wn * TN) / 2 + lane * 2)) * 2;
+                        *(f32x4*)t = f32x4{sm[0], sq[0], sm[1], sq[1]};
+                    }
+                    asm volatile("s_waitcnt lgkmcnt(0)" ::: "memory");
+                }
+            }
+        }
+    }
+    if constexpr (GNP) {
+        if (gn_on) {
+            __builtin_amdgcn_s_barrier();
+            const int cpg = a.N >> 5, ngt = BN / cpg, upg = cpg >> 1;
+            if (tid < 2 * ngt) {
+                const int g = tid >> 1, which = tid & 1;
+                float sum = 0.f;
+                for (int bl = 0; bl < BM / GN_BLOCK_PIX; ++bl)
+                    for (int c = g * upg; c < (g + 1) * upg; ++c) sum += gn_tab[(bl * (BN / 2) + c) * 2 + which];
+                a.gn_partial_out[((size_t)(m0 / BM) * 32 + n0 / cpg) * 2 + tid] = sum;
             }
         }
     }
@@ -1070,10 +1120,14 @@
     }
     if (a.debug) return FGDM_ERR_ARG;
     if constexpr (SPLIT) return launch2p<BM, BN, WM, WN, STAGES, CONV, GEGLU, SPLIT, MS, LN, 0, PIPE, false>(a, s);
+    constexpr bool GNI = BM == 256 && BN == 320 && MS == 16 && !LN && !GEGLU && !SPLIT && CONV != 2 && PIPE != 0;
+    if (a.gn_partial_out && !(GNI && FAST && fast_on && epilogue_path<BM, GEGLU, LN>(a) != 0)) return FGDM_ERR_ARG;
     if constexpr (FAST && !SPLIT) {
         switch (fast_on ? epilogue_path<BM, GEGLU, LN>(a) : 0) {
-            case 1: return launch2p<BM, BN, WM, WN, STAGES, CONV, GEGLU, SPLIT, MS, LN, 1, PIPE, false>(a, s);
-            case 2: if constexpr (!GEGLU && !LN && CONV != 2) return launch2p<BM, BN, WM, WN, STAGES, CONV, GEGLU, SPLIT, MS, LN, 2, PIPE, false>(a, s);
+            case 1: if constexpr (GNI) { if (a.gn_partial_out) return launch2p<BM, BN, WM, WN, STAGES, CONV, GEGLU, SPLIT, MS, LN, 3, PIPE, false>(a, s); }
+                    return launch2p<BM, BN, WM, WN, STAGES, CONV, GEGLU, SPLIT, MS, LN, 1, PIPE, false>(a, s);
+            case 2: if constexpr (GNI) { if (a.gn_partial_out) return launch2p<BM, BN, WM, WN, STAGES, CONV, GEGLU, SPLIT, MS, LN, 4, PIPE, false>(a, s); }
+                    if constexpr (!GEGLU && !LN && CONV != 2) return launch2p<BM, BN, WM, WN, STAGES, CONV, GEGLU, SPLIT, MS, LN, 2, PIPE, false>(a, s);
             default: break;
         }
     }
@@ -1160,8 +1214,25 @@
     return a.W == 8 && a.H == 8;
 }
 
+static bool pipelined_loop(const IgemmArgs& a, int cfg) {
+    const int psel = cfg >> 4;
+    const size_t px = a.mode == IG_LINEAR ? (size_t)a.M : (size_t)a.B * a.H * a.W;
+    const bool small = px * (size_t)std::max(a.C0, a.C1) * 2 < (1ull << 32) && (size_t)(a.N + 320) * a.K * 2 < (1ull << 32);
+    return (psel == 0 ? knob_once(KNOB_IGEMM_PIPE) != 0 : psel == 2) && small;
+}
+
+bool igemm2_gn_capable(const IgemmArgs& a, int cfg) {
+    if ((cfg & 15) != 0 || a.debug || a.splitk > 1 || !knob_once(KNOB_IGEMM_EPI_PATHS)) return false;
+    if (a.mode != IG_LINEAR && !(a.mode == IG_CONV3 && a.Ho == a.H && a.Wo == a.W)) return false;
+    if (a.out_kind != OUT_F16 || a.act != ACT_NONE || a.out2 || a.ln_stats || a.stats_out || a.ld_out != a.N) return false;
+    if ((a.K & 31) || (a.C0 & 31) || (a.C1 & 31) || a.N % 320 || 320 % (a.N / 32) || ((a.N / 32) & 1)) return false;
+    if (!pipelined_loop(a, cfg)) return false;
+    return a.M % 256 == 0 && a.rows_per_sample % 256 == 0 && epilogue_path<256, false, false>(a) != 0;
+}
+
 int igemm2_launch(const IgemmArgs& a, int cfg, hipStream_t s) {
     if ((a.K & 31) || (a.C0 & 31) || (a.C1 & 31)) return FGDM_ERR_ARG;
+    if (a.gn_partial_out && !igemm2_gn_capable(a, cfg)) return FGDM_ERR_ARG;
     const int pipe_default = knob_once(KNOB_IGEMM_PIPE);
     const int tile = cfg & 15, psel = cfg >> 4;
     const size_t px = a.mode == IG_LINEAR ? (size_t)a.M : (size_t)a.B * a.H * a.W;
diff --git a/fgdm_amd/csrc/knobs.h b/fgdm_amd/csrc/knobs.h
--- a/fgdm_amd/csrc/knobs.h
+++ b/fgdm_amd/csrc/knobs.h
@@ -29,6 +29,7 @@
     X(GN_REG_NG, "FGDM_GN_REG_NG", "4", "widest slice of the register-resident GroupNorm, in groups")                           \
     X(GN_FUSED_MAXKB, "FGDM_GN_FUSED_MAXKB", "64", "largest LDS slice (KB) of the single-kernel GroupNorm; 0 = always two kernels") \
     X(GN_CHUNK, "FGDM_GN_CHUNK", FGDM_STR(GN_PIX_PER_CHUNK), "pixels per partial-sum chunk of the two-kernel GroupNorm (multiples of 64)") \
+    X(GN_PRODUCER_STATS, "FGDM_GN_PRODUCER_STATS", "1", "fgdm_create; 0: every two-kernel GroupNorm runs its own statistics pass (same bits)") \
     X(LN_FOLD, "FGDM_LN_FOLD", "1", "fgdm_create; 0: the transformer blocks' LayerNorms as kernels of their own")               \
     X(TWIN_STREAMS, "FGDM_TWIN_STREAMS", "0", "fgdm_create; 1: the ControlNets on a second stream next to the UNet encoder")    \
     X(PAIR_LAUNCH, "FGDM_PAIR_LAUNCH", "1", "fgdm_create; 0: no grouped launches of twin layers")                               \
diff --git a/fgdm_amd/csrc/norm.hip b/fgdm_amd/csrc/norm.hip
--- a/fgdm_amd/csrc/norm.hip
+++ b/fgdm_amd/csrc/norm.hip
@@ -9,56 +9,58 @@
     return c < C0 ? x0 + pix * C0 + c : x1 + pix * C1 + (c - C0);
 }
 
-__global__ __launch_bounds__(256) void gn_stats_kernel(const half_t* __restrict__ x0, int C0,
-                                                        const half_t* __restrict__ x1, int C1, int HW,
-                                                        float* __restrict__ partial, int pix_per_chunk) {
+template <bool PAIR>
+__global__ __launch_bounds__(1024) void gn_stats_kernel(const half_t* __restrict__ x0, int C0,
+                                                         const half_t* __restrict__ x1, int C1, int HW,
+                                                         float* __restrict__ partial, int pix_per_chunk, int rb) {
     extern __shared__ float red[];
-    const int C = C0 + C1, P = C >> 3, cpg = C >> 5;
+    constexpr int U = PAIR ? 2 : 1, UO = 8 / U;
+    const int C = C0 + C1, P = C >> 3, NU = C / U, upg = NU >> 5;
     const int b = blockIdx.y, chunk = blockIdx.x, nchunk = gridDim.x;
-    const int tid = threadIdx.x;
+    const int tid = threadIdx.x, NT = blockDim.x;
     const int p_begin = chunk * pix_per_chunk;
     const int p_end = min(HW, p_begin + pix_per_chunk);
-    const int PI = P <= 256 ? 256 / P : 1;
-    const int nslot = P <= 256 ? 1 : 2;
-    for (int slot = 0; slot < nslot; ++slot) {
-        int o, pi;
-        bool active;
-        if (P <= 256) { o = tid % P; pi = tid / P; active = pi < PI; }
-        else { o = tid + slot * 256; pi = 0; active = o < P; }
-        if (active) {
-            float s[8], q[8];
-#pragma unroll
-            for (int e = 0; e < 8; ++e) { s[e] = 0.f; q[e] = 0.f; }
-            int p = p_begin + pi;
-            for (; p + 3 * PI < p_end; p += 4 * PI) {
+    const int nblk = (p_end - p_begin + GN_BLOCK_PIX - 1) / GN_BLOCK_PIX;
+    float acc = 0.f;
+    for (int b0 = 0; b0 < nblk; b0 += rb) {
+        const int nb = min(rb, nblk - b0);
+        for (int task = tid; task < nb * P; task += NT) {
+            const int bl = task / P, o = task - bl * P;
+            int p = p_begin + (b0 + bl) * GN_BLOCK_PIX;
+            const int pe = min(p_end, p + GN_BLOCK_PIX);
+            float s[UO], q[UO];
+#pragma unroll
+            for (int e = 0; e < UO; ++e) { s[e] = 0.f; q[e] = 0.f; }
+            auto add = [&](const h8& v) {
+#pragma unroll
+                for (int e = 0; e < UO; ++e) {
+                    if constexpr (PAIR) gn_acc2(s[e], q[e], h2{v[2 * e], v[2 * e + 1]});
+                    else gn_acc(s[e], q[e], (float)v[e]);
+                }
+            };
+            for (; p + 3 < pe; p += 4) {
                 h8 v[4];
 #pragma unroll
-                for (int u = 0; u < 4; ++u) v[u] = *(const h8*)src_octet(x0, C0, x1, C1, (size_t)b * HW + p + u * PI, o);
-#pragma unroll
-                for (int u = 0; u < 4; ++u)
-#pragma unroll
-                    for (int e = 0; e < 8; ++e) { const float f = (float)v[u][e]; s[e] += f; q[e] += f * f; }
+                for (int u = 0; u < 4; ++u) v[u] = *(const h8*)src_octet(x0, C0, x1, C1, (size_t)b * HW + p + u, o);
+#pragma unroll
+                for (int u = 0; u < 4; ++u) add(v[u]);
             }
-            for (; p < p_end; p += PI) {
-                const h8 v = *(const h8*)src_octet(x0, C0, x1, C1, (size_t)b * HW + p, o);
-#pragma unroll
-                for (int e = 0; e < 8; ++e) { const float f = (float)v[e]; s[e] += f; q[e] += f * f; }
+            for (; p < pe; ++p) add(*(const h8*)src_octet(x0, C0, x1, C1, (size_t)b * HW + p, o));
+#pragma unroll
+            for (int e = 0; e < UO; ++e) {
+                red[((size_t)bl * NU + o * UO + e) * 2] = s[e];
+                red[((size_t)bl * NU + o * UO + e) * 2 + 1] = q[e];
             }
-#pragma unroll
-            for (int e = 0; e < 8; ++e) {
-                red[((size_t)pi * C + (o << 3) + e) * 2] = s[e];
-                red[((size_t)pi * C + (o << 3) + e) * 2 + 1] = q[e];
-            }
-        }
-    }
-    __syncthreads();
-    if (tid < 64) {
-        const int g = tid >> 1, which = tid & 1;
-        float acc = 0.f;
-        for (int pi = 0; pi < PI; ++pi)
-            for (int c = g * cpg; c < (g + 1) * cpg; ++c) acc += red[((size_t)pi * C + c) * 2 + which];
-        partial[((size_t)b * nchunk + chunk) * 64 + tid] = acc;
-    }
+        }
+        __syncthreads();
+        if (tid < 64) {
+            const int g = tid >> 1, which = tid & 1;
+            for (int bl = 0; bl < nb; ++bl)
+                for (int c = g * upg; c < (g + 1) * upg; ++c) acc += red[((size_t)bl * NU + c) * 2 + which];
+        }
+        __syncthreads();
+    }
+    if (tid < 64) partial[((size_t)b * nchunk + chunk) * 64 + tid] = acc;
 }
 
 __global__ __launch_bounds__(256) void gn_apply_kernel(const half_t* __restrict__ x0, int C0,
@@ -408,24 +410,63 @@
     return (size_t)B * nchunk * 64 + (size_t)B * 64;
 }
 
+static bool gn_reg_slice_ok(int C, int HW, int NG) {
+    const int CW = NG * (C >> 5);
+    if (CW & 7) return false;
+    const int OW = CW >> 3;
+    if (OW < 5 || OW > 64) return false;
+    const int PI = 1024 / OW, np = (HW + PI - 1) / PI;
+    if (np > 21) return false;
+    return ((size_t)PI * CW * 2 + 8 + 2 * (size_t)CW + 2 * (size_t)CW) * sizeof(float) <= 150 * 1024;
+}
+static int gn_reg_fit(int C, int HW) {
+    if (HW > knob_once(KNOB_GN_REG)) return 0;
+    for (int NG = knob_once(KNOB_GN_REG_NG); NG >= 1; NG >>= 1)
+        if (gn_reg_slice_ok(C, HW, NG)) return NG;
+    return 0;
+}
+static bool gn_fused_slice_ok(int C, int HW, int NG, int pass) {
+    const int CW = NG * (C >> 5);
+    const size_t slice = (size_t)HW * CW * 2;
+    if ((CW & 7) || CW > 320 || slice > (size_t)std::min(pass == 0 ? 40 : 64, knob_once(KNOB_GN_FUSED_MAXKB)) * 1024) return false;
+    const int NT = slice > 40 * 1024 ? 512 : 256, OW = CW >> 3, PI = NT / OW;
+    return slice + ((size_t)PI * CW * 2 + 8 + 2 * (size_t)CW) * sizeof(float) <= 150 * 1024;
+}
+static int gn_chunk_pixels() {
+    const int ppc_env = knob_once(KNOB_GN_CHUNK);
+    return (ppc_env >= 64 && ppc_env % 64 == 0) ? ppc_env : GN_PIX_PER_CHUNK;
+}
+bool groupnorm_takes_partials(int C, int HW) {
+    if ((C & 31) || C > 4096 || HW <= 0 || HW % 256 || gn_chunk_pixels() != 256) return false;
+    if (gn_reg_fit(C, HW)) return false;
+    for (int pass = 0; pass < 2; ++pass)
+        for (int NG = 4; NG >= 1; NG >>= 1)
+            if (gn_fused_slice_ok(C, HW, NG, pass)) return false;
+    return true;
+}
+
+int groupnorm_stats_launch(const half_t* x0, int C0, const half_t* x1, int C1, int B, int HW, float* partial, hipStream_t s) {
+    const int C = C0 + C1;
+    if ((C & 31) || (C0 & 7) || (C1 & 7) || C > 4096 || B <= 0 || HW <= 0 || !partial) return FGDM_ERR_ARG;
+    const int ppc = gn_chunk_pixels(), nchunk = (HW + ppc - 1) / ppc;
+    const int P = C >> 3, rb = std::max(1, std::min(ppc / GN_BLOCK_PIX, 65536 / (C * 8)));
+    const int nt = std::min(1024, (rb * P + 63) / 64 * 64);
+    if ((C >> 5) & 1) FGDM_LAUNCH(gn_stats_kernel<false>, dim3(nchunk, B), dim3(nt), (size_t)rb * C * 2 * sizeof(float), s, x0, C0, x1, C1, HW, partial, ppc, rb);
+    else FGDM_LAUNCH(gn_stats_kernel<true>, dim3(nchunk, B), dim3(nt), (size_t)rb * C * 2 * sizeof(float), s, x0, C0, x1, C1, HW, partial, ppc, rb);
+    return hipGetLastError() == hipSuccess ? FGDM_OK : FGDM_ERR_HIP;
+}
+
 int groupnorm_launch(const half_t* x0, int C0, const half_t* x1, int C1, int B, int HW, const float* gamma,
-                     const float* beta, float eps, int silu, half_t* out, float* ws, hipStream_t s) {
+                     const float* beta, float eps, int silu, half_t* out, float* ws, hipStream_t s, const float* partial_in) {
     const int C = C0 + C1;
     if ((C & 31) || (C0 & 7) || (C1 & 7) || C > 4096 || B <= 0 || HW <= 0 || (size_t)HW * (C >> 3) >= (1u << 31)) return FGDM_ERR_ARG;
+    if (partial_in && (x1 || !groupnorm_takes_partials(C, HW))) return FGDM_ERR_ARG;
     auto try_reg = [&]() -> int {
-        const int reg_hw = knob_once(KNOB_GN_REG);
-        const bool reg_on = HW <= reg_hw;
         const int cpg = C >> 5;
-        const int ng_max = knob_once(KNOB_GN_REG_NG);
-        for (int NG = ng_max; reg_on && NG >= 1; NG >>= 1) {
-            const int CW = NG * cpg;
-            if (CW & 7) continue;
-            const int OW = CW >> 3;
-            if (OW < 5 || OW > 64) continue;
+        if (const int NG = gn_reg_fit(C, HW)) {
+            const int CW = NG * cpg, OW = CW >> 3;
             const int PI = 1024 / OW, np = (HW + PI - 1) / PI;
-            if (np > 21) continue;
             const size_t smem = ((size_t)PI * CW * 2 + 8 + 2 * (size_t)CW + 2 * (size_t)CW) * sizeof(float);
-            if (smem > 150 * 1024) continue;
             constexpr int lds = 150 * 1024;
             if (fgdm_dyn_lds<gn_reg_kernel<6>>(lds) || fgdm_dyn_lds<gn_reg_kernel<11>>(lds) || fgdm_dyn_lds<gn_reg_kernel<16>>(lds) ||
                 fgdm_dyn_lds<gn_reg_kernel<21>>(lds) || fgdm_dyn_lds<gn_reg_group_kernel<6>>(lds) || fgdm_dyn_lds<gn_reg_group_kernel<11>>(lds) ||
@@ -439,16 +480,14 @@
     if ((size_t)HW * C >= 64 * 2560) { const int rc = try_reg(); if (rc != 1) return rc; }
     {
         const int cpg = C >> 5;
-        const int max_kb = knob_once(KNOB_GN_FUSED_MAXKB);
         for (int pass = 0; pass < 2; ++pass)
         for (int NG = 4; NG >= 1; NG >>= 1) {
+            if (!gn_fused_slice_ok(C, HW, NG, pass)) continue;
             const int CW = NG * cpg;
             const size_t slice = (size_t)HW * CW * 2;
-            if ((CW & 7) || CW > 320 || slice > (size_t)std::min(pass == 0 ? 40 : 64, max_kb) * 1024) continue;
             const int NT = slice > 40 * 1024 ? 512 : 256;
             const int OW = CW >> 3, PI = NT / OW;
             const size_t smem = slice + ((size_t)PI * CW * 2 + 8 + 2 * (size_t)CW) * sizeof(float);
-            if (smem > 150 * 1024) continue;
             constexpr int lds = 150 * 1024;
             if (fgdm_dyn_lds<gn_fused_kernel<256>>(lds) || fgdm_dyn_lds<gn_fused_kernel<512>>(lds) ||
                 fgdm_dyn_lds<gn_fused_group_kernel<256>>(lds) || fgdm_dyn_lds<gn_fused_group_kernel<512>>(lds))
@@ -458,13 +497,10 @@
         }
     }
     { const int rc = try_reg(); if (rc != 1) return rc; }
-    const int ppc_env = knob_once(KNOB_GN_CHUNK);
-    const int ppc = (ppc_env >= 64 && ppc_env % 64 == 0) ? ppc_env : GN_PIX_PER_CHUNK;
+    const int ppc = gn_chunk_pixels();
     const int nchunk = (HW + ppc - 1) / ppc;
-    float* partial = ws;
-    const int P = C >> 3, PI = P <= 256 ? 256 / P : 1;
-    FGDM_LAUNCH(gn_stats_kernel, dim3(nchunk, B), dim3(256), (size_t)PI * C * 2 * sizeof(float), s, x0, C0, x1,
-                       C1, HW, partial, ppc);
+    const float* partial = partial_in ? partial_in : ws;
+    if (!partial_in && groupnorm_stats_launch(x0, C0, x1, C1, B, HW, ws, s) != FGDM_OK) return FGDM_ERR_HIP;
     const float inv_count = 1.0f / ((float)HW * (float)(C / 32));
     const size_t total = (size_t)HW * (C >> 3);
     int gx = (int)((total + 1023) / 1024);
diff --git a/fgdm_amd/csrc/ops_abi.hip b/fgdm_amd/csrc/ops_abi.hip
--- a/fgdm_amd/csrc/ops_abi.hip
+++ b/fgdm_amd/csrc/ops_abi.hip
@@ -1,5 +1,6 @@
 #include "engine_shared.h"
 #include "replay_plan.h"
+#include "replay.h"
 
 static int op_pack(IgemmArgs& a, TmpDev& tmp, const float* w, const float* bias, int N, int K, int Ks, bool geglu,
                    const int* kmap = nullptr, const float* gamma = nullptr, const float* beta = nullptr) {
@@ -203,6 +204,61 @@
     return rc;
 }
 
+int fgdm_op_conv_gn_partials(const void* x, const void* x2, int Cin, const float* w, const float* bias, const float* rowvec,
+                             const void* resid, int B, int H, int W, int Cout, int ksize, void* out, void* out2,
+                             float* partial_producer, float* partial_producer2, float* partial_stats, float* partial_stats2,
+                             int* info, void* stream) {
+    if (!x || !w || !out || !partial_producer || !partial_stats || !info || (ksize != 1 && ksize != 3)) return FGDM_ERR_ARG;
+    if (x2 && (!out2 || !partial_producer2 || !partial_stats2)) return FGDM_ERR_ARG;
+    if (B <= 0 || H <= 0 || W <= 0 || Cin <= 0 || (Cin & 63) || Cout <= 0 || (Cout & 31)) return FGDM_ERR_ARG;
+    hipStream_t s = as_stream(stream);
+    const int taps = ksize * ksize, K = taps * Cin;
+    std::vector<int> kmap(K);
+    for (int tap = 0; tap < taps; ++tap)
+        for (int c = 0; c < Cin; ++c) kmap[taps == 9 ? ((c >> 6) * 9 + tap) * 64 + (c & 63) : c] = c * taps + tap;
+    TmpDev tmp;
+    IgemmArgs a{};
+    const int prc = op_pack(a, tmp, w, bias, Cout, K, K, false, kmap.data());
+    if (prc != FGDM_OK) return prc;
+    a.A0 = (const half_t*)x; a.C0 = Cin;
+    a.zero = g_zero_page();
+    if (!a.zero) return FGDM_ERR_NOMEM;
+    a.rowvec = rowvec; a.rv_stride = Cout;
+    a.resid = (const half_t*)resid; a.ld_res = Cout;
+    a.B = B; a.H = H; a.W = W; a.Ho = H; a.Wo = W; a.mode = ksize == 3 ? IG_CONV3 : IG_LINEAR;
+    a.M = B * H * W; a.N = Cout; a.K = K;
+    a.act = ACT_NONE; a.out_kind = OUT_F16; a.out = out; a.ld_out = Cout;
+    a.rows_per_sample = H * W; a.scale = 1.f;
+    if (plan_splitk(a, tmp) != FGDM_OK) return FGDM_ERR_NOMEM;
+    const bool emit = igemm_gn_partials(a);
+    info[0] = emit ? 1 : 0; info[1] = 0;
+    if (emit) a.gn_partial_out = partial_producer;
+    int rc;
+    if (!x2) {
+        rc = igemm_launch(a, s);
+    } else {
+        IgemmArgs b = a;
+        b.A0 = (const half_t*)x2; b.out = out2;
+        if (emit) b.gn_partial_out = partial_producer2;
+        if (b.splitk > 1 && !(b.ws = tmp.alloc<float>((size_t)b.splitk * b.M * b.N))) return FGDM_ERR_NOMEM;
+        RecWalk w0, w1;
+        RecWalk* before = fgdm_record_into(&w0);
+        rc = igemm_launch(a, s);
+        fgdm_record_into(&w1);
+        if (rc == FGDM_OK) rc = igemm_launch(b, s);
+        fgdm_record_into(before);
+        struct NoTimer : LaunchTimer { void begin(int, hipStream_t, double, const char*, double) override {} void end(hipStream_t) override {} } nt;
+        ReplayStats st;
+        std::vector<RecWalk*> lists{&w0, &w1};
+        if (rc == FGDM_OK) rc = fgdm_replay(lists, 2, s, nt, st);
+        info[1] = (int)st.fused;
+    }
+    if (rc == FGDM_OK) rc = groupnorm_stats_launch((const half_t*)out, Cout, nullptr, 0, B, H * W, partial_stats, s);
+    if (rc == FGDM_OK && x2) rc = groupnorm_stats_launch((const half_t*)out2, Cout, nullptr, 0, B, H * W, partial_stats2, s);
+    (void)hipStreamSynchronize(s);
+    return rc;
+}
+
 int fgdm_debug_force_igemm_cfg(int cfg) { igemm_set_force_cfg(cfg); return FGDM_OK; }
 
 int fgdm_op_groupnorm(const void* x0, int C0, const void* x1, int C1, int B, int HW, const float* gamma, const float* beta,
diff --git a/fgdm_amd/engine.py b/fgdm_amd/engine.py
--- a/fgdm_amd/engine.py
+++ b/fgdm_amd/engine.py
@@ -417,6 +417,11 @@
         self._check(self.lib.fgdm_launch_stats(self.h, C.byref(a), C.byref(b), C.byref(c)), 'fgdm_launch_stats')
         return dict(replayed_launches=a.value, fused_launches=b.value, fused_problems=c.value)
 
+    def gn_producer_stats(self):
+        a = C.c_int64()
+        self._check(self.lib.fgdm_gn_producer_stats(self.h, C.byref(a)), 'fgdm_gn_producer_stats')
+        return a.value
+
     def control_shapes(self, B, H, W):
         c = self.config
         mc = c.model_channels
diff --git a/include/fgdm.h b/include/fgdm.h
--- a/include/fgdm.h
+++ b/include/fgdm.h
@@ -200,6 +200,11 @@
 int fgdm_profile_end(fgdm_engine* e, double* out);
 int fgdm_workspace_stats(fgdm_engine* e, int64_t* peak_bytes, int64_t* reserved_bytes);
 int fgdm_launch_stats(fgdm_engine* e, int64_t* replayed_launches, int64_t* fused_launches, int64_t* fused_problems);
+int fgdm_gn_producer_stats(fgdm_engine* e, int64_t* skipped_stats_launches);
+int fgdm_op_conv_gn_partials(const void* x, const void* x2, int Cin, const float* w, const float* bias, const float* rowvec,
+                             const void* resid, int B, int H, int W, int Cout, int ksize, void* out, void* out2,
+                             float* partial_producer, float* partial_producer2, float* partial_stats, float* partial_stats2,
+                             int* info, void* stream);
 int fgdm_replay_plan(int n_walks, const int32_t* lens, const uint64_t* key, const uint32_t* grid_x, const uint64_t* shape,
                      int group_max, int chunk, int32_t* out, int out_cap, int* limits);
 
```

New measurement: 8.233, median of 6. About the same (+0.2%).
